# peabody124/PosePipeline

Hardware: AMD Instinct MI355X
Metric: frames/sec (whole node), detect->2D->3D cascade on 1080p; MPJPE vs reference (higher is better)
Workload: dtype f32; eligible float32 convolutions are evaluated as 2-term float16 splits (22 significand bits under per-channel / per-sample power-of-two scales, 3 products per term) on the 16-bit matrix cores with float32 accumulation (float32-accurate at any input magnitude, not bit-identical: tests/test_gpu_spl

## Files before the change

### posepipeline_amd/csrc/api_core.hip

```cpp
#include <dlfcn.h>

#include <algorithm>
#include <memory>

#include "pp_internal.h"
#include "pp_amax.h"

#include <atomic>
extern std::atomic<int> g_decode_generic, g_split_gemm_epi;

static thread_local std::string g_last_error;

void pp_set_error(const char* fmt, ...) {
    char buf[1024];
    va_list ap;
    va_start(ap, fmt);
    vsnprintf(buf, sizeof(buf), fmt, ap);
    va_end(ap);
    g_last_error = buf;
}

namespace {
struct Roctx {
    int (*push)(const char*) = nullptr;
    int (*pop)() = nullptr;
    Roctx() {
        for (const char* lib : {"librocprofiler-sdk-roctx.so", "librocprofiler-sdk-roctx.so.1", "libroctx64.so", "libroctx64.so.4"}) {
            void* h = dlopen(lib, RTLD_LAZY | RTLD_LOCAL);
            if (!h) continue;
            push = reinterpret_cast<int (*)(const char*)>(dlsym(h, "roctxRangePushA"));
            pop = reinterpret_cast<int (*)()>(dlsym(h, "roctxRangePop"));
            if (push && pop) return;
            push = nullptr; pop = nullptr;
        }
    }
};
const Roctx& roctx() {
    static const Roctx r;
    return r;
}
}

void pp_range_push(const char* name) {
    if (roctx().push) (void)roctx().push(name);
}
void pp_range_pop() {
    if (roctx().pop) (void)roctx().pop();
}

int pp_ctx::ensure_scratch(size_t bytes) {
    if (bytes <= scratch_bytes) return PP_OK;
    if (scratch) {
        PP_HIP_CHECK(hipStreamSynchronize(stream));
        PP_HIP_CHECK(hipFree(scratch));
        scratch = nullptr;
        scratch_bytes = 0;
    }
    size_t want = std::max(bytes, size_t(1) << 20);
    PP_HIP_CHECK(hipMalloc(&scratch, want));
    scratch_bytes = want;
    return PP_OK;
}

extern "C" {

int pp_abi_version(void) { return PP_ABI_VERSION; }

int pp_debug_knob(const char* name, int value) {
    PP_REQUIRE(name && value >= -1 && value <= 1, "pp_debug_knob: name and a value in {-1, 0, 1}");
    if (!strcmp(name, "decode_generic")) g_decode_generic.store(value, std::memory_order_relaxed);
    else if (!strcmp(name, "split_gemm_epilogue")) g_split_gemm_epi.store(value, std::memory_order_relaxed);
    else {
        pp_set_error("pp_debug_knob: unknown knob '%s' (decode_generic, split_gemm_epilogue)", name);
        return PP_ERR_ARG;
    }
    return PP_OK;
}

const char* pp_last_error(void) { return g_last_error.c_str(); }

int pp_device_count(void) {
    int n = 0;
    if (hipGetDeviceCount(&n) != hipSuccess) {
        (void)hipGetLastError();
        return 0;
    }
    return n;
}

int pp_ctx_create(int device, pp_ctx** out) {
    PP_REQUIRE(out != nullptr, "pp_ctx_create: out is NULL");
    *out = nullptr;
    int n = 0;
    hipError_t e = hipGetDeviceCount(&n);
    if (e != hipSuccess || n <= 0) {
        (void)hipGetLastError();
        pp_set_error("pp_ctx_create: no HIP device visible (%s) -- this library has no CPU fallback",
                     e == hipSuccess ? "device count 0" : hipGetErrorString(e));
        return PP_ERR_HIP;
    }
    PP_REQUIRE(device >= 0 && device < n, "pp_ctx_create: device %d out of range [0,%d)", device, n);
    PP_HIP_CHECK(hipSetDevice(device));
    std::unique_ptr<pp_ctx> c(new pp_ctx());
    c->device = device;
    PP_HIP_CHECK(hipStreamCreateWithFlags(&c->stream, hipStreamNonBlocking));
    PP_HIP_CHECK(hipEventCreate(&c->ev_start));
    PP_HIP_CHECK(hipEventCreate(&c->ev_stop));
    PP_HIP_CHECK(hipStreamCreateWithFlags(&c->copy_stream, hipStreamNonBlocking));
    PP_HIP_CHECK(hipEventCreateWithFlags(&c->ev_upload, hipEventDisableTiming));
    PP_HIP_CHECK(hipEventCreateWithFlags(&c->ev_consumed, hipEventDisableTiming));
    *out = c.release();
    return PP_OK;
}

void pp_ctx_destroy(pp_ctx* ctx) {
    if (!ctx) return;
    (void)hipSetDevice(ctx->device);
    if (ctx->stream) (void)hipStreamSynchronize(ctx->stream);
    if (ctx->scratch) (void)hipFree(ctx->scratch);
    if (ctx->ev_start) (void)hipEventDestroy(ctx->ev_start);
    if (ctx->ev_stop) (void)hipEventDestroy(ctx->ev_stop);
    if (ctx->copy_stream) {
        (void)hipStreamSynchronize(ctx->copy_stream);
        (void)hipStreamDestroy(ctx->copy_stream);
    }
    if (ctx->ev_upload) (void)hipEventDestroy(ctx->ev_upload);
    if (ctx->ev_consumed) (void)hipEventDestroy(ctx->ev_consumed);
    if (ctx->own_stream && ctx->stream) (void)hipStreamDestroy(ctx->stream);
    delete ctx;
}

int pp_ctx_set_stream(pp_ctx* ctx, void* hip_stream) {
    PP_REQUIRE(ctx, "pp_ctx_set_stream: ctx is NULL");
    PP_HIP_CHECK(hipStreamSynchronize(ctx->stream));
    if (ctx->own_stream && ctx->stream) PP_HIP_CHECK(hipStreamDestroy(ctx->stream));
    ctx->stream = static_cast<hipStream_t>(hip_stream);
    ctx->own_stream = false;
    return PP_OK;
}

int pp_ctx_synchronize(pp_ctx* ctx) {
    PP_REQUIRE(ctx, "pp_ctx_synchronize: ctx is NULL");
    PP_HIP_CHECK(hipStreamSynchronize(ctx->stream));
    return PP_OK;
}

int pp_timer_start(pp_ctx* ctx) {
    PP_REQUIRE(ctx, "pp_timer_start: ctx is NULL");
    PP_HIP_CHECK(hipEventRecord(ctx->ev_start, ctx->stream));
    return PP_OK;
}

int pp_timer_stop(pp_ctx* ctx, float* elapsed_ms) {
    PP_REQUIRE(ctx && elapsed_ms, "pp_timer_stop: NULL argument");
    PP_HIP_CHECK(hipEventRecord(ctx->ev_stop, ctx->stream));
    PP_HIP_CHECK(hipEventSynchronize(ctx->ev_stop));
    PP_HIP_CHECK(hipEventElapsedTime(elapsed_ms, ctx->ev_start, ctx->ev_stop));
    return PP_OK;
}

int pp_malloc(pp_ctx* ctx, size_t bytes, void** dptr) {
    PP_REQUIRE(ctx && dptr, "pp_malloc: NULL argument");
    PP_HIP_CHECK(hipSetDevice(ctx->device));
    PP_HIP_CHECK(hipMalloc(dptr, bytes ? bytes : 1));
    return PP_OK;
}

int pp_free(pp_ctx* ctx, void* dptr) {
    PP_REQUIRE(ctx, "pp_free: ctx is NULL");
    if (!dptr) return PP_OK;
    PP_HIP_CHECK(hipStreamSynchronize(ctx->stream));
    PP_HIP_CHECK(hipFree(dptr));
    return PP_OK;
}

int pp_memcpy_h2d(pp_ctx* ctx, void* dst, const void* src, size_t bytes) {
    PP_REQUIRE(ctx && (bytes == 0 || (dst && src)), "pp_memcpy_h2d: NULL argument");
    PP_HIP_CHECK(hipMemcpyAsync(dst, src, bytes, hipMemcpyHostToDevice, ctx->stream));
    PP_HIP_CHECK(hipStreamSynchronize(ctx->stream));
    return PP_OK;
}

int pp_host_alloc(pp_ctx* ctx, size_t bytes, void** out) {
    PP_REQUIRE(ctx && out, "pp_host_alloc: NULL argument");
    *out = nullptr;
    PP_HIP_CHECK(hipSetDevice(ctx->device));
    PP_HIP_CHECK(hipHostMalloc(out, bytes ? bytes : 1, hipHostMallocDefault));
    return PP_OK;
}

int pp_host_free(pp_ctx* ctx, void* p) {
    PP_REQUIRE(ctx != nullptr, "pp_host_free: ctx is NULL");
    if (p) PP_HIP_CHECK(hipHostFree(p));
    return PP_OK;
}

int pp_upload_begin(pp_ctx* ctx, void* dst, const void* src, size_t bytes) {
    PP_REQUIRE(ctx && (bytes == 0 || (dst && src)), "pp_upload_begin: NULL argument");
    PP_HIP_CHECK(hipStreamWaitEvent(ctx->copy_stream, ctx->ev_consumed, 0));
    PP_HIP_CHECK(hipMemcpyAsync(dst, src, bytes, hipMemcpyHostToDevice, ctx->copy_stream));
    PP_HIP_CHECK(hipEventRecord(ctx->ev_upload, ctx->copy_stream));
    return PP_OK;
}

int pp_upload_begin_nv12(pp_ctx* ctx, void* dst_bgr, void* tmp_nv12, const void* src_host, int frames, int height, int width) {
    PP_REQUIRE(ctx && (frames == 0 || (dst_bgr && tmp_nv12 && src_host)), "pp_upload_begin_nv12: NULL argument");
    PP_REQUIRE(frames >= 0 && height > 0 && width > 0, "pp_upload_begin_nv12: bad shape");
    PP_HIP_CHECK(hipStreamWaitEvent(ctx->copy_stream, ctx->ev_consumed, 0));
    const size_t bytes = (size_t)frames * height * width * 3 / 2;
    if (bytes) PP_HIP_CHECK(hipMemcpyAsync(tmp_nv12, src_host, bytes, hipMemcpyHostToDevice, ctx->copy_stream));
    const int r = pp_launch_nv12_to_bgr((const unsigned char*)tmp_nv12, (unsigned char*)dst_bgr, frames, height, width, ctx->copy_stream);
    if (r != PP_OK) return r;
    PP_HIP_CHECK(hipEventRecord(ctx->ev_upload, ctx->copy_stream));
    return PP_OK;
}

int pp_nv12_to_bgr(pp_ctx* ctx, const uint8_t* nv12, int frames, int height, int width, uint8_t* bgr) {
    PP_REQUIRE(ctx && (frames == 0 || (nv12 && bgr)), "pp_nv12_to_bgr: NULL argument");
    return pp_launch_nv12_to_bgr(nv12, bgr, frames, height, width, ctx->stream);
}

int pp_upload_wait(pp_ctx* ctx, int host_sync) {
    PP_REQUIRE(ctx != nullptr, "pp_upload_wait: ctx is NULL");
    PP_HIP_CHECK(hipStreamWaitEvent(ctx->stream, ctx->ev_upload, 0));
    if (host_sync) PP_HIP_CHECK(hipEventSynchronize(ctx->ev_upload));
    return PP_OK;
}

int pp_upload_release(pp_ctx* ctx) {
    PP_REQUIRE(ctx != nullptr, "pp_upload_release: ctx is NULL");
    PP_HIP_CHECK(hipEventRecord(ctx->ev_consumed, ctx->stream));
    return PP_OK;
}

int pp_memcpy_d2h(pp_ctx* ctx, void* dst, const void* src, size_t bytes) {
    PP_REQUIRE(ctx && (bytes == 0 || (dst && src)), "pp_memcpy_d2h: NULL argument");
    PP_HIP_CHECK(hipMemcpyAsync(dst, src, bytes, hipMemcpyDeviceToHost, ctx->stream));
    PP_HIP_CHECK(hipStreamSynchronize(ctx->stream));
    return PP_OK;
}

int pp_memcpy_d2d(pp_ctx* ctx, void* dst, const void* src, size_t bytes) {
    PP_REQUIRE(ctx && (bytes == 0 || (dst && src)), "pp_memcpy_d2d: NULL argument");
    PP_HIP_CHECK(hipMemcpyAsync(dst, src, bytes, hipMemcpyDeviceToDevice, ctx->stream));
    return PP_OK;
}

}


struct pp_net {
    pp_ctx* ctx = nullptr;
    std::vector<pp_op> ops;
    std::vector<pp_buf> bufs;
    std::vector<size_t> buf_off;
    std::vector<size_t> buf_elems;
    float* weights = nullptr;
    size_t n_weights = 0;
    unsigned char* wsplit = nullptr;
    std::vector<SplitPlan> split_plan;
    int numerics = PP_NET_NUMERICS_EXACT;
    int split_f16 = 0;
    unsigned* amax = nullptr;
    std::vector<int> op_x_slot, op_y_slot, op_post_slot, slot_owner;
    std::vector<int> slot_first, slot_last;
    struct ExtAmax { int buf, slot, first_reader, last_reader; bool provided; };
    std::vector<ExtAmax> ext;
    float* arena = nullptr;
    size_t arena_floats = 0;
    int max_batch = 0;
    hipGraphExec_t graph_exec = nullptr;
    int graph_batch = 0;
    bool use_lanes = true;
    std::vector<hipStream_t> lanes;
    std::vector<int> op_lane;
    std::vector<std::vector<int>> op_waits;
    std::vector<char> op_needs_event;
    std::vector<hipEvent_t> op_done;
    hipEvent_t fork_ev = nullptr;
    std::vector<hipEvent_t> join_ev;
    std::vector<pp_vit_encoder*> vits;
    std::vector<pp_deconv_bf16*> deconvs;

    float* buf_ptr(int b) const { return arena + buf_off[b]; }
    unsigned* amax_slot(int slot) const { return slot >= 0 ? amax + (size_t)slot * max_batch : nullptr; }
};

static ConvArgs net_conv_args(pp_net* net, const pp_op& op, int batch);
static int net_make_lanes(pp_net* net, int n_lanes);

static void net_plan_amax(pp_net* net) {
    const int n = (int)net->ops.size(), nb = (int)net->bufs.size();
    net->op_x_slot.assign(n, -1);
    net->op_y_slot.assign(n, -1);
    net->op_post_slot.assign(n, -1);
    net->slot_owner.clear();
    net->ext.clear();
    if (net->numerics != PP_NET_NUMERICS_SPLIT || !net->split_f16) return;
    auto is_h = [&](int i) { return net->ops[i].type == PP_OP_CONV && net->split_plan[i].kernel != SPLIT_NONE; };
    auto tracks = [&](int i) {
        const pp_op& op = net->ops[i];
        if (op.type == PP_OP_UPSAMPLE_ADD) return true;
        return op.type == PP_OP_CONV && pp_conv_tracks_amax(net_conv_args(net, op, 1), is_h(i));
    };
    {
        std::vector<char> written(nb, 0);
        for (int i = 0; i < n; ++i) {
            const pp_op& op = net->ops[i];
            if (is_h(i) && !written[op.in]) {
                pp_net::ExtAmax* e = nullptr;
                for (auto& x : net->ext)
                    if (x.buf == op.in) e = &x;
                if (!e) {
                    net->ext.push_back({op.in, (int)net->slot_owner.size(), i, i, false});
                    net->slot_owner.push_back(-1);
                    e = &net->ext.back();
                }
                e->last_reader = i;
                net->op_x_slot[i] = e->slot;
            }
            written[op.out] = 1;
        }
    }
    struct Tensor { int slot; std::vector<int> producers; bool wanted; };
    std::vector<Tensor> tensors;
    std::vector<int> cur(nb, -1);
    std::vector<char> read_since(nb, 1);
    std::vector<std::pair<int, int>> readers;
    for (int i = 0; i < n; ++i) {
        const pp_op& op = net->ops[i];
        if (is_h(i) && cur[op.in] >= 0) {
            tensors[cur[op.in]].wanted = true;
            readers.push_back({i, cur[op.in]});
        }
        for (int b : {op.in, op.res1, op.res2, op.in2, op.in3})
            if (b >= 0) read_since[b] = 1;
        if (cur[op.out] < 0 || read_since[op.out]) {
            cur[op.out] = (int)tensors.size();
            tensors.push_back({(int)net->slot_owner.size(), {}, false});
            net->slot_owner.push_back(i);
        }
        tensors[cur[op.out]].producers.push_back(i);
        read_since[op.out] = 0;
    }
    net->slot_first.assign(net->slot_owner.size(), -1);
    net->slot_last.assign(net->slot_owner.size(), -1);
    for (const Tensor& t : tensors) {
        if (!t.wanted) continue;
        net->slot_first[t.slot] = t.producers.front();
        net->slot_last[t.slot] = t.producers.back();
        bool fused = true;
        for (int p : t.producers) fused = fused && tracks(p);
        {
            int covered = 0;
            const int out_b = net->ops[t.producers.front()].out;
            for (int p : t.producers) covered += net->ops[p].type == PP_OP_CONV ? net->ops[p].cout : net->bufs[out_b].c;
            if (covered < net->bufs[out_b].c) fused = false;
        }
        if (fused)
            for (int p : t.producers) net->op_y_slot[p] = t.slot;
        else
            net->op_post_slot[t.producers.back()] = t.slot;
    }
    for (const auto& r : readers) net->op_x_slot[r.first] = tensors[r.second].slot;
}

static int net_reset_amax(pp_net* net, int first, int last, int batch, hipStream_t s) {
    if (!net->amax) return PP_OK;
    int s0 = -1, s1 = -1;
    for (int k = 0; k < (int)net->slot_first.size(); ++k) {
        const int a = net->slot_first[k], b = net->slot_last[k];
        if (a < 0 || b < first || a >= last) continue;
        PP_REQUIRE(a >= first && b < last, "pp_net_run: op range [%d, %d) splits the producers (ops %d .. %d) of a tensor whose per-sample maxima are tracked",
                   first, last, a, b);
    }
    for (int k = 0; k < (int)net->slot_owner.size(); ++k)
        if (net->slot_owner[k] >= first && net->slot_owner[k] < last) {
            if (s0 < 0) s0 = k;
            s1 = k + 1;
        }
    if (s0 >= 0) PP_HIP_CHECK(hipMemsetAsync(net->amax_slot(s0), 0, (size_t)(s1 - s0) * net->max_batch * sizeof(unsigned), s));
    for (auto& e : net->ext) {
        if (e.last_reader < first || e.first_reader >= last) continue;
        if (e.provided) {
            e.provided = false;
            continue;
        }
        PP_HIP_CHECK(hipMemsetAsync(net->amax_slot(e.slot), 0, (size_t)batch * sizeof(unsigned), s));
        int rc = pp_launch_amax(net->buf_ptr(e.buf), batch, net->buf_elems[e.buf], net->amax_slot(e.slot), s);
        if (rc != PP_OK) return rc;
    }
    return PP_OK;
}

static void net_plan_lanes(pp_net* net, int n_lanes) {
    const int n = (int)net->ops.size(), nb = (int)net->bufs.size();
    net->op_lane.assign(n, 0);
    net->op_waits.assign(n, {});
    net->op_needs_event.assign(n, 0);
    std::vector<int> last_writer(nb, -1);
    std::vector<std::vector<int>> readers(nb);
    std::vector<int> lane_tail(n_lanes, -1);
    for (int i = 0; i < n; ++i) {
        const pp_op& op = net->ops[i];
        std::vector<int> deps;
        auto add = [&](int d) {
            if (d >= 0 && std::find(deps.begin(), deps.end(), d) == deps.end()) deps.push_back(d);
        };
        for (int b : {op.in, op.res1, op.res2, op.in2, op.in3})
            if (b >= 0) add(last_writer[b]);
        add(last_writer[op.out]);
        for (int r : readers[op.out]) add(r);
        int lane = -1, best = -1;
        for (int l = 0; l < n_lanes; ++l)
            if (lane_tail[l] >= 0 && lane_tail[l] > best && std::find(deps.begin(), deps.end(), lane_tail[l]) != deps.end()) {
                best = lane_tail[l];
                lane = l;
            }
        if (lane < 0) {
            lane = 0;
            for (int l = 1; l < n_lanes; ++l)
                if (lane_tail[l] < lane_tail[lane]) lane = l;
        }
        net->op_lane[i] = lane;
        for (int d : deps)
            if (net->op_lane[d] != lane) {
                net->op_waits[i].push_back(d);
                net->op_needs_event[d] = 1;
            }
        lane_tail[lane] = i;
        for (int b : {op.in, op.res1, op.res2, op.in2, op.in3})
            if (b >= 0 && b != op.out) readers[b].push_back(i);
        last_writer[op.out] = i;
        readers[op.out].clear();
    }
}

static int net_check_op(const pp_net& net, const pp_op& op, int idx) {
    const int nb = (int)net.bufs.size();
    PP_REQUIRE(op.in >= 0 && op.in < nb && op.out >= 0 && op.out < nb, "op %d: buffer id out of range", idx);
    PP_REQUIRE(op.res1 < nb && op.res2 < nb, "op %d: residual buffer id out of range", idx);
    PP_REQUIRE(op.in2 < nb && op.in3 < nb && (op.type == PP_OP_UPSAMPLE_ADD || (op.in2 < 0 && op.in3 < 0)),
               "op %d: in2 / in3 are inputs of PP_OP_UPSAMPLE_ADD only (-1 elsewhere)", idx);
    const pp_buf& bi = net.bufs[op.in];
    const pp_buf& bo = net.bufs[op.out];
    const int eh = op.pad_end & 1, ew = (op.pad_end >> 1) & 1;
    PP_REQUIRE(op.out_c_off >= 0 && op.in_c_off >= 0 && (op.out_c_off & 3) == 0 && (op.in_c_off & 3) == 0,
               "op %d: channel offsets must be non-negative multiples of 4", idx);
    if (op.type != PP_OP_CONV) {
        for (int b : {op.in, op.out, op.res1, op.res2, op.in2, op.in3})
            PP_REQUIRE(b < 0 || net.bufs[b].pad == 0, "op %d: only convolutions may touch a buffer with a zero halo (buffer %d)", idx, b);
    } else {
        PP_REQUIRE(bo.pad == 0 || (!op.out_nchw && op.out_c_off == 0 && bo.c == op.cout && (op.cout & 3) == 0),
                   "op %d: a halo output buffer must be a plain NHWC tensor of the op's own channels", idx);
    }
    if (op.type == PP_OP_CONV) {
        PP_REQUIRE(bi.c == op.cin && op.in_c_off == 0, "op %d: in buffer has %d channels, op.cin=%d", idx, bi.c, op.cin);
        PP_REQUIRE(op.out_c_off + op.cout <= bo.c && (op.out_c_off == 0 ? true : !op.out_nchw),
                   "op %d: channels [%d, %d) do not fit the out buffer (%d channels)", idx, op.out_c_off,
                   op.out_c_off + op.cout, bo.c);
        PP_REQUIRE(bo.c == op.cout || ((bo.c & 3) == 0 && !op.out_nchw), "op %d: a sliced out buffer needs c %% 4 == 0", idx);
        PP_REQUIRE(op.relu >= PP_RELU_NONE && op.relu <= PP_ACT_SWISH, "op %d: unknown activation %d", idx, op.relu);
        const int ho = pp_conv_out_dim(bi.h + eh, op.kh, op.stride, op.pad_h, op.dil_h) - ((op.pad_end >> 2) & 1);
        const int wo = pp_conv_out_dim(bi.w + ew, op.kw, op.stride, op.pad_w, op.dil_w) - ((op.pad_end >> 3) & 1);
        PP_REQUIRE((ho << op.up_log2) == bo.h && (wo << op.up_log2) == bo.w,
                   "op %d: conv output %dx%d (<<%d) does not match out buffer %dx%d", idx, ho, wo, op.up_log2,
                   bo.h, bo.w);
        const size_t kpad = ((size_t)op.kh * op.kw * op.cin + 31) / 32 * 32;
        const size_t cpad = ((size_t)op.cout + 15) / 16 * 16;
        PP_REQUIRE(op.w_off >= 0 && (size_t)op.w_off + kpad * cpad <= net.n_weights, "op %d: weights out of blob", idx);
        PP_REQUIRE(op.b_off >= 0 && (size_t)op.b_off + cpad <= net.n_weights, "op %d: bias out of blob", idx);
        PP_REQUIRE((op.w_off % 4) == 0 && (op.b_off % 4) == 0, "op %d: blob offsets must be 16-byte aligned", idx);
        if (op.res1 >= 0) PP_REQUIRE(net.bufs[op.res1].c == op.cout, "op %d: res1 channel mismatch", idx);
        if (op.res2 >= 0)
            PP_REQUIRE(net.bufs[op.res2].c == op.cout && net.bufs[op.res2].h == bo.h && net.bufs[op.res2].w == bo.w,
                       "op %d: res2 shape mismatch", idx);
    } else if (op.type == PP_OP_MAXPOOL) {
        PP_REQUIRE(op.cin == op.cout && (op.cin & 3) == 0 && op.in_c_off + op.cin <= bi.c && op.out_c_off + op.cout <= bo.c &&
                       (bi.c & 3) == 0 && (bo.c & 3) == 0,
                   "op %d: maxpool channel slices do not fit", idx);
        PP_REQUIRE(pp_conv_out_dim(bi.h + eh, op.kh, op.stride, op.pad_h, 1) == bo.h &&
                       pp_conv_out_dim(bi.w + ew, op.kw, op.stride, op.pad_w, 1) == bo.w,
                   "op %d: maxpool output dims mismatch", idx);
    } else if (op.type == PP_OP_AVGPOOL) {
        PP_REQUIRE(op.cin == op.cout && (op.cin & 3) == 0 && bi.c == op.cin && bo.c == op.cin && op.in != op.out && op.kh > 0 &&
                       op.kw > 0 && op.stride > 0 && bi.h >= op.kh && bi.w >= op.kw && (bi.h - op.kh) / op.stride + 1 == bo.h &&
                       (bi.w - op.kw) / op.stride + 1 == bo.w,
                   "op %d: avgpool needs in [h][w][c] and out [(h - kh) / s + 1][(w - kw) / s + 1][c], c %% 4 == 0", idx);
    } else if (op.type == PP_OP_COPY) {
        PP_REQUIRE(bi.c == bo.c && bi.h == bo.h && bi.w == bo.w, "op %d: copy shape mismatch", idx);
    } else if (op.type == PP_OP_DEPTH_TO_SPACE) {
        PP_REQUIRE(op.cout > 0 && (op.cout & 3) == 0 && bi.c == 4 * op.cout && bo.c == op.cout && bo.h == 2 * bi.h && bo.w == 2 * bi.w,
                   "op %d: depth_to_space needs in [h][w][4*cout] and out [2h][2w][cout]", idx);
    } else if (op.type == PP_OP_DECONV_BF16) {
        PP_REQUIRE(bi.c == op.cin && bo.c == op.cout && bo.h == 2 * bi.h && bo.w == 2 * bi.w && op.in != op.out,
                   "op %d: deconv_bf16 needs in [h][w][cin] and out [2h][2w][cout]", idx);
        PP_REQUIRE(op.cin % 64 == 0 && (op.cout & 7) == 0, "op %d: deconv_bf16 needs cin %% 64 == 0 and cout %% 8 == 0", idx);
        PP_REQUIRE(op.relu == PP_RELU_NONE || op.relu == PP_RELU_LAST, "op %d: deconv_bf16 supports PP_RELU_NONE / PP_RELU_LAST", idx);
        PP_REQUIRE(op.w_off >= 0 && (op.w_off % 4) == 0 && (size_t)op.w_off + (size_t)16 * op.cout * op.cin <= net.n_weights &&
                       op.b_off >= 0 && (op.b_off % 4) == 0 && (size_t)op.b_off + op.cout <= net.n_weights,
                   "op %d: deconv_bf16 parameters out of blob", idx);
    } else if (op.type == PP_OP_UPSAMPLE_ADD) {
        PP_REQUIRE(op.cin == op.cout && (op.cout & 3) == 0 && bi.c == op.cout && bo.c == op.cout && op.up_log2 >= 0 &&
                       (bi.h << op.up_log2) == bo.h && (bi.w << op.up_log2) == bo.w && op.in != op.out,
                   "op %d: upsample_add needs in [h][w][c] and out [h << up][w << up][c]", idx);
        PP_REQUIRE(op.relu == PP_RELU_NONE || op.relu == PP_RELU_LAST, "op %d: upsample_add supports PP_RELU_NONE / PP_RELU_LAST", idx);
        for (int r : {op.res1, op.res2})
            if (r >= 0)
                PP_REQUIRE(net.bufs[r].c == bo.c && net.bufs[r].h == bo.h && net.bufs[r].w == bo.w, "op %d: residual shape mismatch", idx);
        PP_REQUIRE(op.in3 < 0 || op.in2 >= 0, "op %d: in3 without in2", idx);
        for (int k = 0; k < 2; ++k) {
            const int b = k ? op.in3 : op.in2, u = k ? op.up3_log2 : op.up2_log2;
            if (b >= 0)
                PP_REQUIRE(u >= 0 && u <= 5 && net.bufs[b].c == bo.c && (net.bufs[b].h << u) == bo.h && (net.bufs[b].w << u) == bo.w &&
                               b != op.out, "op %d: in%d must be [h >> up][w >> up][c] of the out buffer", idx, k + 2);
        }
    } else if (op.type == PP_OP_VIT_ENCODER) {
        PP_REQUIRE(op.cin == op.cout && bi.c == op.cin && bo.c == op.cin && bi.h == bo.h && bi.w == bo.w && op.in != op.out,
                   "op %d: vit encoder needs distinct in / out buffers of [h][w][dim]", idx);
        PP_REQUIRE(op.kh > 0 && op.kw > 0 && op.stride > 0, "op %d: vit encoder needs depth (kh), heads (kw), mlp ratio (stride)", idx);
        PP_REQUIRE(op.w_off >= 0 && (op.w_off % 4) == 0 &&
                       (size_t)op.w_off + pp_vit_param_floats(bi.h * bi.w, op.cin, op.kh, op.cin * op.stride) <= net.n_weights,
                   "op %d: vit encoder parameters out of blob", idx);
    } else {
        pp_set_error("op %d: unsupported op type %d", idx, op.type);
        return PP_ERR_UNSUPPORTED;
    }
    return PP_OK;
}

static ConvArgs net_conv_args(pp_net* net, const pp_op& op, int batch) {
    const pp_buf& bi = net->bufs[op.in];
    const pp_buf& bo = net->bufs[op.out];
    ConvArgs a{};
    a.x = net->buf_ptr(op.in);
    a.y = net->buf_ptr(op.out);
    a.w = net->weights + op.w_off;
    a.bias = net->weights + op.b_off;
    a.res1 = op.res1 >= 0 ? net->buf_ptr(op.res1) : nullptr;
    a.res2 = op.res2 >= 0 ? net->buf_ptr(op.res2) : nullptr;
    a.N = batch; a.Hin = bi.h; a.Win = bi.w; a.Cin = op.cin;
    a.Hout = bo.h >> op.up_log2; a.Wout = bo.w >> op.up_log2;
    a.Cout = op.cout; a.CoutPad = (op.cout + 15) / 16 * 16;
    a.KH = op.kh; a.KW = op.kw; a.stride = op.stride; a.pad_h = op.pad_h; a.pad_w = op.pad_w;
    a.dil_h = op.dil_h; a.dil_w = op.dil_w;
    a.K = op.kh * op.kw * op.cin; a.Kpad = (a.K + 31) / 32 * 32;
    a.HWout = a.Hout * a.Wout; a.M = batch * a.HWout;
    a.relu = op.relu; a.up_log2 = op.up_log2; a.out_nchw = op.out_nchw;
    a.res1_shift = op.res1_shift; a.res1_off_w = op.res1_off_w;
    a.res1_H = op.res1 >= 0 ? net->bufs[op.res1].h : 0;
    a.res1_W = op.res1 >= 0 ? net->bufs[op.res1].w : 0;
    a.y_stride = bo.c; a.y_coff = op.out_c_off;
    a.x_pad = bi.pad; a.y_pad = bo.pad;
    a.r1_pad = op.res1 >= 0 ? net->bufs[op.res1].pad : 0;
    a.r2_pad = op.res2 >= 0 ? net->bufs[op.res2].pad : 0;
    const size_t idx = &op - net->ops.data();
    a.wsplit = (net->wsplit && idx < net->split_plan.size() && net->split_plan[idx].off >= 0) ? net->wsplit + net->split_plan[idx].off : nullptr;
    a.numerics = net->numerics;
    a.split_f16 = net->split_f16;
    if (idx < net->op_x_slot.size()) {
        a.x_amax = net->amax_slot(net->op_x_slot[idx]);
        a.y_amax = net->amax_slot(net->op_y_slot[idx]);
    }
    return a;
}

static int net_launch_op_body(pp_net* net, const pp_op& op, int batch, hipStream_t s);

static int net_launch_op(pp_net* net, const pp_op& op, int batch, hipStream_t s) {
    const size_t idx = &op - net->ops.data();
    int rc = net_launch_op_body(net, op, batch, s);
    if (rc == PP_OK && net->amax && net->op_post_slot[idx] >= 0)
        rc = pp_launch_amax(net->buf_ptr(op.out), batch, net->buf_elems[op.out], net->amax_slot(net->op_post_slot[idx]), s);
    return rc;
}

static int net_launch_op_body(pp_net* net, const pp_op& op, int batch, hipStream_t s) {
    const pp_buf& bi = net->bufs[op.in];
    const pp_buf& bo = net->bufs[op.out];
    if (op.type == PP_OP_CONV) {
        const ConvArgs a = net_conv_args(net, op, batch);
        return pp_launch_conv(a, &net->split_plan[&op - net->ops.data()], s);
    } else if (op.type == PP_OP_MAXPOOL) {
        PoolArgs p{};
        p.x = net->buf_ptr(op.in); p.y = net->buf_ptr(op.out);
        p.N = batch; p.Hin = bi.h; p.Win = bi.w; p.C = op.cin; p.Hout = bo.h; p.Wout = bo.w;
        p.x_stride = bi.c; p.x_coff = op.in_c_off; p.y_stride = bo.c; p.y_coff = op.out_c_off;
        p.KH = op.kh; p.KW = op.kw; p.stride = op.stride; p.pad_h = op.pad_h; p.pad_w = op.pad_w;
        return pp_launch_maxpool(p, s);
    } else if (op.type == PP_OP_AVGPOOL) {
        return pp_launch_avgpool(net->buf_ptr(op.in), net->buf_ptr(op.out), batch, bi.h, bi.w, op.cin, op.kh, op.kw, op.stride, s);
    } else if (op.type == PP_OP_COPY) {
        PP_HIP_CHECK(hipMemcpyAsync(net->buf_ptr(op.out), net->buf_ptr(op.in),
                                    (size_t)batch * net->buf_elems[op.in] * sizeof(float),
                                    hipMemcpyDeviceToDevice, s));
        return PP_OK;
    } else if (op.type == PP_OP_DEPTH_TO_SPACE) {
        return pp_launch_depth_to_space(net->buf_ptr(op.in), net->buf_ptr(op.out), batch, bi.h, bi.w, op.cout, s);
    } else if (op.type == PP_OP_DECONV_BF16) {
        return pp_deconv_bf16_run(net->deconvs[&op - net->ops.data()], net->buf_ptr(op.in), net->buf_ptr(op.out), batch,
                                  op.relu == PP_RELU_LAST, s);
    } else if (op.type == PP_OP_UPSAMPLE_ADD) {
        return pp_launch_upsample_add(net->buf_ptr(op.in), op.res1 >= 0 ? net->buf_ptr(op.res1) : nullptr,
                                      op.res2 >= 0 ? net->buf_ptr(op.res2) : nullptr, net->buf_ptr(op.out), batch, bo.h, bo.w,
                                      bo.c, op.up_log2, op.relu == PP_RELU_LAST, s, op.in2 >= 0 ? net->buf_ptr(op.in2) : nullptr,
                                      op.up2_log2, op.in3 >= 0 ? net->buf_ptr(op.in3) : nullptr, op.up3_log2,
                                      net->amax && net->op_y_slot[&op - net->ops.data()] >= 0 ? net->amax_slot(net->op_y_slot[&op - net->ops.data()]) : nullptr);
    } else if (op.type == PP_OP_VIT_ENCODER) {
        pp_vit_encoder* enc = net->vits[&op - net->ops.data()];
        return pp_vit_encoder_run(enc, net->buf_ptr(op.in), net->buf_ptr(op.out), batch, s);
    }
    return PP_ERR_UNSUPPORTED;
}

int pp_net_dims(pp_net* net, int buf, int* h, int* w, int* c) {
    if (!net || buf < 0 || buf >= (int)net->bufs.size()) return PP_ERR_ARG;
    *h = net->bufs[buf].h; *w = net->bufs[buf].w; *c = net->bufs[buf].c;
    return PP_OK;
}
int pp_net_max_batch(pp_net* net) { return net ? net->max_batch : 0; }
pp_ctx* pp_net_ctx(pp_net* net) { return net ? net->ctx : nullptr; }

unsigned* pp_net_input_amax_slot(pp_net* net, int buf) {
    if (!net || !net->amax) return nullptr;
    for (auto& e : net->ext)
        if (e.buf == buf) return net->amax_slot(e.slot);
    return nullptr;
}

extern "C" {

int pp_net_create(pp_ctx* ctx, const pp_op* ops, int n_ops, const pp_buf* bufs, int n_bufs,
                  const float* weights, size_t n_weights, int max_batch, pp_net** out) {
    return pp_net_create_mem(ctx, ops, n_ops, bufs, n_bufs, weights, n_weights, PP_MEM_HOST, max_batch, out);
}

int pp_net_create_mem(pp_ctx* ctx, const pp_op* ops, int n_ops, const pp_buf* bufs, int n_bufs,
                      const float* weights, size_t n_weights, int weights_mem, int max_batch, pp_net** out) {
    return pp_net_create_ex(ctx, ops, n_ops, bufs, n_bufs, weights, n_weights, weights_mem, max_batch, PP_NET_NUMERICS_DEFAULT, out);
}

int pp_net_numerics(pp_net* net) { return net ? net->numerics : PP_ERR_ARG; }
int pp_net_split_kind(pp_net* net) {
    if (!net) return PP_ERR_ARG;
    return net->numerics != PP_NET_NUMERICS_SPLIT ? PP_NET_NUMERICS_EXACT : net->split_f16 ? PP_NET_NUMERICS_SPLIT_F16 : PP_NET_NUMERICS_SPLIT_BF16;
}

int pp_net_create_ex(pp_ctx* ctx, const pp_op* ops, int n_ops, const pp_buf* bufs, int n_bufs,
                     const float* weights, size_t n_weights, int weights_mem, int max_batch, int numerics, pp_net** out) {
    PP_REQUIRE(ctx && ops && bufs && weights && out, "pp_net_create: NULL argument");
    PP_REQUIRE(numerics >= PP_NET_NUMERICS_DEFAULT && numerics <= PP_NET_NUMERICS_SPLIT_F16, "pp_net_create_ex: bad numerics %d", numerics);
    PP_REQUIRE(weights_mem == PP_MEM_HOST || weights_mem == PP_MEM_DEVICE, "pp_net_create: bad weights_mem %d", weights_mem);
    PP_REQUIRE(n_ops > 0 && n_bufs > 0 && max_batch > 0, "pp_net_create: empty program");
    *out = nullptr;
    std::unique_ptr<pp_net> net(new pp_net());
    net->ctx = ctx;
    net->ops.assign(ops, ops + n_ops);
    net->bufs.assign(bufs, bufs + n_bufs);
    net->max_batch = max_batch;
    net->n_weights = n_weights;
    net->numerics = numerics != PP_NET_NUMERICS_DEFAULT ? numerics : (pp_conv_split_enabled() ? PP_NET_NUMERICS_SPLIT : PP_NET_NUMERICS_EXACT);
    if (net->numerics >= PP_NET_NUMERICS_SPLIT) {
        net->split_f16 = net->numerics == PP_NET_NUMERICS_SPLIT ? pp_conv_split_f16_default() : net->numerics == PP_NET_NUMERICS_SPLIT_F16;
        net->numerics = PP_NET_NUMERICS_SPLIT;
    }
    size_t off = 0;
    for (int b = 0; b < n_bufs; ++b) {
        PP_REQUIRE(bufs[b].h > 0 && bufs[b].w > 0 && bufs[b].c > 0 && bufs[b].pad >= 0 && bufs[b].pad <= 8, "buffer %d has an empty dim / bad halo", b);
        const size_t e = (size_t)(bufs[b].h + bufs[b].pad) * (bufs[b].w + bufs[b].pad) * bufs[b].c;
        net->buf_elems.push_back(e);
        net->buf_off.push_back(off);
        off += (e * max_batch + 63) / 64 * 64;
    }
    net->arena_floats = off;
    for (int i = 0; i < n_ops; ++i) {
        int rc = net_check_op(*net, net->ops[i], i);
        if (rc != PP_OK) return rc;
    }
    PP_HIP_CHECK(hipSetDevice(ctx->device));
    PP_HIP_CHECK(hipMalloc((void**)&net->weights, n_weights * sizeof(float)));
    PP_HIP_CHECK(hipMemcpyAsync(net->weights, weights, n_weights * sizeof(float),
                                weights_mem == PP_MEM_HOST ? hipMemcpyHostToDevice : hipMemcpyDeviceToDevice, ctx->stream));
    PP_HIP_CHECK(hipMalloc((void**)&net->arena, net->arena_floats * sizeof(float)));
    PP_HIP_CHECK(hipMemsetAsync(net->arena, 0, net->arena_floats * sizeof(float), ctx->stream));
    net->vits.assign(n_ops, nullptr);
    net->deconvs.assign(n_ops, nullptr);
    for (int i = 0; i < n_ops; ++i) {
        const pp_op& op = net->ops[i];
        if (op.type == PP_OP_DECONV_BF16) {
            const pp_buf& bi = net->bufs[op.in];
            int rc = pp_deconv_bf16_create(net->weights + op.w_off, net->weights + op.b_off, bi.h, bi.w, op.cin, op.cout,
                                           max_batch, ctx->stream, &net->deconvs[i]);
            if (rc != PP_OK) {
                pp_net_destroy(net.release());
                return rc;
            }
        }
        if (op.type != PP_OP_VIT_ENCODER) continue;
        const pp_buf& bi = net->bufs[op.in];
        int rc = pp_vit_encoder_create(net->weights + op.w_off, bi.h * bi.w, op.cin, op.kh, op.kw, op.cin * op.stride,
                                       max_batch, ctx->stream, &net->vits[i]);
        if (rc != PP_OK) {
            pp_net_destroy(net.release());
            return rc;
        }
    }
    net->split_plan.assign(n_ops, SplitPlan());
    if (net->numerics == PP_NET_NUMERICS_SPLIT) {
        size_t bytes = 0;
        for (int i = 0; i < n_ops; ++i) {
            if (net->ops[i].type != PP_OP_CONV) continue;
            SplitPlan p = pp_conv_split_plan(net_conv_args(net.get(), net->ops[i], 1));
            if (p.kernel == SPLIT_NONE) continue;
            p.off = (long long)bytes;
            bytes += (p.bytes + 255) / 256 * 256;
            net->split_plan[i] = p;
        }
        net_plan_amax(net.get());
        if (!net->slot_owner.empty()) {
            const size_t ab = net->slot_owner.size() * (size_t)max_batch * sizeof(unsigned);
            PP_HIP_CHECK(hipMalloc((void**)&net->amax, ab));
            PP_HIP_CHECK(hipMemsetAsync(net->amax, 0, ab, ctx->stream));
        }
        if (bytes) {
            PP_HIP_CHECK(hipMalloc((void**)&net->wsplit, bytes));
            for (int i = 0; i < n_ops; ++i) {
                const SplitPlan& p = net->split_plan[i];
                if (p.kernel == SPLIT_NONE) continue;
                int rc = pp_conv_split_weights(p, net_conv_args(net.get(), net->ops[i], 1), net->wsplit + p.off, ctx->stream);
                if (rc != PP_OK) return rc;
            }
        }
    }
    PP_HIP_CHECK(hipStreamSynchronize(ctx->stream));
    for (int i = 0; i < n_ops; ++i)
        if (net->ops[i].type == PP_OP_CONV) {
            int rc = pp_conv_prepare(net_conv_args(net.get(), net->ops[i], 1));
            if (rc != PP_OK) return rc;
        }
    const char* env_lanes = getenv("POSEPIPE_NET_LANES");
    const int n_lanes = env_lanes ? atoi(env_lanes) : 4;
    int rc_l = net_make_lanes(net.get(), n_lanes);
    if (rc_l != PP_OK) return rc_l;
    *out = net.release();
    return PP_OK;
}

static int net_make_lanes(pp_net* net, int n_lanes) {
    for (auto l : net->lanes) (void)hipStreamDestroy(l);
    net->lanes.clear();
    for (auto e : net->op_done)
        if (e) (void)hipEventDestroy(e);
    net->op_done.clear();
    for (auto e : net->join_ev)
        if (e) (void)hipEventDestroy(e);
    net->join_ev.clear();
    if (net->fork_ev) (void)hipEventDestroy(net->fork_ev);
    net->fork_ev = nullptr;
    const int n_ops = (int)net->ops.size();
    if (n_lanes > 1 && n_ops >= 8) {
        net_plan_lanes(net, n_lanes);
        net->lanes.resize(n_lanes);
        for (auto& l : net->lanes) PP_HIP_CHECK(hipStreamCreateWithFlags(&l, hipStreamNonBlocking));
        net->op_done.assign(n_ops, nullptr);
        for (int i = 0; i < n_ops; ++i)
            if (net->op_needs_event[i]) PP_HIP_CHECK(hipEventCreateWithFlags(&net->op_done[i], hipEventDisableTiming));
        PP_HIP_CHECK(hipEventCreateWithFlags(&net->fork_ev, hipEventDisableTiming));
        net->join_ev.resize(n_lanes);
        for (auto& e : net->join_ev) PP_HIP_CHECK(hipEventCreateWithFlags(&e, hipEventDisableTiming));
    }
    return PP_OK;
}

int pp_net_input_amax(pp_net* net, int buf, void** dptr) {
    PP_REQUIRE(net && dptr && buf >= 0 && buf < (int)net->bufs.size(), "pp_net_input_amax: bad argument");
    *dptr = nullptr;
    for (auto& e : net->ext)
        if (e.buf == buf && net->amax) {
            e.provided = true;
            *dptr = net->amax_slot(e.slot);
        }
    return PP_OK;
}

int pp_net_conv_kinds(pp_net* net, int* kinds) {
    PP_REQUIRE(net && kinds, "pp_net_conv_kinds: NULL argument");
    for (size_t i = 0; i < net->ops.size(); ++i) {
        if (net->ops[i].type != PP_OP_CONV) {
            kinds[i] = 0;
            continue;
        }
        kinds[i] = net->split_plan[i].kernel != SPLIT_NONE ? 2 : 1;
    }
    return PP_OK;
}

void pp_net_destroy(pp_net* net) {
    if (!net) return;
    if (net->ctx && net->ctx->stream) (void)hipStreamSynchronize(net->ctx->stream);
    for (auto l : net->lanes) {
        (void)hipStreamSynchronize(l);
        (void)hipStreamDestroy(l);
    }
    for (auto e : net->op_done)
        if (e) (void)hipEventDestroy(e);
    for (auto e : net->join_ev)
        if (e) (void)hipEventDestroy(e);
    if (net->fork_ev) (void)hipEventDestroy(net->fork_ev);
    if (net->graph_exec) (void)hipGraphExecDestroy(net->graph_exec);
    for (auto* v : net->vits) pp_vit_encoder_destroy(v);
    for (auto* d : net->deconvs) pp_deconv_bf16_destroy(d);
    if (net->weights) (void)hipFree(net->weights);
    if (net->wsplit) (void)hipFree(net->wsplit);
    if (net->amax) (void)hipFree(net->amax);
    if (net->arena) (void)hipFree(net->arena);
    delete net;
}

int pp_net_buffer(pp_net* net, int buf, void** dptr, size_t* bytes_per_sample) {
    PP_REQUIRE(net && buf >= 0 && buf < (int)net->bufs.size(), "pp_net_buffer: bad buffer id");
    PP_REQUIRE(net->bufs[buf].pad == 0, "pp_net_buffer: buffer %d has a zero halo (conv-internal layout); expose dense buffers only", buf);
    if (dptr) *dptr = net->buf_ptr(buf);
    if (bytes_per_sample) *bytes_per_sample = net->buf_elems[buf] * sizeof(float);
    return PP_OK;
}

int pp_net_run(pp_net* net, int batch, int first_op, int last_op) {
    PP_REQUIRE(net, "pp_net_run: net is NULL");
    PP_REQUIRE(batch > 0 && batch <= net->max_batch, "pp_net_run: batch %d not in (0,%d]", batch, net->max_batch);
    if (last_op < 0) last_op = (int)net->ops.size();
    PP_REQUIRE(first_op >= 0 && last_op <= (int)net->ops.size() && first_op <= last_op, "pp_net_run: bad op range");
    if (net->graph_exec && batch == net->graph_batch && first_op == 0 && last_op == (int)net->ops.size()) {
        PP_HIP_CHECK(hipGraphLaunch(net->graph_exec, net->ctx->stream));
        return PP_OK;
    }
    hipStream_t main = net->ctx->stream;
    PpRange range("pp_net_run");
    {
        int rc = net_reset_amax(net, first_op, last_op, batch, main);
        if (rc != PP_OK) return rc;
    }
    if (net->lanes.empty() || !net->use_lanes || last_op - first_op < 8) {
        for (int i = first_op; i < last_op; ++i) {
            int rc = net_launch_op(net, net->ops[i], batch, main);
            if (rc != PP_OK) return rc;
        }
        return PP_OK;
    }
    PP_HIP_CHECK(hipEventRecord(net->fork_ev, main));
    for (hipStream_t l : net->lanes) PP_HIP_CHECK(hipStreamWaitEvent(l, net->fork_ev, 0));
    for (int i = first_op; i < last_op; ++i) {
        hipStream_t s = net->lanes[net->op_lane[i]];
        for (int d : net->op_waits[i])
            if (d >= first_op) PP_HIP_CHECK(hipStreamWaitEvent(s, net->op_done[d], 0));
        int rc = net_launch_op(net, net->ops[i], batch, s);
        if (rc != PP_OK) return rc;
        if (net->op_needs_event[i]) PP_HIP_CHECK(hipEventRecord(net->op_done[i], s));
    }
    for (size_t l = 0; l < net->lanes.size(); ++l) {
        PP_HIP_CHECK(hipEventRecord(net->join_ev[l], net->lanes[l]));
        PP_HIP_CHECK(hipStreamWaitEvent(main, net->join_ev[l], 0));
    }
    return PP_OK;
}

int pp_net_vit_timing(pp_net* net, int enable, float* ms3, int* n_gemm) {
    PP_REQUIRE(net, "pp_net_vit_timing: net is NULL");
    for (auto* v : net->vits) {
        if (!v) continue;
        if (ms3) {
            PP_HIP_CHECK(hipStreamSynchronize(net->ctx->stream));
            int rc = pp_vit_encoder_get_timing(v, ms3, n_gemm);
            if (rc != PP_OK) return rc;
        }
        pp_vit_encoder_set_timing(v, enable);
        return PP_OK;
    }
    pp_set_error("pp_net_vit_timing: the program has no PP_OP_VIT_ENCODER");
    return PP_ERR_STATE;
}

int pp_net_set_lane_count(pp_net* net, int n_lanes) {
    PP_REQUIRE(net && n_lanes >= 1 && n_lanes <= 16, "pp_net_set_lane_count: net is NULL or n_lanes not in [1, 16]");
    PP_HIP_CHECK(hipStreamSynchronize(net->ctx->stream));
    for (auto l : net->lanes) PP_HIP_CHECK(hipStreamSynchronize(l));
    if (net->graph_exec) {
        PP_HIP_CHECK(hipGraphExecDestroy(net->graph_exec));
        net->graph_exec = nullptr;
    }
    return net_make_lanes(net, n_lanes);
}

int pp_net_set_lanes(pp_net* net, int enable) {
    PP_REQUIRE(net, "pp_net_set_lanes: net is NULL");
    PP_HIP_CHECK(hipStreamSynchronize(net->ctx->stream));
    net->use_lanes = enable != 0;
    return PP_OK;
}

int pp_net_capture(pp_net* net, int batch) {
    PP_REQUIRE(net, "pp_net_capture: net is NULL");
    PP_REQUIRE(batch > 0 && batch <= net->max_batch, "pp_net_capture: bad batch");
    if (net->graph_exec) {
        PP_HIP_CHECK(hipGraphExecDestroy(net->graph_exec));
        net->graph_exec = nullptr;
    }
    hipStream_t s = net->ctx->stream;
    PP_HIP_CHECK(hipStreamSynchronize(s));
    hipGraph_t graph = nullptr;
    PP_HIP_CHECK(hipStreamBeginCapture(s, hipStreamCaptureModeThreadLocal));
    int rc = net_reset_amax(net, 0, (int)net->ops.size(), batch, s);
    for (size_t i = 0; i < net->ops.size() && rc == PP_OK; ++i) rc = net_launch_op(net, net->ops[i], batch, s);
    hipError_t e = hipStreamEndCapture(s, &graph);
    if (rc != PP_OK) {
        if (graph) (void)hipGraphDestroy(graph);
        return rc;
    }
    PP_HIP_CHECK(e);
    PP_HIP_CHECK(hipGraphInstantiate(&net->graph_exec, graph, nullptr, nullptr, 0));
    PP_HIP_CHECK(hipGraphDestroy(graph));
    net->graph_batch = batch;
    return PP_OK;
}

int pp_net_forward(pp_net* net, int batch, int in_buf, const float* in, int out_buf, float* out, int mem) {
    PP_REQUIRE(net && in && out, "pp_net_forward: NULL argument");
    PP_REQUIRE(in_buf >= 0 && in_buf < (int)net->bufs.size() && out_buf >= 0 && out_buf < (int)net->bufs.size(),
               "pp_net_forward: bad buffer id");
    PP_REQUIRE(batch > 0 && batch <= net->max_batch, "pp_net_forward: batch %d not in (0,%d]", batch, net->max_batch);
    PP_REQUIRE(net->bufs[in_buf].pad == 0 && net->bufs[out_buf].pad == 0, "pp_net_forward: input / output buffers must be dense (pad 0)");
    hipStream_t s = net->ctx->stream;
    const hipMemcpyKind kin = mem == PP_MEM_HOST ? hipMemcpyHostToDevice : hipMemcpyDeviceToDevice;
    const hipMemcpyKind kout = mem == PP_MEM_HOST ? hipMemcpyDeviceToHost : hipMemcpyDeviceToDevice;
    PP_HIP_CHECK(hipMemcpyAsync(net->buf_ptr(in_buf), in, (size_t)batch * net->buf_elems[in_buf] * sizeof(float), kin, s));
    for (auto& e : net->ext)
        if (e.buf == in_buf) e.provided = false;
    int rc = pp_net_run(net, batch, 0, (int)net->ops.size());
    if (rc != PP_OK) return rc;
    PP_HIP_CHECK(hipMemcpyAsync(out, net->buf_ptr(out_buf), (size_t)batch * net->buf_elems[out_buf] * sizeof(float), kout, s));
    PP_HIP_CHECK(hipStreamSynchronize(s));
    return PP_OK;
}

int pp_net_profile(pp_net* net, int batch, float* ms_per_op) {
    PP_REQUIRE(net, "pp_net_profile: net is NULL");
    PP_REQUIRE(batch > 0 && batch <= net->max_batch, "pp_net_profile: bad batch");
    hipStream_t s = net->ctx->stream;
    const size_t n = net->ops.size();
    std::vector<hipEvent_t> ev(n + 1);
    for (auto& e : ev) PP_HIP_CHECK(hipEventCreate(&e));
    int rc = net_reset_amax(net, 0, (int)n, batch, s);
    PP_HIP_CHECK(hipEventRecord(ev[0], s));
    for (size_t i = 0; i < n && rc == PP_OK; ++i) {
        rc = net_launch_op(net, net->ops[i], batch, s);
        if (rc == PP_OK && hipEventRecord(ev[i + 1], s) != hipSuccess) rc = PP_ERR_HIP;
    }
    if (rc == PP_OK && hipStreamSynchronize(s) != hipSuccess) rc = PP_ERR_HIP;
    if (rc == PP_OK && ms_per_op) {
        for (size_t i = 0; i < n; ++i) {
            float ms = 0.f;
            (void)hipEventElapsedTime(&ms, ev[i], ev[i + 1]);
            ms_per_op[i] = ms;
        }
    }
    for (auto& e : ev) (void)hipEventDestroy(e);
    return rc;
}

int pp_conv2d(pp_ctx* ctx, const pp_op* op, int n, int hin, int win, const float* x, const float* w,
              const float* bias, const float* res1, const float* res2, float* y, int res1_h, int res1_w,
              int mem) {
    PP_REQUIRE(ctx && op && x && w && bias && y, "pp_conv2d: NULL argument");
    PP_REQUIRE(op->type == PP_OP_CONV, "pp_conv2d: op is not a conv");
    PP_REQUIRE(n > 0 && hin > 0 && win > 0, "pp_conv2d: empty input");
    ConvArgs a{};
    a.N = n; a.Hin = hin; a.Win = win; a.Cin = op->cin;
    a.Hout = pp_conv_out_dim(hin + (op->pad_end & 1), op->kh, op->stride, op->pad_h, op->dil_h) - ((op->pad_end >> 2) & 1);
    a.Wout = pp_conv_out_dim(win + ((op->pad_end >> 1) & 1), op->kw, op->stride, op->pad_w, op->dil_w) - ((op->pad_end >> 3) & 1);
    PP_REQUIRE(a.Hout > 0 && a.Wout > 0, "pp_conv2d: empty output");
    a.Cout = op->cout; a.CoutPad = (op->cout + 15) / 16 * 16;
    a.KH = op->kh; a.KW = op->kw; a.stride = op->stride; a.pad_h = op->pad_h; a.pad_w = op->pad_w;
    a.dil_h = op->dil_h; a.dil_w = op->dil_w;
    a.K = op->kh * op->kw * op->cin; a.Kpad = (a.K + 31) / 32 * 32;
    a.HWout = a.Hout * a.Wout; a.M = n * a.HWout;
    a.relu = op->relu; a.up_log2 = op->up_log2; a.out_nchw = op->out_nchw;
    a.res1_shift = op->res1_shift; a.res1_off_w = op->res1_off_w;
    const int Ho2 = a.Hout << op->up_log2, Wo2 = a.Wout << op->up_log2;
    a.res1_H = res1 ? (res1_h > 0 ? res1_h : Ho2) : 0;
    a.res1_W = res1 ? (res1_w > 0 ? res1_w : Wo2) : 0;
    a.y_stride = op->cout; a.y_coff = 0;
    PP_REQUIRE(op->out_c_off == 0 && op->in_c_off == 0, "pp_conv2d: channel slices need a layer program");
    const size_t x_e = (size_t)n * hin * win * op->cin;
    const size_t w_e = (size_t)a.Kpad * a.CoutPad;
    const size_t b_e = a.CoutPad;
    const size_t y_e = (size_t)n * Ho2 * Wo2 * op->cout;
    const size_t r1_e = res1 ? (size_t)n * a.res1_H * a.res1_W * op->cout : 0;
    const size_t r2_e = res2 ? y_e : 0;
    if (mem == PP_MEM_DEVICE) {
        a.x = x; a.w = w; a.bias = bias; a.res1 = res1; a.res2 = res2; a.y = y;
        return pp_launch_conv(a, nullptr, ctx->stream);
    }
    size_t total = 0;
    for (size_t e : {x_e, w_e, b_e, y_e, r1_e, r2_e}) total += ScratchCursor::align(e * sizeof(float));
    int rc = ctx->ensure_scratch(total);
    if (rc != PP_OK) return rc;
    ScratchCursor cur(ctx);
    float* dx = cur.take<float>(x_e);
    float* dw = cur.take<float>(w_e);
    float* db = cur.take<float>(b_e);
    float* dy = cur.take<float>(y_e);
    float* dr1 = cur.take<float>(r1_e);
    float* dr2 = cur.take<float>(r2_e);
    hipStream_t s = ctx->stream;
    PP_HIP_CHECK(hipMemcpyAsync(dx, x, x_e * 4, hipMemcpyHostToDevice, s));
    PP_HIP_CHECK(hipMemcpyAsync(dw, w, w_e * 4, hipMemcpyHostToDevice, s));
    PP_HIP_CHECK(hipMemcpyAsync(db, bias, b_e * 4, hipMemcpyHostToDevice, s));
    if (res1) PP_HIP_CHECK(hipMemcpyAsync(dr1, res1, r1_e * 4, hipMemcpyHostToDevice, s));
    if (res2) PP_HIP_CHECK(hipMemcpyAsync(dr2, res2, r2_e * 4, hipMemcpyHostToDevice, s));
    a.x = dx; a.w = dw; a.bias = db; a.res1 = res1 ? dr1 : nullptr; a.res2 = res2 ? dr2 : nullptr; a.y = dy;
    rc = pp_launch_conv(a, nullptr, s);
    if (rc != PP_OK) return rc;
    PP_HIP_CHECK(hipMemcpyAsync(y, dy, y_e * 4, hipMemcpyDeviceToHost, s));
    PP_HIP_CHECK(hipStreamSynchronize(s));
    return PP_OK;
}

}
```

### posepipeline_amd/csrc/conv_igemm.hip

```cpp
#include <dlfcn.h>

#include <algorithm>
#include <atomic>
#include <cstdlib>
#include <map>
#include <mutex>
#include <vector>

#include "pp_internal.h"
#include "pp_amax.h"

typedef float f32x4 __attribute__((ext_vector_type(4)));

namespace {

constexpr int BK = 32;

__device__ __forceinline__ int swz(int j) {
    return ((j >> 1) & 1) | ((j & 1) << 1) | ((((j >> 1) ^ (j >> 2)) & 1) << 2);
}

__device__ __forceinline__ unsigned udiv(unsigned n, unsigned m, unsigned s1, unsigned s2) {
    const unsigned t = __umulhi(m, n);
    return (t + ((n - t) >> s1)) >> s2;
// ... 82 lines not shown
        const bool kok = k0 + 4 * kq < a.K;
        if constexpr (WALK) {
            int kw1 = kw0 + 1, kh1 = kh0;
            if (kw1 == a.KW) {
                kw1 = 0;
                kh1 = kh0 + 1;
            }
            const unsigned d0 = (unsigned)((kh0 * a.dil_h * a.Win + kw0 * a.dil_w) * a.Cin + c0s) * 4u;
            const unsigned d1 = (unsigned)((kh1 * a.dil_h * a.Win + kw1 * a.dil_w) * a.Cin + c0s - a.Cin) * 4u;
            const unsigned p0 = ((unsigned)(kh0 * a.dil_h) << 16) | (unsigned)(kw0 * a.dil_w);
            const unsigned p1 = ((unsigned)(kh1 * a.dil_h) << 16) | (unsigned)(kw1 * a.dil_w);
            const bool first = 4 * kq < a.Cin - c0s;
            const unsigned dpk = kok ? (first ? p0 : p1) : 0x7fff7fffu;
            const unsigned delta = (first ? d0 : d1) + (unsigned)kq16;
#pragma unroll
            for (int i = 0; i < NQ; ++i) {
                const u16x2 hw = __builtin_bit_cast(u16x2, __builtin_bit_cast(i16x2, phw[i]) + __builtin_bit_cast(i16x2, dpk));
                const bool ok = __builtin_bit_cast(unsigned, __builtin_elementwise_max(hw, __builtin_bit_cast(u16x2, lim))) == lim;
                const unsigned off = ok ? pbase[i] + delta : 0xffffffffu;
                xr[i] = __builtin_bit_cast(float4, __builtin_amdgcn_raw_buffer_load_b128(xrsrc, (int)off, 0, 0));
            }
            c0s += BK;
            if (c0s >= a.Cin) {
                c0s -= a.Cin;
                kh0 = kh1;
                kw0 = kw1;
            }
        } else {
            const unsigned k4 = (unsigned)(k0 + 4 * kq);
            const unsigned tap = udiv(k4, a.div_c_m, a.div_c_s1, a.div_c_s2);
            const int qc = (int)(k4 - tap * (unsigned)a.Cin);
            const int qkh = (int)udiv(tap, a.div_kw_m, a.div_kw_s1, a.div_kw_s2);
            const int qkw = (int)tap - qkh * a.KW;
            const int dh = qkh * a.dil_h, dw = qkw * a.dil_w;
#pragma unroll
            for (int i = 0; i < NQ; ++i) {
                const int hi = (phw[i] >> 16) + dh;
                const int wi = (int)(short)(phw[i] & 0xffff) + dw;
                const bool ok = kok && (unsigned)hi < (unsigned)a.Hin && (unsigned)wi < (unsigned)a.Win;
                const unsigned off = ok ? (pbase[i] + (unsigned)((hi * a.Win + wi) * a.Cin + qc)) * 4u : 0xffffffffu;
                xr[i] = __builtin_bit_cast(float4, __builtin_amdgcn_raw_buffer_load_b128(xrsrc, (int)off, 0, 0));
            }
        }
        const float* wsrc = wblob + (size_t)(k0 / BK) * a.CoutPad * BK;
        wr0 = *reinterpret_cast<const float4*>(wsrc + wofs0);
        if (NW > 1) wr1 = *reinterpret_cast<const float4*>(wsrc + wofs1);
    };

    auto store_chunk = [&]() {
        const int within = kq & 3, hi_slot = kq >> 2;
#pragma unroll
        for (int i = 0; i < NQ; ++i) {
            float* row = Xs + (prow0 + 32 * i) * BK + within;
            row[((0 + hi_slot) ^ wsw) * 4] = xr[i].x;
            row[((2 + hi_slot) ^ wsw) * 4] = xr[i].y;
            row[((4 + hi_slot) ^ wsw) * 4] = xr[i].z;
            row[((6 + hi_slot) ^ wsw) * 4] = xr[i].w;
        }
        *reinterpret_cast<float4*>(Ws + prow0 * BK + ((kq ^ wsw) * 4)) = wr0;
        if (NW > 1) *reinterpret_cast<float4*>(Ws + (prow0 + 32) * BK + ((kq ^ wsw) * 4)) = wr1;
    };

    f32x4 acc[CT][PT];
#pragma unroll
    for (int ct = 0; ct < CT; ++ct)
#pragma unroll
        for (int pt = 0; pt < PT; ++pt) acc[ct][pt] = f32x4{0.f, 0.f, 0.f, 0.f};

    const int lrow = lane >> 4;
    const int lcol = lane & 15;
    const int rsw = swz(lcol);
    const float* wrd = Ws + lcol * BK;
    const float* xrd = Xs + (wave * (16 * PT) + lcol) * BK;

    f32x4 av[CT], bv[PT];
    auto read_operands = [&](int h) {
        const int so = ((2 * lrow + h) ^ rsw) * 4;
#pragma unroll
        for (int ct = 0; ct < CT; ++ct) av[ct] = *reinterpret_cast<const f32x4*>(wrd + ct * 16 * BK + so);
#pragma unroll
        for (int pt = 0; pt < PT; ++pt) bv[pt] = *reinterpret_cast<const f32x4*>(xrd + pt * 16 * BK + so);
    };
    auto mma_steps = [&](int s0, int s1) {
#pragma unroll
        for (int s = s0; s < s1; ++s)
#pragma unroll
            for (int ct = 0; ct < CT; ++ct)
#pragma unroll
                for (int pt = 0; pt < PT; ++pt)
                    acc[ct][pt] = __builtin_amdgcn_mfma_f32_16x16x4f32(av[ct][s], bv[pt][s], acc[ct][pt], 0, 0, 0);
    };

    load_chunk(0);
    int k0 = 0;
    for (; k0 + BK < a.Kpad; k0 += BK) {
        __syncthreads();
        store_chunk();
        __syncthreads();
        read_operands(0);
        __builtin_amdgcn_sched_barrier(0);
        mma_steps(0, 1);
        __builtin_amdgcn_sched_barrier(0);
        load_chunk(k0 + BK);
        __builtin_amdgcn_sched_barrier(0);
        mma_steps(1, 4);
        read_operands(1);
        mma_steps(0, 4);
    }
    __syncthreads();
    store_chunk();
    __syncthreads();
    read_operands(0);
    mma_steps(0, 4);
    if (k0 + 16 < a.K) {
        read_operands(1);
        mma_steps(0, 4);
    }

    const int up = a.up_log2;
    const int f = 1 << up;
    const int Ho2 = a.Hout << up, Wo2 = a.Wout << up;
    const bool vec4 = ((a.Cout & 3) == 0) && !a.out_nchw;
    const bool res1_plain = (a.res1_shift == 0 && a.res1_off_w == 0 && a.res1_H == Ho2 && a.res1_W == Wo2);
    if (up == 0 && vec4 && (!a.res1 || res1_plain) && a.relu <= PP_RELU_FIRST && a.y_stride == a.Cout) {
        constexpr int PB = (CT * PT <= 6) ? PT : 1;
        bool cok[CT];
        int cos[CT];
        float4 b4[CT];
#pragma unroll
        for (int ct = 0; ct < CT; ++ct) {
            const int co = c0 + ct * 16 + 4 * lrow;
            cok[ct] = co < a.Cout;
            cos[ct] = cok[ct] ? co : 0;
            b4[ct] = *reinterpret_cast<const float4*>(a.bias + cos[ct]);
        }
        float ymax[PT];
#pragma unroll
        for (int pt = 0; pt < PT; ++pt) ymax[pt] = 0.f;
#pragma unroll
        for (int p0 = 0; p0 < PT; p0 += PB) {
            bool mok[PB];
            size_t moff[PB];
#pragma unroll
            for (int pb = 0; pb < PB; ++pb) {
                const int m = m0 + wave * (16 * PT) + (p0 + pb) * 16 + lcol;
                mok[pb] = m < a.M;
                moff[pb] = (size_t)(mok[pb] ? m : 0) * (size_t)a.Cout;
            }
            float4 o[CT][PB];
            if (a.res1) {
#pragma unroll
                for (int ct = 0; ct < CT; ++ct)
#pragma unroll
                    for (int pb = 0; pb < PB; ++pb)
                        o[ct][pb] = *reinterpret_cast<const float4*>(a.res1 + moff[pb] + cos[ct]);
            }
#pragma unroll
            for (int ct = 0; ct < CT; ++ct)
#pragma unroll
                for (int pb = 0; pb < PB; ++pb) {
                    const f32x4 c = acc[ct][p0 + pb];
                    float4 v = make_float4(c[0] + b4[ct].x, c[1] + b4[ct].y, c[2] + b4[ct].z, c[3] + b4[ct].w);
                    if (a.relu == PP_RELU_FIRST) { v.x = fmaxf(v.x, 0.f); v.y = fmaxf(v.y, 0.f); v.z = fmaxf(v.z, 0.f); v.w = fmaxf(v.w, 0.f); }
                    if (a.res1) { v.x += o[ct][pb].x; v.y += o[ct][pb].y; v.z += o[ct][pb].z; v.w += o[ct][pb].w; }
                    o[ct][pb] = v;
                }
            if (a.res2) {
                float4 r2[CT][PB];
#pragma unroll
                for (int ct = 0; ct < CT; ++ct)
#pragma unroll
                    for (int pb = 0; pb < PB; ++pb)
                        r2[ct][pb] = *reinterpret_cast<const float4*>(a.res2 + moff[pb] + cos[ct]);
#pragma unroll
                for (int ct = 0; ct < CT; ++ct)
#pragma unroll
                    for (int pb = 0; pb < PB; ++pb) {
                        o[ct][pb].x += r2[ct][pb].x; o[ct][pb].y += r2[ct][pb].y;
                        o[ct][pb].z += r2[ct][pb].z; o[ct][pb].w += r2[ct][pb].w;
                    }
            }
#pragma unroll
            for (int ct = 0; ct < CT; ++ct)
#pragma unroll
                for (int pb = 0; pb < PB; ++pb) {
                    float4 v = o[ct][pb];
                    if (a.relu == PP_RELU_LAST) { v.x = fmaxf(v.x, 0.f); v.y = fmaxf(v.y, 0.f); v.z = fmaxf(v.z, 0.f); v.w = fmaxf(v.w, 0.f); }
                    if (mok[pb] && cok[ct]) {
                        *reinterpret_cast<float4*>(a.y + moff[pb] + cos[ct]) = v;
                        ymax[p0 + pb] = fmaxf(ymax[p0 + pb], pp_abs4max(v));
                    }
                }
        }
        if (a.y_amax) {
            __shared__ float amax_red[16];
            int yimg[PT];
#pragma unroll
            for (int pt = 0; pt < PT; ++pt)
                yimg[pt] = (int)udiv((unsigned)min(m0 + wave * (16 * PT) + pt * 16 + lcol, a.M - 1), a.div_hw_m, a.div_hw_s1, a.div_hw_s2);
            const unsigned wlast = (unsigned)min(m0 + 64 * PT - 1, a.M - 1);
            pp_amax_commit_wg<4, PT>(a.y_amax, yimg, ymax, (int)udiv((unsigned)min(m0, (int)wlast), a.div_hw_m, a.div_hw_s1, a.div_hw_s2),
                                     (int)udiv(wlast, a.div_hw_m, a.div_hw_s1, a.div_hw_s2), amax_red);
        }
        return;
    }
#pragma unroll
    for (int pt = 0; pt < PT; ++pt) {
        const int m = m0 + wave * (16 * PT) + pt * 16 + lcol;
        if (m >= a.M) continue;
        const int n = (int)udiv((unsigned)m, a.div_hw_m, a.div_hw_s1, a.div_hw_s2);
        const int rem = m - n * a.HWout;
        const int ho = (int)udiv((unsigned)rem, a.div_w_m, a.div_w_s1, a.div_w_s2);
        const int wo = rem - ho * a.Wout;
#pragma unroll
        for (int ct = 0; ct < CT; ++ct) {
            const int co = c0 + ct * 16 + 4 * lrow;
            if (co >= a.Cout) continue;
            const float4 b4 = *reinterpret_cast<const float4*>(a.bias + co);
            float v[4] = {acc[ct][pt][0] + b4.x, acc[ct][pt][1] + b4.y, acc[ct][pt][2] + b4.z,
                          acc[ct][pt][3] + b4.w};
            if (a.relu == PP_RELU_FIRST) {
#pragma unroll
                for (int r = 0; r < 4; ++r) v[r] = fmaxf(v[r], 0.f);
            } else if (a.relu >= PP_ACT_LEAKY) {
#pragma unroll
                for (int r = 0; r < 4; ++r) v[r] = activate(v[r], a.relu);
            }
            for (int dy = 0; dy < f; ++dy) {
                for (int dx = 0; dx < f; ++dx) {
                    const int h2 = (ho << up) + dy, w2 = (wo << up) + dx;
                    const size_t opix = ((size_t)n * Ho2 + h2) * Wo2 + w2;
                    float o[4] = {v[0], v[1], v[2], v[3]};
                    if (a.res1) {
                        size_t rpix = opix;
                        if (!res1_plain) {
                            rpix = ((size_t)n * a.res1_H + (h2 >> a.res1_shift)) * a.res1_W +
                                   (w2 >> a.res1_shift) + a.res1_off_w;
                        }
                        const float* rp = a.res1 + rpix * a.Cout + co;
                        if (vec4) {
                            const float4 r4 = *reinterpret_cast<const float4*>(rp);
                            o[0] += r4.x; o[1] += r4.y; o[2] += r4.z; o[3] += r4.w;
                        } else {
#pragma unroll
                            for (int r = 0; r < 4; ++r)
                                if (co + r < a.Cout) o[r] += rp[r];
                        }
                    }
                    if (a.res2) {
                        const float* rp = a.res2 + opix * a.Cout + co;
                        if (vec4) {
                            const float4 r4 = *reinterpret_cast<const float4*>(rp);
                            o[0] += r4.x; o[1] += r4.y; o[2] += r4.z; o[3] += r4.w;
                        } else {
#pragma unroll
                            for (int r = 0; r < 4; ++r)
                                if (co + r < a.Cout) o[r] += rp[r];
                        }
                    }
                    if (a.relu == PP_RELU_LAST) {
#pragma unroll
                        for (int r = 0; r < 4; ++r) o[r] = fmaxf(o[r], 0.f);
                    }
                    if (a.out_nchw) {
                        const size_t plane = (size_t)Ho2 * Wo2;
                        float* yp = a.y + ((size_t)n * a.Cout + co) * plane + (size_t)h2 * Wo2 + w2;
#pragma unroll
                        for (int r = 0; r < 4; ++r)
                            if (co + r < a.Cout) yp[r * plane] = o[r];
                    } else if (vec4) {
                        *reinterpret_cast<float4*>(a.y + opix * a.y_stride + a.y_coff + co) = make_float4(o[0], o[1], o[2], o[3]);
                    } else {
                        float* yp = a.y + opix * a.y_stride + a.y_coff + co;
#pragma unroll
                        for (int r = 0; r < 4; ++r)
                            if (co + r < a.Cout) yp[r] = o[r];
                    }
                }
            }
        }
    }
}

template <int CT, int PT>
int launch_t(const ConvArgs& a, hipStream_t stream) {
    dim3 grid((a.M + 64 * PT - 1) / (64 * PT), (a.CoutPad + 16 * CT - 1) / (16 * CT));
    if (a.Cin >= BK)
        hipLaunchKernelGGL((conv_igemm_kernel<CT, PT, true>), grid, dim3(256), 0, stream, a);
    else
        hipLaunchKernelGGL((conv_igemm_kernel<CT, PT, false>), grid, dim3(256), 0, stream, a);
    hipError_t e = hipGetLastError();
    if (e != hipSuccess) {
        pp_set_error("conv_igemm launch failed: %s", hipGetErrorString(e));
        return PP_ERR_HIP;
    }
    return PP_OK;
}

template <int CT>
int launch_ct(const ConvArgs& a, int pt, hipStream_t stream) {
    return pt >= 2 ? launch_t<CT, 2>(a, stream) : launch_t<CT, 1>(a, stream);
}

__global__ __launch_bounds__(256) void maxpool_kernel(PoolArgs a) {
    const int c4n = a.C >> 2;
    const size_t xs = a.x_stride ? a.x_stride : a.C, ys = a.y_stride ? a.y_stride : a.C;
    const size_t total = (size_t)a.N * a.Hout * a.Wout * c4n;
    for (size_t i = blockIdx.x * (size_t)blockDim.x + threadIdx.x; i < total; i += (size_t)gridDim.x * blockDim.x) {
        const int c4 = i % c4n;
        size_t p = i / c4n;
        const int wo = p % a.Wout;
        p /= a.Wout;
        const int ho = p % a.Hout;
        const int n = p / a.Hout;
        float4 m = make_float4(-INFINITY, -INFINITY, -INFINITY, -INFINITY);
        for (int kh = 0; kh < a.KH; ++kh) {
            const int hi = ho * a.stride - a.pad_h + kh;
            if ((unsigned)hi >= (unsigned)a.Hin) continue;
            for (int kw = 0; kw < a.KW; ++kw) {
                const int wi = wo * a.stride - a.pad_w + kw;
                if ((unsigned)wi >= (unsigned)a.Win) continue;
                const float4 v = *reinterpret_cast<const float4*>(
                    a.x + (((size_t)n * a.Hin + hi) * a.Win + wi) * xs + a.x_coff + 4 * c4);
                m.x = fmaxf(m.x, v.x); m.y = fmaxf(m.y, v.y); m.z = fmaxf(m.z, v.z); m.w = fmaxf(m.w, v.w);
            }
        }
        *reinterpret_cast<float4*>(a.y + (((size_t)n * a.Hout + ho) * a.Wout + wo) * ys + a.y_coff + 4 * c4) = m;
    }
}

int env_int(const char* name, int dflt) {
    const char* v = getenv(name);
    return v ? atoi(v) : dflt;
}

struct TuneKey {
    int cin, cout, kh, kw, stride, dil_h, dil_w;
    bool operator<(const TuneKey& o) const { return memcmp(this, &o, sizeof(TuneKey)) < 0; }
};
struct TuneTable {
    struct Choice { int m, ct, pt, variant; };
    std::map<TuneKey, std::vector<Choice>> best;
    TuneTable() {
        std::string path;
        if (const char* e = getenv("POSEPIPE_CONV_TUNING")) {
            path = e;
        } else {
            Dl_info info;
            if (dladdr((void*)&pp_conv_out_dim, &info) && info.dli_fname) {
                path = info.dli_fname;
                const size_t slash = path.rfind('/');
                path = (slash == std::string::npos ? std::string(".") : path.substr(0, slash)) + "/conv_tuning.txt";
            }
        }
        if (path.empty() || path == "0") return;
        FILE* f = fopen(path.c_str(), "r");
        if (!f) return;
        char line[256];
        while (fgets(line, sizeof(line), f)) {
            TuneKey k;
            memset(&k, 0, sizeof(k));
            Choice c{0, 0, 0, -1};
            if (line[0] == '#' || sscanf(line, "%d %d %d %d %d %d %d %d %d %d %d", &k.cin, &k.cout, &k.kh, &k.kw, &k.stride, &k.dil_h,
                                         &k.dil_w, &c.m, &c.ct, &c.pt, &c.variant) < 10)
                continue;
            if (c.ct >= 1 && c.ct <= 4 && (c.pt == 1 || c.pt == 2) && c.m > 0 && c.variant != 2) best[k].push_back(c);
        }
        fclose(f);
        for (auto& kv : best) std::sort(kv.second.begin(), kv.second.end(), [](const Choice& x, const Choice& y) { return x.m < y.m; });
    }
    const Choice* find(const TuneKey& k, int m) const {
        auto it = best.find(k);
        if (it == best.end()) return nullptr;
        const Choice* pick = nullptr;
        double best_r = 1.5;
        for (const Choice& c : it->second) {
            const double r = c.m > m ? (double)c.m / m : (double)m / c.m;
            if (r <= best_r) {
                best_r = r;
                pick = &c;
            }
        }
        return pick;
    }
};
struct TapKey {
    int dev, cin, kh, kw, dil_h, dil_w, win, k;
    bool operator<(const TapKey& o) const { return memcmp(this, &o, sizeof(TapKey)) < 0; }
};
std::mutex g_tap_mutex;
std::map<TapKey, uint2*> g_tap_tables;

const uint2* tap_table_for(const ConvArgs& a, bool create) {
    TapKey key;
    memset(&key, 0, sizeof(key));
    if (hipGetDevice(&key.dev) != hipSuccess) return nullptr;
    const int pitch = a.Win + a.x_pad;
    key.cin = a.Cin; key.kh = a.KH; key.kw = a.KW; key.dil_h = a.dil_h; key.dil_w = a.dil_w; key.win = pitch; key.k = a.K;
    std::lock_guard<std::mutex> lock(g_tap_mutex);
    auto it = g_tap_tables.find(key);
    if (it != g_tap_tables.end()) return it->second;
    if (!create) return nullptr;
    const int nsteps = (a.K + 15) / 16;
    std::vector<uint2> h((size_t)(nsteps + 1) * 4);
    for (int s = 0; s <= nsteps; ++s)
        for (int q = 0; q < 4; ++q) {
            const int k = 16 * s + 4 * q;
            uint2 e = make_uint2(0x7fff7fffu, 0x80000000u);
            if (k < a.K) {
                const int tap = k / a.Cin, c = k - tap * a.Cin;
                const int kh = tap / a.KW, kw = tap - kh * a.KW;
                e.x = ((unsigned)(kh * a.dil_h) << 16) | (unsigned)(kw * a.dil_w);
                e.y = (unsigned)(((kh * a.dil_h * pitch + kw * a.dil_w) * a.Cin + c) * 4);
            }
            h[(size_t)s * 4 + q] = e;
        }
    uint2* d = nullptr;
    if (hipMalloc((void**)&d, h.size() * sizeof(uint2)) != hipSuccess) return nullptr;
    if (hipMemcpy(d, h.data(), h.size() * sizeof(uint2), hipMemcpyHostToDevice) != hipSuccess) {
        (void)hipFree(d);
        return nullptr;
    }
    g_tap_tables[key] = d;
    return d;
}

int g_force_ct = 0, g_force_pt = 0;
int g_variant = -1;

}

extern "C" int pp_conv_variant(int variant) {
    if (variant < -1 || variant > 4) {
        pp_set_error("pp_conv_variant: -1 (default), 0 (two-barrier kernel), 1 (three-stage pipelined kernel), 3 (pipelined + tap table: "
                     "the bit-exact default) or 4 (bf16-split kernel where eligible)");
        return PP_ERR_ARG;
    }
    g_variant = variant;
    return PP_OK;
}

extern "C" int pp_conv_force(int ct, int pt) {
    if (ct < 0 || ct > 4 || (pt != 0 && pt != 1 && pt != 2)) {
        pp_set_error("pp_conv_force: ct in 0..4, pt in {0, 1, 2} (0 = automatic)");
        return PP_ERR_ARG;
    }
    g_force_ct = ct;
    g_force_pt = pt;
    return PP_OK;
}

int pp_conv_out_dim(int in, int k, int stride, int pad, int dil) {
    return (in + 2 * pad - dil * (k - 1) - 1) / stride + 1;
}

static void magic_u32(unsigned d, unsigned* m, unsigned* s1, unsigned* s2) {
    unsigned l = 0;
    while ((1ull << l) < d) ++l;
    *m = (unsigned)((((1ull << l) - d) << 32) / d + 1);
    *s1 = l < 1 ? l : 1;
    *s2 = l > 0 ? l - 1 : 0;
}

std::atomic<int> g_exact{-1};
bool pp_conv_split_enabled() {
    static const int env_exact = env_int("POSEPIPE_CONV_EXACT", 0);
    static const int env_variant = env_int("POSEPIPE_CONV_VARIANT", -1);
    const int v = g_variant >= 0 ? g_variant : env_variant;
    const int ge = g_exact.load(std::memory_order_relaxed);
    const int exact = ge >= 0 ? ge : env_exact;
    return v == 4 || (v < 0 && !exact);
}

std::atomic<int> g_split_f16{-1};
bool pp_conv_split_f16_default() {
    static const int env_f16 = env_int("POSEPIPE_SPLIT_F16", 1);
    const int g = g_split_f16.load(std::memory_order_relaxed);
    return (g >= 0 ? g : env_f16) != 0;
}

extern "C" int pp_conv_split_kind(int f16) {
    if (f16 < -1 || f16 > 1) {
        pp_set_error("pp_conv_split_kind: 1 (two float16 terms, three products), 0 (three bfloat16 terms, six products) or -1 (POSEPIPE_SPLIT_F16)");
        return PP_ERR_ARG;
    }
    g_split_f16.store(f16, std::memory_order_relaxed);
    return PP_OK;
}

extern "C" int pp_conv_exact(int exact) {
    if (exact < -1 || exact > 1) {
        pp_set_error("pp_conv_exact: 1 (bit-exact fp32 MFMA kernels), 0 (bf16-split kernels where eligible) or -1 (POSEPIPE_CONV_EXACT)");
        return PP_ERR_ARG;
    }
    g_exact.store(exact, std::memory_order_relaxed);
    return PP_OK;
}

bool pp_conv_tracks_amax(const ConvArgs& a, bool split) {
    if (a.HWout < 64) return false;
    if (split) return true;
    const int Ho2 = a.Hout << a.up_log2, Wo2 = a.Wout << a.up_log2;
    const bool res1_plain = a.res1_shift == 0 && a.res1_off_w == 0 && a.res1_H == Ho2 && a.res1_W == Wo2;
    return a.up_log2 == 0 && (a.Cout & 3) == 0 && !a.out_nchw && (!a.res1 || res1_plain) && a.relu <= PP_RELU_FIRST &&
           (a.y_stride == 0 || a.y_stride == a.Cout);
}

int pp_conv_prepare(const ConvArgs& a) {
    if (a.Cin % 4 != 0 || a.K <= 0) return PP_OK;
    return tap_table_for(a, true) ? PP_OK : PP_ERR_HIP;
}

int pp_launch_conv(const ConvArgs& a_in, const SplitPlan* plan, hipStream_t stream) {
    ConvArgs a = a_in;
    a.tap_table = nullptr;
    magic_u32((unsigned)a.HWout, &a.div_hw_m, &a.div_hw_s1, &a.div_hw_s2);
    magic_u32((unsigned)a.Wout, &a.div_w_m, &a.div_w_s1, &a.div_w_s2);
    magic_u32((unsigned)a.Cin, &a.div_c_m, &a.div_c_s1, &a.div_c_s2);
    magic_u32((unsigned)a.KW, &a.div_kw_m, &a.div_kw_s1, &a.div_kw_s2);
    static const int xcd_remap = env_int("POSEPIPE_CONV_XCD", 1);
    a.xcd_remap = xcd_remap;
    if (a.Cin % 4 != 0) {
        pp_set_error("conv: Cin=%d must be a multiple of 4 (pad the input channels)", a.Cin);
        return PP_ERR_ARG;
    }
    if (a.Hin + a.pad_h >= 32768 || a.Win + a.pad_w >= 32768) {
        pp_set_error("conv: spatial dims must be < 32768");
        return PP_ERR_ARG;
    }
    if (a.M <= 0) return PP_OK;
    const size_t img_bytes = (size_t)(a.Hin + a.x_pad) * (a.Win + a.x_pad) * a.Cin * sizeof(float);
    static const size_t max_bytes_env = (size_t)env_int("POSEPIPE_CONV_MAX_MB", 0) << 20;
    const size_t max_bytes = max_bytes_env ? max_bytes_env : 0xfffffff0u;
    if (img_bytes > max_bytes) {
        pp_set_error("conv: one input image of %zu bytes exceeds the 4 GiB buffer range", img_bytes);
        return PP_ERR_ARG;
    }
    if ((size_t)a.N * img_bytes > max_bytes) {
        const int per = (int)(max_bytes / img_bytes);
        const size_t y_img = (size_t)((a.Hout << a.up_log2) + a.y_pad) * ((a.Wout << a.up_log2) + a.y_pad) * (a.y_stride ? a.y_stride : a.Cout);
        const size_t r1_img = (size_t)(a.res1_H + a.r1_pad) * (a.res1_W + a.r1_pad) * a.Cout;
        const size_t r2_img = (size_t)((a.Hout << a.up_log2) + a.r2_pad) * ((a.Wout << a.up_log2) + a.r2_pad) * a.Cout;
        for (int n0 = 0; n0 < a.N; n0 += per) {
            ConvArgs p = a_in;
            p.N = std::min(per, a.N - n0);
            p.M = p.N * a.HWout;
            p.x = a.x + (size_t)n0 * (img_bytes / sizeof(float));
            p.y = a.y + (size_t)n0 * y_img;
            if (a.res1) p.res1 = a.res1 + (size_t)n0 * r1_img;
            if (a.res2) p.res2 = a.res2 + (size_t)n0 * r2_img;
            if (a.x_amax) p.x_amax = a.x_amax + n0;
            if (a.y_amax) p.y_amax = a.y_amax + n0;
            const int rc = pp_launch_conv(p, plan, stream);
            if (rc != PP_OK) return rc;
        }
        return PP_OK;
    }
    a.x_bytes = (unsigned)((size_t)a.N * img_bytes);
    if (a.y_stride == 0) a.y_stride = a.Cout;
    if (plan && plan->kernel != SPLIT_NONE) return pp_launch_conv_split(*plan, a, stream);
    if (!plan && a.numerics == 0 && pp_conv_split_enabled()) {
        a.split_f16 = pp_conv_split_f16_default();
        const SplitPlan p = pp_conv_split_plan(a);
        if (p.kernel != SPLIT_NONE) {
            void* tmp = nullptr;
            const size_t wbytes = (p.bytes + 255) / 256 * 256;
            PP_HIP_CHECK(hipMalloc(&tmp, wbytes + (p.f16 ? (size_t)a.N * sizeof(unsigned) : 0)));
            a.wsplit = tmp;
            int rc = pp_conv_split_weights(p, a, tmp, stream);
            if (rc == PP_OK && p.f16) {
                unsigned* am = reinterpret_cast<unsigned*>(static_cast<unsigned char*>(tmp) + wbytes);
                if (hipMemsetAsync(am, 0, (size_t)a.N * sizeof(unsigned), stream) != hipSuccess) rc = PP_ERR_HIP;
                if (rc == PP_OK) rc = pp_launch_amax(a.x, a.N, img_bytes / sizeof(float), am, stream);
                a.x_amax = am;
            }
            if (rc == PP_OK) rc = pp_launch_conv_split(p, a, stream);
            (void)hipStreamSynchronize(stream);
            (void)hipFree(tmp);
            return rc;
        }
    }
    if (a.y_amax && !pp_conv_tracks_amax(a, false)) {
        pp_set_error("conv: this layer's epilogue does not track the output maximum (ConvArgs::y_amax; see pp_conv_tracks_amax)");
        return PP_ERR_STATE;
    }
    static const int force_ct = env_int("POSEPIPE_CONV_CT", 0), force_pt = env_int("POSEPIPE_CONV_PT", 0),
                     min_blocks = env_int("POSEPIPE_CONV_MIN_BLOCKS", 512);
    const int tiles = a.CoutPad / 16;
    int best_ct = 1, best_waste = 1 << 30;
    for (int ct = 4; ct >= 1; --ct) {
        const int waste = ((tiles + ct - 1) / ct) * ct - tiles;
        if (waste < best_waste) {
            best_waste = waste;
            best_ct = ct;
        }
    }
    static const TuneTable tuning;
    static const int env_variant = env_int("POSEPIPE_CONV_VARIANT", -1);
    int tuned_pt = 0, variant = 0;
    if (!tuning.best.empty()) {
        TuneKey k;
        memset(&k, 0, sizeof(k));
        k.cin = a.Cin; k.cout = a.Cout; k.kh = a.KH; k.kw = a.KW; k.stride = a.stride; k.dil_h = a.dil_h; k.dil_w = a.dil_w;
        if (const TuneTable::Choice* c = tuning.find(k, a.M)) {
            best_ct = c->ct;
            tuned_pt = c->pt;
            if (c->variant >= 0) variant = c->variant;
        }
    }
    if (env_variant >= 0) variant = env_variant;
    if (g_variant >= 0) variant = g_variant;
    if (variant == 4) variant = 0;
    if (force_ct) best_ct = force_ct;
    if (g_force_ct) best_ct = g_force_ct;
    const int cblocks = (tiles + best_ct - 1) / best_ct;
    int pt = 2;
    while (pt > 1 && (long)((a.M + 64 * pt - 1) / (64 * pt)) * cblocks < min_blocks) pt >>= 1;
    if (tuned_pt) pt = tuned_pt;
    if (force_pt) pt = force_pt;
    if (g_force_pt) pt = g_force_pt;
    {
        static const int pt_by_ct[5] = {0, env_int("POSEPIPE_CONV_PT_CT1", 0), env_int("POSEPIPE_CONV_PT_CT2", 0),
                                        env_int("POSEPIPE_CONV_PT_CT3", 0), env_int("POSEPIPE_CONV_PT_CT4", 0)};
        if (pt_by_ct[best_ct] && (long)((a.M + 64 * pt_by_ct[best_ct] - 1) / (64 * pt_by_ct[best_ct])) * cblocks >= min_blocks)
            pt = pt_by_ct[best_ct];
    }
    a.no_bounds = 0;
    const bool halo = (a.x_pad | a.y_pad | a.r1_pad | a.r2_pad) != 0;
    if (halo) variant = 3;
    if (variant == 3) {
        a.no_bounds = a.pad_h <= a.x_pad && a.pad_w <= a.x_pad &&
                      (a.Hout - 1) * a.stride - a.pad_h + (a.KH - 1) * a.dil_h <= a.Hin - 1 + a.x_pad &&
                      (a.Wout - 1) * a.stride - a.pad_w + (a.KW - 1) * a.dil_w <= a.Win - 1 + a.x_pad && a.x_bytes < 0x7fffff00u;
        a.tap_table = tap_table_for(a, true);
        if (!a.tap_table) {
            pp_set_error("conv: could not build the tap table");
            return PP_ERR_HIP;
        }
    }
    if (variant >= 1) return pp_launch_conv_p3(a, best_ct, pt, stream, variant == 2);
    switch (best_ct) {
        case 4: return launch_ct<4>(a, pt, stream);
        case 3: return launch_ct<3>(a, pt, stream);
        case 2: return launch_ct<2>(a, pt, stream);
        default: return launch_ct<1>(a, pt, stream);
    }
}

int pp_launch_maxpool(const PoolArgs& a, hipStream_t stream) {
    if (a.C % 4 != 0) {
        pp_set_error("maxpool: C=%d must be a multiple of 4", a.C);
        return PP_ERR_ARG;
    }
    const size_t total = (size_t)a.N * a.Hout * a.Wout * (a.C / 4);
    if (total == 0) return PP_OK;
    const int blocks = (int)std::min<size_t>((total + 255) / 256, 256 * 8);
    hipLaunchKernelGGL(maxpool_kernel, dim3(blocks), dim3(256), 0, stream, a);
    hipError_t e = hipGetLastError();
    if (e != hipSuccess) {
        pp_set_error("maxpool launch failed: %s", hipGetErrorString(e));
        return PP_ERR_HIP;
    }
    return PP_OK;
}
```

### posepipeline_amd/csrc/conv_split.hip

```cpp
#include <algorithm>
#include <atomic>
#include <map>
#include <mutex>
#include <type_traits>
#include <vector>
#include <cstring>
#include <cstdio>

#include "pp_internal.h"
#include "pp_amax.h"

#ifndef PP_SPLIT_ABLATE
#define PP_SPLIT_ABLATE 0
#endif

typedef __attribute__((ext_vector_type(8))) __bf16 bf16x8;
typedef __attribute__((ext_vector_type(8))) _Float16 f16x8;
typedef __attribute__((ext_vector_type(16))) float f32x16;

std::atomic<int> g_split_gemm_epi{-1};

namespace {


// ... 1424 lines not shown
        __builtin_amdgcn_s_barrier();
    }

    }

    PP_TL_MARK(2);
    PP_TL_MARK(6);
    if (a.epi_lds) {
        unsigned char* stg = smem + wave * (16384 + 2048);
        uint4* tab = reinterpret_cast<uint4*>(stg + 16384);
#pragma unroll
        for (int i = 0; i < 2; ++i) {
            const int p = lane + 64 * i;
            const long long m = m0 + wm * 128 + p;
            uint4 t = make_uint4(0u, 0u, 0u, 0u);
            if (m < a.S) {
                const int img = (int)pp_udiv((unsigned)m, a.dv_per), rem = (int)((unsigned)m - (unsigned)img * (unsigned)(a.H * a.W));
                const int oy = (int)pp_udiv((unsigned)rem, a.dv_row), ox = rem - oy * a.W;
                t.x = (unsigned)(((size_t)img * (a.H + a.y_pad) + oy) * (a.W + a.y_pad) + ox);
                t.y = (unsigned)(((size_t)img * (a.r1_H + a.r1_pad) + (oy >> a.r1_shift)) * (a.r1_W + a.r1_pad) + (ox >> a.r1_shift));
                t.z = (unsigned)(((size_t)img * (a.H + a.r2_pad) + oy) * (a.W + a.r2_pad) + ox);
                t.w = (unsigned)img + 1u;
            }
            tab[p] = t;
        }
        const int rdrow = lane >> 3, rdpos = lane & 7, rdchunk = rdpos ^ rdrow;
        float xinv[H ? 4 : 1];
        if constexpr (H) {
#pragma unroll
            for (int pb = 0; pb < 4; ++pb) xinv[pb] = pp_act_unscale(oam_first);
            if (img_first != img_last) {
#pragma unroll
                for (int pb = 0; pb < 4; ++pb) {
                    const unsigned mp = (unsigned)min(m0 + wm * 128 + pb * 32 + (lane & 31), a.S - 1);
                    xinv[pb] = pp_act_unscale(a.x_amax[pp_udiv(mp, a.dv_per)]);
                }
            }
        }
        float ymax = 0.f, ymax1 = 0.f;
#pragma unroll
        for (int cb = 0; cb < 2; ++cb) {
#pragma unroll
            for (int pb = 0; pb < 4; ++pb)
#pragma unroll
                for (int g = 0; g < 4; ++g) {
                    const int co = (cb0 + cb) * 32 + 8 * g + 4 * (lane >> 5);
                    const float4 b4 = *reinterpret_cast<const float4*>(a.bias + co);
                    const f32x16 cc = acc[cb][pb];
                    float4 v;
                    if constexpr (H) {
                        const float4 sc = *reinterpret_cast<const float4*>(a.wscale + co);
                        const float xi = xinv[pb];
                        v = make_float4(__builtin_fmaf(cc[4 * g + 0], sc.x * xi, b4.x), __builtin_fmaf(cc[4 * g + 1], sc.y * xi, b4.y),
                                        __builtin_fmaf(cc[4 * g + 2], sc.z * xi, b4.z), __builtin_fmaf(cc[4 * g + 3], sc.w * xi, b4.w));
                    } else {
                        v = make_float4(cc[4 * g + 0] + b4.x, cc[4 * g + 1] + b4.y, cc[4 * g + 2] + b4.z, cc[4 * g + 3] + b4.w);
                    }
                    if (a.relu == PP_RELU_FIRST) { v.x = fmaxf(v.x, 0.f); v.y = fmaxf(v.y, 0.f); v.z = fmaxf(v.z, 0.f); v.w = fmaxf(v.w, 0.f); }
                    else if (a.relu >= PP_ACT_LEAKY) { v.x = split_activate(v.x, a.relu); v.y = split_activate(v.y, a.relu); v.z = split_activate(v.z, a.relu); v.w = split_activate(v.w, a.relu); }
                    *reinterpret_cast<float4*>(stg + (pb * 32 + (lane & 31)) * 128 + (((2 * g + (lane >> 5)) ^ (lane & 7)) << 4)) = v;
                }
            const int co = (cb0 + cb) * 32 + rdchunk * 4;
            const unsigned* tabw = reinterpret_cast<const unsigned*>(tab);
#pragma unroll
            for (int h8 = 0; h8 < 2; ++h8) {
            float4 vv[8];
#pragma unroll
            for (int i8 = 0; i8 < 8; ++i8) vv[i8] = *reinterpret_cast<const float4*>(stg + ((h8 * 8 + i8) * 8 + rdrow) * 128 + rdpos * 16);
            if (a.res1) {
                float4 rv[8];
#pragma unroll
                for (int i8 = 0; i8 < 8; ++i8) rv[i8] = *reinterpret_cast<const float4*>(a.res1 + (size_t)tabw[((h8 * 8 + i8) * 8 + rdrow) * 4 + 1] * a.Cout + co);
#pragma unroll
                for (int i8 = 0; i8 < 8; ++i8) { vv[i8].x += rv[i8].x; vv[i8].y += rv[i8].y; vv[i8].z += rv[i8].z; vv[i8].w += rv[i8].w; }
            }
            if (a.res2) {
                float4 rv[8];
#pragma unroll
                for (int i8 = 0; i8 < 8; ++i8) rv[i8] = *reinterpret_cast<const float4*>(a.res2 + (size_t)tabw[((h8 * 8 + i8) * 8 + rdrow) * 4 + 2] * a.Cout + co);
#pragma unroll
                for (int i8 = 0; i8 < 8; ++i8) { vv[i8].x += rv[i8].x; vv[i8].y += rv[i8].y; vv[i8].z += rv[i8].z; vv[i8].w += rv[i8].w; }
            }
#pragma unroll
            for (int i8 = 0; i8 < 8; ++i8) {
                const int it = h8 * 8 + i8;
                float4 v = vv[i8];
                if (a.relu == PP_RELU_LAST) { v.x = fmaxf(v.x, 0.f); v.y = fmaxf(v.y, 0.f); v.z = fmaxf(v.z, 0.f); v.w = fmaxf(v.w, 0.f); }
                const uint2 t = *reinterpret_cast<const uint2*>(tabw + (it * 8 + rdrow) * 4);
                const unsigned tw = tabw[(it * 8 + rdrow) * 4 + 3];
                if (tw) *reinterpret_cast<float4*>(a.y + (size_t)t.x * a.Cout + co) = v;
                if (a.y_amax) {
                    const float m = tw ? pp_abs4max(v) : 0.f;
                    if (img_last - img_first <= 1) {
                        if ((int)tw - 1 == img_first) ymax = fmaxf(ymax, m);
                        else ymax1 = fmaxf(ymax1, m);
                    } else {
                        float m8 = fmaxf(m, __shfl_xor(m, 1));
                        m8 = fmaxf(m8, __shfl_xor(m8, 2));
                        m8 = fmaxf(m8, __shfl_xor(m8, 4));
                        if (rdpos == 0 && m8 > 0.f) atomicMax(a.y_amax + (tw - 1u), __float_as_uint(m8));
                    }
                }
            }
            }
        }
        if (a.y_amax) {
            const unsigned wlast = (unsigned)min(m0 + BM - 1, a.S - 1);
            const int im[2] = {img_first, img_last};
            const float ym[2] = {ymax, ymax1};
            pp_amax_commit_wg<NWAVE, 2>(a.y_amax, im, ym, (int)pp_udiv((unsigned)min(m0, (long long)wlast), a.dv_per), (int)pp_udiv(wlast, a.dv_per),
                                        reinterpret_cast<float*>(smem));
        }
        PP_TL_MARK(3);
#ifdef PP_SPLIT_TIMELINE
        asm volatile("s_waitcnt vmcnt(0)" ::: "memory");
        PP_TL_MARK(7);
#endif
        PP_TL_FLUSH();
        return;
    }

    int rimg[4];
    float rmax[4];
#pragma unroll
    for (int pb = 0; pb < 4; ++pb) {
        const long long mt = m0 + wm * 128 + pb * 32 + (lane & 31);
        const bool pok = mt < a.S;
        const long long m = pok ? mt : a.S - 1;
        const int img = (int)pp_udiv((unsigned)m, a.dv_per), rem = (int)((unsigned)m - (unsigned)img * (unsigned)(a.H * a.W));
        float xi = 1.f, ymax = 0.f;
        if constexpr (H) xi = pp_act_unscale(a.x_amax[img]);
        rimg[pb] = img;
        const int oy = (int)pp_udiv((unsigned)rem, a.dv_row), ox = rem - oy * a.W;
        const size_t ypix = ((size_t)img * (a.H + a.y_pad) + oy) * (a.W + a.y_pad) + ox;
        const size_t r1pix = ((size_t)img * (a.r1_H + a.r1_pad) + (oy >> a.r1_shift)) * (a.r1_W + a.r1_pad) + (ox >> a.r1_shift);
        const size_t r2pix = ((size_t)img * (a.H + a.r2_pad) + oy) * (a.W + a.r2_pad) + ox;
#pragma unroll
        for (int cb = 0; cb < 2; ++cb) {
#pragma unroll
            for (int g = 0; g < 4; ++g) {
                const int co = (cb0 + cb) * 32 + 8 * g + 4 * (lane >> 5);
                if (co >= a.Cout || !pok) continue;
                const float4 b4 = *reinterpret_cast<const float4*>(a.bias + co);
                const f32x16 cc = acc[cb][pb];
                float4 v;
                if constexpr (H) {
                    const float4 sc = *reinterpret_cast<const float4*>(a.wscale + co);
                    v = make_float4(__builtin_fmaf(cc[4 * g + 0], sc.x * xi, b4.x), __builtin_fmaf(cc[4 * g + 1], sc.y * xi, b4.y),
                                    __builtin_fmaf(cc[4 * g + 2], sc.z * xi, b4.z), __builtin_fmaf(cc[4 * g + 3], sc.w * xi, b4.w));
                } else {
                    v = make_float4(cc[4 * g + 0] + b4.x, cc[4 * g + 1] + b4.y, cc[4 * g + 2] + b4.z, cc[4 * g + 3] + b4.w);
                }
                if (a.relu == PP_RELU_FIRST) { v.x = fmaxf(v.x, 0.f); v.y = fmaxf(v.y, 0.f); v.z = fmaxf(v.z, 0.f); v.w = fmaxf(v.w, 0.f); }
                else if (a.relu >= PP_ACT_LEAKY) { v.x = split_activate(v.x, a.relu); v.y = split_activate(v.y, a.relu); v.z = split_activate(v.z, a.relu); v.w = split_activate(v.w, a.relu); }
                if (a.res1) {
                    const float4 r = *reinterpret_cast<const float4*>(a.res1 + r1pix * a.Cout + co);
                    v.x += r.x; v.y += r.y; v.z += r.z; v.w += r.w;
                }
                if (a.res2) {
                    const float4 r = *reinterpret_cast<const float4*>(a.res2 + r2pix * a.Cout + co);
                    v.x += r.x; v.y += r.y; v.z += r.z; v.w += r.w;
                }
                if (a.relu == PP_RELU_LAST) { v.x = fmaxf(v.x, 0.f); v.y = fmaxf(v.y, 0.f); v.z = fmaxf(v.z, 0.f); v.w = fmaxf(v.w, 0.f); }
                *reinterpret_cast<float4*>(a.y + ypix * a.Cout + co) = v;
                ymax = fmaxf(ymax, pp_abs4max(v));
            }
        }
        rmax[pb] = ymax;
    }
    if (a.y_amax) {
        const unsigned wlast = (unsigned)min(m0 + BM - 1, a.S - 1);
        pp_amax_commit_wg<NWAVE, 4>(a.y_amax, rimg, rmax, (int)pp_udiv((unsigned)min(m0, (long long)wlast), a.dv_per), (int)pp_udiv(wlast, a.dv_per),
                                    reinterpret_cast<float*>(smem));
    }
}

template <bool H>
__global__ __launch_bounds__(256) void split_weights_kernel(const float* w, uint4* out, int Cin, int taps, int CoutPad, int ncb,
                                                            size_t total, const float* cmax) {
    const size_t i = blockIdx.x * (size_t)256 + threadIdx.x;
    if (i >= total) return;
    const int lane = (int)(i & 63);
    size_t r = i >> 6;
    const int cb = (int)(r % ncb);
    r /= ncb;
    const int t = (int)(r % taps);
    const int c = (int)(r / taps);
    const int cout = cb * 32 + (lane & 31);
    unsigned short h[3][8];
#pragma unroll
    for (int j = 0; j < 8; ++j) {
        const int cin = c * 16 + (lane >> 5) * 8 + j;
        const int k = t * Cin + cin;
        float v = 0.f;
        if (cout < CoutPad) v = w[((size_t)(k >> 5) * CoutPad + cout) * 32 + 8 * (k & 3) + ((k & 31) >> 2)];
        if constexpr (H) {
            split_weight_h(v, channel_scale(cmax[cout]), h[0][j], h[1][j], h[2][j]);
            continue;
        }
        const __bf16 q0 = (__bf16)v;
        const float r1 = v - (float)q0;
        const __bf16 q1 = (__bf16)r1;
        const float r2 = r1 - (float)q1;
        const __bf16 q2 = (__bf16)r2;
        h[0][j] = __builtin_bit_cast(unsigned short, q0);
        h[1][j] = __builtin_bit_cast(unsigned short, q1);
        h[2][j] = __builtin_bit_cast(unsigned short, q2);
    }
    constexpr int WPL = H ? 2 : 3;
    const size_t frag = (i >> 6) * WPL;
#pragma unroll
    for (int pl = 0; pl < WPL; ++pl) {
        uint4 o;
        o.x = h[pl][0] | ((unsigned)h[pl][1] << 16);
        o.y = h[pl][2] | ((unsigned)h[pl][3] << 16);
        o.z = h[pl][4] | ((unsigned)h[pl][5] << 16);
        o.w = h[pl][6] | ((unsigned)h[pl][7] << 16);
        out[(frag + pl) * 64 + lane] = o;
    }
}

void make_magic(unsigned d, unsigned (&dv)[2]) {
    if (d <= 1) { dv[0] = 0; dv[1] = 32; return; }
    unsigned k = 0;
    while ((1ull << k) < d) ++k;
    dv[0] = (unsigned)((((1ull << k) - d) << 32) / d + 1);
    dv[1] = k - 1;
}

int env_int(const char* name, int dflt) {
    const char* v = getenv(name);
    return v ? atoi(v) : dflt;
}

TileGeom pick_tile(int H, int W, int max_np, int pxb) {
    static const int force = env_int("POSEPIPE_SPLIT_TILE", -1);
    TileGeom best{};
    best.eff = -1.0;
    const int cand[4][2] = {{0, 0}, {0, 1}, {1, 0}, {2, 0}};
    const int nblk = 4 * pxb;
    for (int i = 0; i < 4; ++i) {
        if (force >= 0 && i != force) continue;
        TileGeom g{};
        g.bw_log2 = cand[i][0];
        g.gx_log2 = cand[i][1];
        const int BW = 32 >> g.bw_log2, BH = 1 << g.bw_log2, GX = 1 << g.gx_log2, GY = nblk / GX;
        g.TW = GX * BW;
        g.TH = GY * BH;
        g.PWp = g.TW + 2;
        if (g.bw_log2 == 2)
            while (g.PWp % 8 != 4) ++g.PWp;
        g.NP = (g.TH + 2) * g.PWp;
        g.NPp = g.NP;
        while (g.NPp % 8 != 4) ++g.NPp;
        g.tiles_x = (W + g.TW - 1) / g.TW;
        g.tiles_y = (H + g.TH - 1) / g.TH;
        if (g.NP > max_np) continue;
        g.eff = (double)H * W / ((double)g.tiles_x * g.tiles_y * 128.0 * pxb) - 1e-4 * g.NP / 256.0;
        if (g.eff > best.eff) best = g;
    }
    return best;
}

TileGeom pick_tile_s2(int H, int W, int max_np) {
    static const int force = env_int("POSEPIPE_SPLIT_TILE_S2", -1);
    TileGeom best{};
    best.eff = -1.0;
    const int cand[4][2] = {{0, 0}, {1, 0}, {2, 0}, {1, 1}};
    for (int i = 0; i < 4; ++i) {
        if (force >= 0 && i != force) continue;
        TileGeom g{};
        g.bw_log2 = cand[i][0];
        g.gx_log2 = cand[i][1];
        const int BW = 32 >> g.bw_log2, BH = 1 << g.bw_log2, GX = 1 << g.gx_log2, GY = 4 / GX;
        g.TW = GX * BW;
        g.TH = GY * BH;
        g.PWp = g.TW + 1;
        if (g.bw_log2 == 2)
            while (g.PWp % 8 != 4) ++g.PWp;
        g.NP = 4 * (g.TH + 1) * g.PWp;
        g.NPp = g.NP;
        while (g.NPp % 8 != 4) ++g.NPp;
        g.tiles_x = (W + g.TW - 1) / g.TW;
        g.tiles_y = (H + g.TH - 1) / g.TH;
        if (g.NP > max_np) continue;
        g.eff = (double)H * W / ((double)g.tiles_x * g.tiles_y * 128.0) - 0.05 * g.NP / 612.0;
        if (g.eff > best.eff) best = g;
    }
    return best;
}

struct StemArgs {
    const float* x;
    const uint4* w;
    const float* wscale;
    const float* bias;
    float* y;
    const unsigned* x_amax;
    unsigned* y_amax;
    int N, Hin, Win, xp_h, xp_w, Hout, Wout, y_pad, relu;
    int tiles_x, tiles_y, ntiles;
    unsigned dv_tx[2], dv_ty[2];
    unsigned x_bytes;
};
constexpr int STEM_TH = 16, STEM_TW = 32, STEM_PH = 2 * STEM_TH + 5, STEM_PW = 72, STEM_STEPS = 14;
constexpr int STEM_PLANE = STEM_PH * STEM_PW * 8, STEM_BUF = 2 * STEM_PLANE, STEM_WBYTES = STEM_STEPS * 2 * 2 * 1024;
constexpr int STEM_SLOTS = (STEM_PH * STEM_PW + 511) / 512;
constexpr int STEM_LDS = STEM_WBYTES + 2 * STEM_BUF + 256;

__global__ __launch_bounds__(512, 1) void conv_split_stem7_kernel(StemArgs a) {
    extern __shared__ __attribute__((aligned(16))) unsigned char smem[];
    unsigned char* const wl = smem;
    unsigned char* const pbase = smem + STEM_WBYTES;
    float* const red = reinterpret_cast<float*>(smem + STEM_WBYTES + 2 * STEM_BUF);
    const int tid = threadIdx.x, lane = tid & 63, wave = tid >> 6;
    const int px = lane & 31, hk = lane >> 5;

    for (int i = tid; i < STEM_WBYTES / 16; i += 512) reinterpret_cast<uint4*>(wl)[i] = a.w[i];

    const __amdgpu_buffer_rsrc_t xrsrc = __builtin_amdgcn_make_buffer_rsrc((void*)a.x, 0, (int)a.x_bytes, 0x00020000);
    float4 xr[STEM_SLOTS];
    int tn = 0, ty0 = 0, tx0 = 0;
    auto locate = [&](int t, int& n, int& y0, int& x0) {
        const unsigned q = pp_udiv((unsigned)t, a.dv_tx);
        x0 = (int)((unsigned)t - q * (unsigned)a.tiles_x) * STEM_TW;
        n = (int)pp_udiv(q, a.dv_ty);
        y0 = (int)(q - (unsigned)n * (unsigned)a.tiles_y) * STEM_TH;
    };
    auto load_patch = [&](int t) {
        locate(t, tn, ty0, tx0);
#pragma unroll
        for (int j = 0; j < STEM_SLOTS; ++j) {
            const int p = tid + 512 * j;
            const int pr = p / STEM_PW, pc = p - pr * STEM_PW;
            const int iy = 2 * ty0 - 3 + pr, ix = 2 * tx0 - 3 + pc;
            const bool ok = p < STEM_PH * STEM_PW && (unsigned)iy < (unsigned)a.Hin && (unsigned)ix < (unsigned)a.Win;
            const unsigned off = ok ? (unsigned)((tn * a.xp_h + iy) * a.xp_w + ix) * 16u : 0xffffffffu;
            xr[j] = __builtin_bit_cast(float4, __builtin_amdgcn_raw_buffer_load_b128(xrsrc, (int)off, 0, 0));
        }
    };
    auto store_patch = [&](int buf, float sx) {
#pragma unroll
        for (int j = 0; j < STEM_SLOTS; ++j) {
            const int p = tid + 512 * j;
            uint2 p0, p1;
            split4h(xr[j], sx, p0, p1);
            if (p >= STEM_PH * STEM_PW) continue;
            unsigned char* d = pbase + buf * STEM_BUF + p * 8;
            *reinterpret_cast<uint2*>(d) = p0;
            *reinterpret_cast<uint2*>(d + STEM_PLANE) = p1;
        }
    };

    const int xofs = ((4 * wave) * STEM_PW + 2 * px + 2 * hk) * 8;
    const unsigned char* const wlane = wl + lane * 16;
    const int rdrow = lane >> 3, rdc = lane & 7;
    float bias_l[2][4], wsc_l[2][4];
#pragma unroll
    for (int cb = 0; cb < 2; ++cb) {
        const float4 b = *reinterpret_cast<const float4*>(a.bias + cb * 32 + 4 * rdc);
        const float4 c = *reinterpret_cast<const float4*>(a.wscale + cb * 32 + 4 * rdc);
        bias_l[cb][0] = b.x; bias_l[cb][1] = b.y; bias_l[cb][2] = b.z; bias_l[cb][3] = b.w;
        wsc_l[cb][0] = c.x; wsc_l[cb][1] = c.y; wsc_l[cb][2] = c.z; wsc_l[cb][3] = c.w;
    }

    int t = blockIdx.x;
    if (t >= a.ntiles) return;
    load_patch(t);
    {
        const float sx = pp_act_scale(a.x_amax[tn]);
        store_patch(0, sx);
    }
    __syncthreads();
    int it = 0;
    for (; t < a.ntiles; t += gridDim.x, ++it) {
        const int buf = it & 1;
        int n, y0, x0;
        locate(t, n, y0, x0);
        const unsigned am = a.x_amax[n];
        const int tnext = t + (int)gridDim.x;
        const bool more = tnext < a.ntiles;
        unsigned am_next = 0;
        if (more) {
            load_patch(tnext);
            am_next = a.x_amax[tn];
        }
        f32x16 acc[2][2];
#pragma unroll
        for (int cb = 0; cb < 2; ++cb)
#pragma unroll
            for (int pb = 0; pb < 2; ++pb)
#pragma unroll
                for (int i = 0; i < 16; ++i) acc[cb][pb][i] = 0.f;
        const unsigned char* const pl = pbase + buf * STEM_BUF + xofs;
        uint4 wf[2][2][2], xf[2][2][2];
        auto load_frags = [&](int s, int set) {
#pragma unroll
            for (int cb = 0; cb < 2; ++cb)
#pragma unroll
                for (int pn = 0; pn < 2; ++pn) wf[set][cb][pn] = *reinterpret_cast<const uint4*>(wlane + ((s * 2 + cb) * 2 + pn) * 1024);
#pragma unroll
            for (int pb = 0; pb < 2; ++pb)
#pragma unroll
                for (int pn = 0; pn < 2; ++pn)
                    xf[set][pb][pn] = *reinterpret_cast<const uint4*>(pl + pn * STEM_PLANE + ((2 * pb + (s >> 1)) * STEM_PW + (s & 1) * 4) * 8);
        };
        load_frags(0, 0);
#pragma unroll
        for (int s = 0; s < STEM_STEPS; ++s) {
            if (s == STEM_STEPS / 2 && more) store_patch(buf ^ 1, pp_act_scale(am_next));
            if (s + 1 < STEM_STEPS) load_frags(s + 1, (s + 1) & 1);
            __builtin_amdgcn_sched_barrier(0);
            constexpr int WI[3] = {1, 0, 0}, XI[3] = {0, 1, 0};
#pragma unroll
            for (int p = 0; p < 3; ++p)
#pragma unroll
                for (int pb = 0; pb < 2; ++pb)
#pragma unroll
                    for (int cb = 0; cb < 2; ++cb)
                        acc[cb][pb] = __builtin_amdgcn_mfma_f32_32x32x16_f16(__builtin_bit_cast(f16x8, wf[s & 1][cb][WI[p]]),
                                                                             __builtin_bit_cast(f16x8, xf[s & 1][pb][XI[p]]), acc[cb][pb], 0, 0, 0);
            __builtin_amdgcn_sched_barrier(0);
        }
        __syncthreads();

        const float xinv = pp_act_unscale(am);
        unsigned char* const stg = pbase + buf * STEM_BUF + wave * 4096;
        float ymax = 0.f;
#pragma unroll
        for (int pb = 0; pb < 2; ++pb) {
            const int oy = y0 + 2 * wave + pb;
#pragma unroll
            for (int cb = 0; cb < 2; ++cb) {
#pragma unroll
                for (int g = 0; g < 4; ++g) {
                    const float4 v = make_float4(acc[cb][pb][4 * g], acc[cb][pb][4 * g + 1], acc[cb][pb][4 * g + 2], acc[cb][pb][4 * g + 3]);
                    *reinterpret_cast<float4*>(stg + px * 128 + (((2 * g + hk) ^ (px & 7)) << 4)) = v;
                }
                asm volatile("s_waitcnt lgkmcnt(0)" ::: "memory");
#pragma unroll
                for (int r4 = 0; r4 < 4; ++r4) {
                    const int r = r4 * 8 + rdrow, ox = x0 + r;
                    const float4 c = *reinterpret_cast<const float4*>(stg + r * 128 + ((rdc ^ (r & 7)) << 4));
                    float4 v = make_float4(__builtin_fmaf(c.x, wsc_l[cb][0] * xinv, bias_l[cb][0]), __builtin_fmaf(c.y, wsc_l[cb][1] * xinv, bias_l[cb][1]),
                                           __builtin_fmaf(c.z, wsc_l[cb][2] * xinv, bias_l[cb][2]), __builtin_fmaf(c.w, wsc_l[cb][3] * xinv, bias_l[cb][3]));
                    if (a.relu != PP_RELU_NONE) { v.x = fmaxf(v.x, 0.f); v.y = fmaxf(v.y, 0.f); v.z = fmaxf(v.z, 0.f); v.w = fmaxf(v.w, 0.f); }
                    if (oy < a.Hout && ox < a.Wout) {
                        *reinterpret_cast<float4*>(a.y + (((size_t)n * (a.Hout + a.y_pad) + oy) * (a.Wout + a.y_pad) + ox) * 64 + cb * 32 + 4 * rdc) = v;
                        ymax = fmaxf(ymax, pp_abs4max(v));
                    }
                }
                asm volatile("s_waitcnt lgkmcnt(0)" ::: "memory");
            }
        }
        if (a.y_amax) {
            const int img[1] = {n};
            const float m[1] = {ymax};
            pp_amax_commit_wg<8, 1>(a.y_amax, img, m, n, n, red);
        }
        __syncthreads();
    }
}

__global__ __launch_bounds__(256) void split_weights_stem7_kernel(const float* w, uint4* out, int CoutPad, const float* cmax) {
    const int i = blockIdx.x * 256 + threadIdx.x;
    if (i >= STEM_STEPS * 2 * 64) return;
    const int lane = i & 63, cb = (i >> 6) & 1, s = i >> 7;
    const int cout = cb * 32 + (lane & 31);
    unsigned short h[2][8];
#pragma unroll
    for (int j = 0; j < 8; ++j) {
        const int dy = s >> 1, dx = 4 * (s & 1) + 2 * (lane >> 5) + (j >> 2), c = j & 3;
        float v = 0.f;
        if (dx < 7) {
            const int k = (dy * 7 + dx) * 4 + c;
            v = w[((size_t)(k >> 5) * CoutPad + cout) * 32 + 8 * (k & 3) + ((k & 31) >> 2)];
        }
        unsigned short q2;
        split_weight_h(v, channel_scale(cmax[cout]), h[0][j], h[1][j], q2);
    }
#pragma unroll
    for (int pn = 0; pn < 2; ++pn) {
        uint4 o;
        o.x = h[pn][0] | ((unsigned)h[pn][1] << 16);
        o.y = h[pn][2] | ((unsigned)h[pn][3] << 16);
        o.z = h[pn][4] | ((unsigned)h[pn][5] << 16);
        o.w = h[pn][6] | ((unsigned)h[pn][7] << 16);
        out[(size_t)(((s * 2 + cb) * 2 + pn) * 64 + lane)] = o;
    }
}

}


static TileGeom tap_tiling(const ConvArgs& a, int nw, int stream_env) {
    const int max_np = nw == 8 ? 768 : 512, xp_h = a.Hin + a.x_pad, xp_w = a.Win + a.x_pad;
    TileGeom g = pick_tile(a.Hout, a.Wout, max_np, nw / 2);
    g.mode = MODE_TILE;
    const int snp = 64 * nw + 2 + 2 * xp_w;
    const double stream_eff = (double)a.Hout * a.Wout / ((double)xp_h * xp_w);
    bool use_stream = a.x_pad >= 1 && snp <= max_np && (g.eff < 0 || stream_eff > g.eff + 0.02);
    if (stream_env == 0 && g.eff >= 0) use_stream = false;
    if (stream_env == 1 && a.x_pad >= 1 && snp <= max_np) use_stream = true;
    if (use_stream) {
        g.mode = MODE_STREAM;
        g.PWp = xp_w;
        g.NP = g.NPp = snp;
        while (g.NPp % 8 != 4) ++g.NPp;
    }
    return g;
}

SplitPlan pp_conv_split_plan(const ConvArgs& a) {
    static const int stem7_on = env_int("POSEPIPE_SPLIT_STEM7", 1);
    static const int s2_on = env_int("POSEPIPE_SPLIT_S2", 1), s2p_on = env_int("POSEPIPE_SPLIT_S2P", 1);
    static const int gemm8_on = env_int("POSEPIPE_SPLIT_GEMM8", 1), gemm4_min_c = env_int("POSEPIPE_SPLIT_GEMM4_MIN_C", 64);
    static const int gemm_min_cin = env_int("POSEPIPE_SPLIT_GEMM_MIN_CIN", 1024);
    static const int c48_on = env_int("POSEPIPE_SPLIT_C48", 1), c48_mult = env_int("POSEPIPE_SPLIT_C48_MULT", 0);
    static const int stream_env = env_int("POSEPIPE_SPLIT_STREAM", -1);
    const char* s2_env = getenv("POSEPIPE_SPLIT_S2_MIN_CIN");
    SplitPlan p;
    p.f16 = a.split_f16 != 0;
    const size_t wpl = p.f16 ? 2 : 3;
    p.ncb = (a.Cout + 31) / 32;
    p.nout = p.ncb * 32;
    if (stem7_on && p.f16 && a.KH == 7 && a.KW == 7 && a.stride == 2 && a.pad_h == 3 && a.pad_w == 3 && a.dil_h == 1 && a.dil_w == 1 &&
        a.Cin == 4 && a.Cout == 64 && a.CoutPad >= 64 && a.up_log2 == 0 && !a.out_nchw && !a.res1 && !a.res2 &&
        (a.relu == PP_RELU_NONE || a.relu == PP_RELU_FIRST || a.relu == PP_RELU_LAST) && (a.y_stride == 0 || a.y_stride == a.Cout) &&
        a.y_coff == 0 && a.Hout == (a.Hin - 1) / 2 + 1 && a.Wout == (a.Win - 1) / 2 + 1) {
        p.kernel = SPLIT_STEM7;
        p.cin = a.Cin;
        p.frag_bytes = STEM_WBYTES;
        p.bytes = p.frag_bytes + (size_t)2 * p.nout * sizeof(float);
        return p;
    }
    const bool k3 = a.KH == 3 && a.KW == 3 && a.stride == 1 && a.pad_h == 1 && a.pad_w == 1 && a.dil_h == 1 && a.dil_w == 1 &&
                    a.Hout == a.Hin && a.Wout == a.Win;
    const bool k1 = a.KH == 1 && a.KW == 1 && a.pad_h == 0 && a.pad_w == 0;
    const bool full = a.KH == a.Hin && a.KW == a.Win && a.pad_h == 0 && a.pad_w == 0 && a.dil_h == 1 && a.dil_w == 1 &&
                      a.x_pad == 0 && a.Hout == 1 && a.Wout == 1 && !k1;
    const bool s2_pick = s2_env ? a.Cin >= atoi(s2_env) : p.f16 ? (a.Cin >= 96 || (a.Cin >= 48 && p.ncb >= 6)) : (a.Cin >= 128 && (p.ncb & 1) == 0);
    const bool s2_shape = a.KH == 3 && a.KW == 3 && a.stride == 2 && a.pad_h == 1 && a.pad_w == 1 && a.dil_h == 1 && a.dil_w == 1 && !full;
    const bool s2p_map = a.Hout * a.Wout >= 1500 || (a.Hout * a.Wout >= 400 && a.Cout >= 96);
    const bool s2p = s2p_on && p.f16 && s2_shape && s2p_map;
    const bool k3s2 = s2_on && s2_shape && (s2_pick || s2p);
    if (!(k3 || k1 || full || k3s2)) return p;
    p.taps = (k3 || k3s2) ? 9 : 1;
    p.cin = full ? a.K : a.Cin;
    const bool product = gemm8_on && p.taps == 1 && p.cin >= gemm4_min_c && a.Cout % 128 == 0;
    const bool one_column = p.f16 && p.cin >= 256 && a.Cout > 32 && a.Cout <= 64 && a.HWout >= 4096;
    if (p.taps == 1 && p.cin < gemm_min_cin && !one_column && !product) return p;
    const bool res1_plain = !a.res1 || (a.res1_off_w == 0 && a.res1_shift >= 0 && a.res1_shift <= 4 &&
                                        ((a.Hout - 1) >> a.res1_shift) < a.res1_H && ((a.Wout - 1) >> a.res1_shift) < a.res1_W &&
                                        (a.res1_shift > 0 || (a.res1_H == a.Hout && a.res1_W == a.Wout)));
    if (!(p.cin % 16 == 0 && a.Cout % 4 == 0 && a.up_log2 == 0 && !a.out_nchw && res1_plain && a.relu <= PP_ACT_SWISH &&
          (a.y_stride == 0 || a.y_stride == a.Cout) && a.y_coff == 0))
        return p;
    const bool c48 = c48_on && k3 && ((a.Cout > 32 && a.Cout <= 48) || (c48_mult == 1 && a.Cout % 48 == 0) || (c48_mult == 2 && a.Cout == 192));
    size_t steps = (size_t)(p.cin / 16) * p.taps;
    if (product) {
        p.kernel = SPLIT_PRODUCT;
    } else if (!k3 && !s2p) {
        p.kernel = p.taps > 1 ? SPLIT_TAP_GATHER : SPLIT_ONE_TAP;
        p.tile[0].mode = MODE_GEMM;
        p.tile[0].NP = 256;
        p.tile[0].NPp = 260;
    } else if (s2p) {
        p.kernel = SPLIT_S2P;
        p.tile[0] = pick_tile_s2(a.Hout, a.Wout, 13 * 64);
        p.tile[0].mode = MODE_TILE;
    } else if (c48) {
        p.kernel = SPLIT_C48;
        p.ncb = (a.Cout + 47) / 48 * 3;
        p.nout = p.ncb * 16;
        steps = (size_t)(p.cin / 16) * 5;
        p.tile[0] = tap_tiling(a, 4, stream_env);
    } else {
        p.kernel = SPLIT_TAP3;
        p.tile[0] = tap_tiling(a, 4, stream_env);
        p.tile[1] = tap_tiling(a, 8, stream_env);
    }
    p.frag_bytes = (steps + 1) * p.ncb * wpl * 64 * sizeof(uint4);
    p.bytes = p.frag_bytes + (p.f16 ? (size_t)2 * p.nout * sizeof(float) : 0);
    return p;
}

int pp_conv_split_weights(const SplitPlan& p, const ConvArgs& a, void* out, hipStream_t stream) {
    float* cmax = nullptr;
    if (p.f16) {
        float* inv_scale = reinterpret_cast<float*>(static_cast<unsigned char*>(out) + p.frag_bytes);
        cmax = inv_scale + p.nout;
        hipLaunchKernelGGL(weight_channel_max_kernel, dim3((unsigned)p.nout), dim3(64), 0, stream, a.w, a.Kpad / 32, a.CoutPad, p.nout, cmax, inv_scale);
    }
    const char* what = "split_weights";
    if (p.kernel == SPLIT_STEM7) {
        what = "split_weights_stem7";
        hipLaunchKernelGGL(split_weights_stem7_kernel, dim3((STEM_STEPS * 2 * 64 + 255) / 256), dim3(256), 0, stream, a.w, (uint4*)out, a.CoutPad, cmax);
    } else if (p.kernel == SPLIT_C48) {
        what = "split_weights48";
        const size_t total = (size_t)(p.cin / 16) * 5 * p.ncb * 64;
        const dim3 grid((unsigned)((total + 255) / 256));
        if (p.f16) hipLaunchKernelGGL(split_weights48_kernel<true>, grid, dim3(256), 0, stream, a.w, (uint4*)out, p.cin, a.CoutPad, p.ncb, total, cmax);
        else hipLaunchKernelGGL(split_weights48_kernel<false>, grid, dim3(256), 0, stream, a.w, (uint4*)out, p.cin, a.CoutPad, p.ncb, total, cmax);
    } else {
        const size_t total = (size_t)(p.cin / 16) * p.taps * p.ncb * 64;
        const dim3 grid((unsigned)((total + 255) / 256));
        if (p.f16) hipLaunchKernelGGL(split_weights_kernel<true>, grid, dim3(256), 0, stream, a.w, (uint4*)out, p.cin, p.taps, a.CoutPad, p.ncb, total, cmax);
        else hipLaunchKernelGGL(split_weights_kernel<false>, grid, dim3(256), 0, stream, a.w, (uint4*)out, p.cin, p.taps, a.CoutPad, p.ncb, total, cmax);
    }
    hipError_t e = hipGetLastError();
    if (e != hipSuccess) {
        pp_set_error("%s launch failed: %s", what, hipGetErrorString(e));
        return PP_ERR_HIP;
    }
    return PP_OK;
}

__global__ __launch_bounds__(256) void amax_kernel(const float4* x, size_t quads, unsigned per, unsigned* amax) {
    const unsigned n = blockIdx.x / per, part = blockIdx.x - n * per;
    const float4* xs = x + (size_t)n * quads;
    float m = 0.f;
    for (size_t i = (size_t)part * 256 + threadIdx.x; i < quads; i += (size_t)per * 256) m = fmaxf(m, pp_abs4max(xs[i]));
    __shared__ float red[16];
    const int im[1] = {(int)n};
    const float mm[1] = {m};
    pp_amax_commit_wg<4, 1>(amax, im, mm, (int)n, (int)n, red);
}

int pp_launch_amax(const float* x, int n, size_t elems, unsigned* amax, hipStream_t stream) {
    if (n <= 0 || elems == 0) return PP_OK;
    if (elems % 4 != 0) {
        pp_set_error("amax: %zu floats per sample (a multiple of 4 is required)", elems);
        return PP_ERR_ARG;
    }
    const size_t quads = elems / 4;
    const unsigned per = (unsigned)std::min<size_t>(std::max<size_t>((quads + 1023) / 1024, 1), std::max<size_t>(2048 / (size_t)n, 1));
    hipLaunchKernelGGL(amax_kernel, dim3(per * (unsigned)n), dim3(256), 0, stream, (const float4*)x, quads, per, amax);
    hipError_t e = hipGetLastError();
    if (e != hipSuccess) {
        pp_set_error("amax launch failed: %s", hipGetErrorString(e));
        return PP_ERR_HIP;
    }
    return PP_OK;
}

#ifdef PP_SPLIT_TIMELINE
static unsigned long long* tl_buf = nullptr;
static const size_t TL_MAX_WG = 1 << 19;
static unsigned long long* tl_begin(const ConvArgs& a, hipStream_t stream) {
    static const char* path = getenv("POSEPIPE_SPLIT_TIMELINE");
    static const int only_cin = env_int("POSEPIPE_SPLIT_TIMELINE_CIN", 0);
    static const int max_launches = env_int("POSEPIPE_SPLIT_TIMELINE_MAX", 300);
    static int recorded = 0;
    if (!path || (only_cin && a.Cin != only_cin) || recorded >= max_launches) return nullptr;
    ++recorded;
    if (!tl_buf && hipMalloc(&tl_buf, TL_MAX_WG * 128) != hipSuccess) return nullptr;
    (void)hipMemsetAsync(tl_buf, 0, TL_MAX_WG * 128, stream);
    return tl_buf;
}
static void tl_end(const ConvArgs& a, const SplitArgs& s, const char* kernel, unsigned nwg, hipStream_t stream) {
    if (!s.dbg) return;
    (void)hipStreamSynchronize(stream);
    nwg = std::min<unsigned>(nwg, TL_MAX_WG);
    std::vector<unsigned long long> h((size_t)nwg * 16);
    (void)hipMemcpy(h.data(), tl_buf, h.size() * 8, hipMemcpyDeviceToHost);
    static int launch = 0;
    FILE* f = fopen(getenv("POSEPIPE_SPLIT_TIMELINE"), "ab");
    if (!f) return;
    long long hdr[16] = {0x54494d454c494e45ll, launch++, (long long)nwg, a.N, a.Hout, a.Wout, a.Cin, a.Cout, s.mode, s.nchunks, s.gx, s.gy,
                         a.res1 != nullptr, a.res2 != nullptr, 0, 0};
    memcpy(&hdr[14], kernel, std::min<size_t>(strlen(kernel), 15));
    fwrite(hdr, 8, 16, f);
    fwrite(h.data(), 8, h.size(), f);
    fclose(f);
}
#define PP_TL_BEGIN() s.dbg = tl_begin(a, stream)
#define PP_TL_END(name, nwg) tl_end(a, s, name, nwg, stream)
#else
#define PP_TL_BEGIN()
#define PP_TL_END(name, nwg)
#endif

static void fill_divisors(SplitArgs& s) {
    const bool stream_mode = s.mode == MODE_STREAM;
    make_magic(stream_mode ? (unsigned)(s.xp_h * s.PWp) : (unsigned)(s.H * s.W), s.dv_per);
    make_magic(stream_mode ? (unsigned)s.PWp : (unsigned)s.W, s.dv_row);
    make_magic((unsigned)std::max(s.tiles_x, 1), s.dv_tx);
    make_magic((unsigned)std::max(s.tiles_y, 1), s.dv_ty);
    make_magic((unsigned)std::max(s.PWp, 1), s.dv_pw);
    make_magic((unsigned)std::max(s.gy, 1), s.dv_ncol);
    make_magic((unsigned)std::max(s.gx >> 3, 1), s.dv_run0);
    make_magic((unsigned)((s.gx >> 3) + 1), s.dv_run1);
    make_magic((unsigned)std::max(s.ktaps, 1), s.dv_ktaps);
    make_magic((unsigned)std::max(s.KW, 1), s.dv_kw);
}

template <auto K, int MAX_LDS, class Args>
static void launch_split(dim3 grid, unsigned threads, size_t lds, hipStream_t stream, const Args& s) {
    static PpPerDeviceOnce once;
    once.run([] { (void)hipFuncSetAttribute((const void*)K, hipFuncAttributeMaxDynamicSharedMemorySize, MAX_LDS); });
    hipLaunchKernelGGL(K, grid, dim3(threads), lds, stream, s);
}

template <int NS, int... MORE, class F>
static void with_nslot(int nslot, F&& f) {
    if constexpr (sizeof...(MORE) == 0) f(std::integral_constant<int, NS>());
    else if (nslot <= NS) f(std::integral_constant<int, NS>());
    else with_nslot<MORE...>(nslot, f);
}

template <int T, int NW, bool R4, int NS>
static void launch_tap(int cob, bool f16, dim3 grid, size_t lds, hipStream_t stream, const SplitArgs& s) {
    constexpr int L = (NW == 8 ? 160 : 100) * 1024;
    if constexpr (R4) {
        if (cob == 3) return launch_split<conv_split_kernel<9, NS, 3, 2, 4, true, true>, L>(grid, 256, lds, stream, s);
        if (cob == 4) return launch_split<conv_split_kernel<9, NS, 4, 2, 4, true, true>, L>(grid, 256, lds, stream, s);
    }
    if (f16 && cob == 2) launch_split<conv_split_kernel<T, NS, 2, 2, NW, R4, true>, L>(grid, 64 * NW, lds, stream, s);
    else if (f16) launch_split<conv_split_kernel<T, NS, 1, 2, NW, R4, true>, L>(grid, 64 * NW, lds, stream, s);
    else if (cob == 2) launch_split<conv_split_kernel<T, NS, 2, 2, NW, R4, false>, L>(grid, 64 * NW, lds, stream, s);
    else launch_split<conv_split_kernel<T, NS, 1, 2, NW, R4, false>, L>(grid, 64 * NW, lds, stream, s);
}

static unsigned apply_tiling(SplitArgs& s, const TileGeom& g, const ConvArgs& a, int nw) {
    s.mode = g.mode;
    s.NP = g.NP;
    s.NPp = g.NPp;
    if (g.mode == MODE_GEMM) {
        s.S = (long long)a.M;
        return (unsigned)((a.M + 255) / 256);
    }
    s.PWp = g.PWp;
    if (g.mode == MODE_STREAM) {
        s.S = (long long)a.N * s.xp_h * s.xp_w;
        return (unsigned)((s.S + 64 * nw - 1) / (64 * nw));
    }
    s.tiles_x = g.tiles_x; s.tiles_y = g.tiles_y; s.TH = g.TH; s.TW = g.TW; s.bw_log2 = g.bw_log2; s.gx_log2 = g.gx_log2;
    return (unsigned)(g.tiles_x * g.tiles_y * a.N);
}

static int launch_stem7(const ConvArgs& a, hipStream_t stream) {
    if (!a.x_amax) {
        pp_set_error("conv_split: the fp16 form needs the per-sample maximum of its input (ConvArgs::x_amax)");
        return PP_ERR_STATE;
    }
    StemArgs s{};
    s.x = a.x; s.w = (const uint4*)a.wsplit; s.bias = a.bias; s.y = a.y;
    s.wscale = reinterpret_cast<const float*>(static_cast<const unsigned char*>(a.wsplit) + STEM_WBYTES);
    s.x_amax = a.x_amax; s.y_amax = a.y_amax;
    s.N = a.N; s.Hin = a.Hin; s.Win = a.Win; s.xp_h = a.Hin + a.x_pad; s.xp_w = a.Win + a.x_pad;
    s.Hout = a.Hout; s.Wout = a.Wout; s.y_pad = a.y_pad; s.relu = a.relu;
    s.tiles_x = (a.Wout + STEM_TW - 1) / STEM_TW;
    s.tiles_y = (a.Hout + STEM_TH - 1) / STEM_TH;
    s.ntiles = a.N * s.tiles_x * s.tiles_y;
    s.x_bytes = a.x_bytes;
    make_magic((unsigned)s.tiles_x, s.dv_tx);
    make_magic((unsigned)s.tiles_y, s.dv_ty);
    static const int ncu = [] {
        int dev = 0, n = 256;
        if (hipGetDevice(&dev) == hipSuccess) (void)hipDeviceGetAttribute(&n, hipDeviceAttributeMultiprocessorCount, dev);
        return n > 0 ? n : 256;
    }();
    launch_split<conv_split_stem7_kernel, STEM_LDS>(dim3((unsigned)std::min(s.ntiles, ncu)), 512, STEM_LDS, stream, s);
    hipError_t e = hipGetLastError();
    if (e != hipSuccess) {
        pp_set_error("conv_split_stem7 launch failed: %s", hipGetErrorString(e));
        return PP_ERR_HIP;
    }
    return PP_OK;
}

int pp_launch_conv_split(const SplitPlan& p, const ConvArgs& a, hipStream_t stream) {
    if (a.wsplit && p.kernel == SPLIT_STEM7) return launch_stem7(a, stream);
    if (!a.wsplit || p.kernel == SPLIT_NONE) {
        pp_set_error("conv_split: layer not eligible");
        return PP_ERR_ARG;
    }
    static const int colmaj_mb = env_int("POSEPIPE_SPLIT_COLMAJOR_MB", 256), gemm_remap = env_int("POSEPIPE_SPLIT_GEMM_REMAP", 1);
    static const int epi_env = env_int("POSEPIPE_SPLIT_GEMM_EPI", 1);
    static const int cob2_env = env_int("POSEPIPE_SPLIT_S2_COB", 0), cob_env = env_int("POSEPIPE_SPLIT_COB", 0);
    static const int nw8_f16 = env_int("POSEPIPE_SPLIT_NW8_F16", 0);
    static const int nw8_min_blocks = env_int("POSEPIPE_SPLIT_NW8_MIN_BLOCKS", 512), nw8_min_chunks = env_int("POSEPIPE_SPLIT_NW8_MIN_CHUNKS", 16);
    static const int ring4_env = env_int("POSEPIPE_SPLIT_RING4", 1), ring48_env = env_int("POSEPIPE_SPLIT_RING48", 1);
    const bool full = p.cin != a.Cin;
    SplitArgs s{};
    s.x = a.x; s.w = (const uint4*)a.wsplit; s.bias = a.bias; s.res1 = a.res1; s.res2 = a.res2; s.y = a.y;
    s.N = a.N; s.H = a.Hout; s.W = a.Wout; s.Cin = p.cin; s.Cout = a.Cout;
    s.ncb = p.ncb;
    s.xp_h = full ? 1 : a.Hin + a.x_pad;
    s.xp_w = full ? 1 : a.Win + a.x_pad;
    s.stride = a.stride;
    s.y_pad = a.y_pad; s.r1_pad = a.r1_pad; s.r2_pad = a.r2_pad; s.relu = a.relu;
    s.r1_shift = a.res1 ? a.res1_shift : 0;
    s.r1_H = a.res1 ? a.res1_H : a.Hout;
    s.r1_W = a.res1 ? a.res1_W : a.Wout;
    s.nchunks = p.cin / 16;
    s.ktaps = 1; s.KW = a.KW; s.pad = a.pad_h; s.Hin = a.Hin; s.Win = a.Win;
    if (p.kernel == SPLIT_TAP_GATHER) {
        s.ktaps = p.taps;
        s.nchunks = (p.cin / 16) * p.taps;
    }
    s.x_bytes = a.x_bytes;
    s.xcd_remap = a.xcd_remap;
    const bool f16 = p.f16 != 0;
    const int xp = f16 ? 2 : 3;
    const int wpl = f16 ? 2 : 3;
    s.wscale = f16 ? reinterpret_cast<const float*>(static_cast<const unsigned char*>(a.wsplit) + p.frag_bytes) : nullptr;
    s.x_amax = a.x_amax;
    s.y_amax = a.y_amax;
    if (f16 && !a.x_amax) {
        pp_set_error("conv_split: the fp16 form needs the per-sample maximum of its input (ConvArgs::x_amax)");
        return PP_ERR_STATE;
    }
    PP_TL_BEGIN();
    s.col_major = (size_t)a.x_bytes <= (size_t)colmaj_mb << 20;
    const char* tag;
    dim3 grid;
    if (p.kernel == SPLIT_PRODUCT) {
        s.mode = MODE_GEMM;
        s.S = (long long)a.M;
        s.col_major = 0;
        const int BM = 256, BN = 128;
        grid = dim3((unsigned)((a.M + BM - 1) / BM), (unsigned)(a.Cout / BN));
        s.gx = (int)grid.x; s.gy = (int)grid.y;
        s.xcd_remap = gemm_remap && s.gy > 1;
        if (s.xcd_remap) grid = dim3((unsigned)((s.gx + 7) / 8 * 8 * s.gy), 1);
        const int epi_knob = g_split_gemm_epi.load(std::memory_order_relaxed);
        s.epi_lds = epi_knob >= 0 ? epi_knob : epi_env;
        const int nwave = 4;
        fill_divisors(s);
        const size_t lds_loop = f16 ? (size_t)3 * BM * 64 + (size_t)3 * BN * 2 * wpl * 16 : (size_t)2 * (xp * 2 * (BM + 4) * 16 + BN * 2 * wpl * 16);
        const size_t lds = std::max<size_t>(lds_loop, s.epi_lds ? (size_t)nwave * (16384 + 2048) : 0);
        if (f16) launch_split<conv_split_gemm_kernel<2, 2, true>, 80 * 1024>(grid, 256, lds, stream, s);
        else launch_split<conv_split_gemm_kernel<2, 2, false>, 80 * 1024>(grid, 256, lds, stream, s);
        tag = "g256x128";
    } else if (p.kernel == SPLIT_S2P) {
        if (p.tile[0].eff < 0) {
            pp_set_error("conv_split: no strided-patch tile for a %dx%d map", a.Hout, a.Wout);
            return PP_ERR_STATE;
        }
        const unsigned gx = apply_tiling(s, p.tile[0], a, 4);
        s.SP = (s.TH + 1) * s.PWp;
        int cob = 1;
        for (int c : {4, 3, 2})
            if (s.ncb % c == 0 && (size_t)2 * 2 * s.NPp * 16 + (size_t)4 * c * 2 * 1024 <= 80 * 1024 && (cob2_env == 0 || cob2_env == c)) {
                cob = c;
                break;
            }
        grid = dim3(gx, (unsigned)(s.ncb / cob));
        s.gx = (int)grid.x; s.gy = (int)grid.y;
        if (s.xcd_remap) grid = dim3((unsigned)((s.gx + 7) / 8 * 8 * s.gy), 1);
        fill_divisors(s);
        make_magic((unsigned)s.SP, s.dv_row);
        const size_t lds = (size_t)2 * 2 * s.NPp * 16 + (size_t)4 * cob * 2 * 1024;
        with_nslot<10, 11, 13>((s.NP + 63) / 64, [&](auto ns) {
            constexpr int NS = decltype(ns)::value, L = 100 * 1024;
            if (cob == 4) launch_split<conv_split_kernel<9, NS, 4, 1, 4, true, true, true>, L>(grid, 256, lds, stream, s);
            else if (cob == 3) launch_split<conv_split_kernel<9, NS, 3, 1, 4, true, true, true>, L>(grid, 256, lds, stream, s);
            else if (cob == 2) launch_split<conv_split_kernel<9, NS, 2, 1, 4, true, true, true>, L>(grid, 256, lds, stream, s);
            else launch_split<conv_split_kernel<9, NS, 1, 1, 4, true, true, true>, L>(grid, 256, lds, stream, s);
        });
        tag = "s2p";
    } else if (p.kernel == SPLIT_C48) {
        const unsigned gx = apply_tiling(s, p.tile[0], a, 4);
        s.gx = (int)gx;
        s.gy = s.ncb / 3;
        grid = s.xcd_remap ? dim3((unsigned)((s.gx + 7) / 8 * 8 * s.gy), 1) : dim3(gx, (unsigned)s.gy);
        fill_divisors(s);
        const size_t patch48 = (size_t)2 * xp * 2 * s.NPp * 16;
        const bool ring48 = f16 && ring48_env && patch48 + (size_t)4 * 3 * wpl * 1024 <= 80 * 1024;
        const size_t lds = patch48 + (ring48 ? (size_t)4 * 3 * wpl * 1024 : 0);
        with_nslot<5, 6, 7, 8>((s.NP + 63) / 64, [&](auto ns) {
            constexpr int NS = decltype(ns)::value, L = 100 * 1024;
            if (ring48) launch_split<conv_split48_kernel<NS, true, true>, L>(grid, 256, lds, stream, s);
            else if (f16) launch_split<conv_split48_kernel<NS, true, false>, L>(grid, 256, lds, stream, s);
            else launch_split<conv_split48_kernel<NS, false, false>, L>(grid, 256, lds, stream, s);
        });
        tag = "c48";
    } else {
        const bool tap3 = p.kernel == SPLIT_TAP3;
        int cob = (s.ncb & 1) ? 1 : 2;
        if (tap3 && f16 && s.ncb % 3 == 0 && (cob_env == 0 || cob_env == 3)) cob = 3;
        else if (tap3 && f16 && s.ncb % 4 == 0 && (cob_env == 0 || cob_env == 4)) cob = 4;
        int nw = tap3 && (!f16 || nw8_f16) ? 8 : 4;
        unsigned gx = apply_tiling(s, p.tile[nw == 8], a, nw);
        if (nw == 8 && !((long)gx * (s.ncb / cob) >= nw8_min_blocks && s.nchunks >= nw8_min_chunks)) {
            nw = 4;
            gx = apply_tiling(s, p.tile[0], a, nw);
        }
        const int nslot = (s.NP + 16 * nw - 1) / (16 * nw);
        const auto ring_fits = [&](int c) {
            return ring4_env && nw == 4 && s.mode != MODE_GEMM && (size_t)xp * 2 * s.NPp * 16 + (size_t)4 * c * wpl * 1024 <= 80 * 1024;
        };
        if (cob >= 3 && !(ring_fits(cob) && (cob_env >= 3 || (long)gx * (s.ncb / cob) >= 400))) cob = (s.ncb & 1) ? 1 : 2;
        const bool ring = ring_fits(cob);
        grid = dim3(gx, (unsigned)(s.ncb / cob));
        s.gx = (int)grid.x; s.gy = (int)grid.y;
        if (s.xcd_remap) grid = dim3((unsigned)((s.gx + 7) / 8 * 8 * s.gy), 1);
        const size_t lds = (size_t)(ring ? 1 : 2) * xp * 2 * s.NPp * 16 + ((nw == 8 || ring) ? (size_t)4 * cob * wpl * 1024 : 0);
        fill_divisors(s);
        if (s.mode == MODE_GEMM) launch_tap<1, 4, false, 4>(cob, f16, grid, lds, stream, s);
        else if (nw == 8) with_nslot<5, 6>(nslot, [&](auto ns) { launch_tap<9, 8, false, decltype(ns)::value>(cob, f16, grid, lds, stream, s); });
        else if (ring) with_nslot<5, 6, 7, 8>(nslot, [&](auto ns) { launch_tap<9, 4, true, decltype(ns)::value>(cob, f16, grid, lds, stream, s); });
        else with_nslot<5, 6, 7, 8>(nslot, [&](auto ns) { launch_tap<9, 4, false, decltype(ns)::value>(cob, f16, grid, lds, stream, s); });
        tag = s.mode == MODE_GEMM ? "gemm4" : nw == 8 ? "nw8" : ring ? "ring4" : "nw4";
    }
    PP_TL_END(tag, grid.x * grid.y);
    hipError_t e = hipGetLastError();
    if (e != hipSuccess) {
        pp_set_error("conv_split (%s) launch failed: %s", tag, hipGetErrorString(e));
        return PP_ERR_HIP;
    }
    return PP_OK;
}
```

### posepipeline_amd/csrc/crop_affine.hip

```cpp
#include <cmath>

#include "pp_internal.h"

namespace {

__device__ __forceinline__ int sat_round_i32(double v) {
    double r = rint(v);
    if (r > 2147483647.0) return 2147483647;
    if (r < -2147483648.0) return (int)0x80000000;
    return (int)r;
}

__device__ __forceinline__ int sat_short(int v) { return v < -32768 ? -32768 : (v > 32767 ? 32767 : v); }

__global__ __launch_bounds__(256) void crop_affine_kernel(const uint8_t* __restrict__ frames, int H, int W,
                                                          const PersonXform* __restrict__ xf, int n_person,
                                                          int out_w, int out_h, const float* __restrict__ lut,
                                                          int cm0, int cm1, int cm2, int flip,
                                                          float* __restrict__ out, uint8_t* __restrict__ crop_u8) {
    __shared__ float s_lut[3 * 256];
    for (int i = threadIdx.x; i < 768; i += blockDim.x) s_lut[i] = lut[i];
    __syncthreads();
    const int person = blockIdx.y;
    const PersonXform t = xf[person];
    const int npix = out_w * out_h;
    const size_t sample = (size_t)npix * 4;
    float* o0 = out + (size_t)person * sample;
    float* o1 = out + (size_t)(n_person + person) * sample;
    const uint8_t* img = frames + (size_t)t.frame * H * W * 3;
    for (int p = blockIdx.x * blockDim.x + threadIdx.x; p < npix; p += gridDim.x * blockDim.x) {
        const int y = p / out_w;
        const int x = p - y * out_w;
        float4 v = make_float4(0.f, 0.f, 0.f, 0.f);
        uint8_t c3[3] = {0, 0, 0};
        if (t.valid) {
            const int adelta = sat_round_i32(__dmul_rn(__dmul_rn(t.a00, (double)x), 1024.0));
            const int bdelta = sat_round_i32(__dmul_rn(__dmul_rn(t.a10, (double)x), 1024.0));
            const int X0 = sat_round_i32(__dmul_rn(__dadd_rn(__dmul_rn(t.a01, (double)y), t.b0), 1024.0)) + 16;
            const int Y0 = sat_round_i32(__dmul_rn(__dadd_rn(__dmul_rn(t.a11, (double)y), t.b1), 1024.0)) + 16;
            const int X = (X0 + adelta) >> 5;
            const int Y = (Y0 + bdelta) >> 5;
            const int sx = sat_short(X >> 5), sy = sat_short(Y >> 5);
            const int fx = X & 31, fy = Y & 31;
            const int w00 = (32 - fx) * (32 - fy), w01 = fx * (32 - fy), w10 = (32 - fx) * fy, w11 = fx * fy;
            const bool x0in = (unsigned)sx < (unsigned)W, x1in = (unsigned)(sx + 1) < (unsigned)W;
            const bool y0in = (unsigned)sy < (unsigned)H, y1in = (unsigned)(sy + 1) < (unsigned)H;
            const uint8_t* r0 = img + ((size_t)sy * W + sx) * 3;
            const uint8_t* r1 = r0 + (size_t)W * 3;
#pragma unroll
            for (int c = 0; c < 3; ++c) {
                const int p00 = (y0in && x0in) ? r0[c] : 0;
                const int p01 = (y0in && x1in) ? r0[3 + c] : 0;
                const int p10 = (y1in && x0in) ? r1[c] : 0;
                const int p11 = (y1in && x1in) ? r1[3 + c] : 0;
                c3[c] = (uint8_t)(((p00 * w00 + p01 * w01 + p10 * w10 + p11 * w11) * 32 + 16384) >> 15);
            }
            v.x = s_lut[0 * 256 + c3[cm0]];
            v.y = s_lut[1 * 256 + c3[cm1]];
            v.z = s_lut[2 * 256 + c3[cm2]];
        }
        *reinterpret_cast<float4*>(o0 + (size_t)p * 4) = v;
        if (flip) *reinterpret_cast<float4*>(o1 + ((size_t)y * out_w + (out_w - 1 - x)) * 4) = v;
        if (crop_u8) {
            uint8_t* cp = crop_u8 + ((size_t)person * npix + p) * 3;
            cp[0] = c3[0]; cp[1] = c3[1]; cp[2] = c3[2];
        }
    }
}

__global__ __launch_bounds__(256) void flip_w_kernel(const float4* __restrict__ src, float4* __restrict__ dst,
                                                     size_t rows, int w) {
    const size_t total = rows * w;
    for (size_t i = blockIdx.x * (size_t)blockDim.x + threadIdx.x; i < total; i += (size_t)gridDim.x * blockDim.x) {
        const size_t r = i / w;
        const int x = (int)(i - r * w);
        dst[r * w + (w - 1 - x)] = src[i];
    }
}

bool solve6(double A[6][6], double b[6], double x[6]) {
    const int n = 6;
    for (int i = 0; i < n; ++i) {
        int k = i;
        for (int j = i + 1; j < n; ++j)
            if (std::fabs(A[j][i]) > std::fabs(A[k][i])) k = j;
        if (std::fabs(A[k][i]) < 2.220446049250313e-16 * 100) return false;
        if (k != i) {
            for (int j = i; j < n; ++j) std::swap(A[i][j], A[k][j]);
            std::swap(b[i], b[k]);
        }
        const double d = -1.0 / A[i][i];
        for (int j = i + 1; j < n; ++j) {
            const double alpha = A[j][i] * d;
            for (int c = i + 1; c < n; ++c) A[j][c] += alpha * A[i][c];
            b[j] += alpha * b[i];
        }
    }
    for (int i = n - 1; i >= 0; --i) {
        double s = b[i];
        for (int c = i + 1; c < n; ++c) s -= A[i][c] * x[c];
        x[i] = s / A[i][i];
    }
    return true;
}

}

bool pp_person_transform(const double* bb, int out_w, int out_h, float cs[4], PersonXform* t, int udp) {
    t->valid = 0;
    cs[0] = cs[1] = cs[2] = cs[3] = 0.f;
    if (std::isnan(bb[0]) || std::isnan(bb[1]) || std::isnan(bb[2]) || std::isnan(bb[3])) return false;
    double x = bb[0], y = bb[1], w = bb[2], h = bb[3];
    const double aspect = (double)out_w / (double)out_h;
    const float cx = (float)(x + w * 0.5), cy = (float)(y + h * 0.5);
    if (w > aspect * h) h = w * 1.0 / aspect;
    else if (w < aspect * h) w = h * aspect;
    float sx = (float)(w / 200.0), sy = (float)(h / 200.0);
    sx = sx * 1.25f;
    sy = sy * 1.25f;
    cs[0] = cx; cs[1] = cy; cs[2] = sx; cs[3] = sy;
    double M[6];
    if (udp) {
        const float in_x = cx * 2.0f, in_y = cy * 2.0f, tg_x = sx * 200.0f, tg_y = sy * 200.0f;
        const double scale_x = ((double)out_w - 1.0) / (double)tg_x, scale_y = ((double)out_h - 1.0) / (double)tg_y;
        M[0] = (double)(float)(1.0 * scale_x);
        M[1] = (double)(float)(-0.0 * scale_x);
        M[2] = (double)(float)(scale_x * (-0.5 * (double)in_x * 1.0 + 0.5 * (double)in_y * 0.0 + 0.5 * (double)tg_x));
        M[3] = (double)(float)(0.0 * scale_y);
        M[4] = (double)(float)(1.0 * scale_y);
        M[5] = (double)(float)(scale_y * (-0.5 * (double)in_x * 0.0 - 0.5 * (double)in_y * 1.0 + 0.5 * (double)tg_y));
        if (!(std::isfinite(M[0]) && std::isfinite(M[4]) && std::isfinite(M[2]) && std::isfinite(M[5])))
            for (double& m : M) m = 0.0;
    } else {
    const float src_w = sx * 200.0f;
    const float s0x = cx, s0y = cy;
    const float s1x = (float)((double)cx + 0.0);
    const float s1y = (float)((double)cy + (double)src_w * -0.5);
    const float d0 = s0x - s1x, d1 = s0y - s1y;
    const float s2x = s1x + (-d1), s2y = s1y + d0;
    const float dst_w = (float)out_w, dst_h = (float)out_h;
    const float t0x = (float)(dst_w * 0.5), t0y = (float)(dst_h * 0.5);
    const float t1x = t0x, t1y = (float)((double)t0y + (double)dst_w * -0.5);
    const float e0 = t0x - t1x, e1 = t0y - t1y;
    const float t2x = t1x + (-e1), t2y = t1y + e0;
    const float sp[3][2] = {{s0x, s0y}, {s1x, s1y}, {s2x, s2y}};
    const float dp[3][2] = {{t0x, t0y}, {t1x, t1y}, {t2x, t2y}};
    double A[6][6] = {}, b[6];
    for (int i = 0; i < 3; ++i) {
        A[2 * i][0] = sp[i][0]; A[2 * i][1] = sp[i][1]; A[2 * i][2] = 1.0;
        A[2 * i + 1][3] = sp[i][0]; A[2 * i + 1][4] = sp[i][1]; A[2 * i + 1][5] = 1.0;
        b[2 * i] = dp[i][0]; b[2 * i + 1] = dp[i][1];
    }
    if (!solve6(A, b, M)) {
        for (double& m : M) m = 0.0;
    }
    }
    double D = M[0] * M[4] - M[1] * M[3];
    D = D != 0 ? 1.0 / D : 0;
    const double A11 = M[4] * D, A22 = M[0] * D;
    M[0] = A11; M[1] *= -D; M[3] *= -D; M[4] = A22;
    const double b1 = -M[0] * M[2] - M[1] * M[5];
    const double b2 = -M[3] * M[2] - M[4] * M[5];
    t->a00 = M[0]; t->a01 = M[1]; t->b0 = b1;
    t->a10 = M[3]; t->a11 = M[4]; t->b1 = b2;
    t->valid = 1;
    return true;
}

int pp_enqueue_crop(hipStream_t s, const uint8_t* frames, int h, int w, const PersonXform* xf, int n_person,
                    int out_w, int out_h, const float* lut, const int32_t chan_map[3], int flip, float* out,
                    uint8_t* crop_u8) {
    if (n_person <= 0) return PP_OK;
    const int npix = out_w * out_h;
    dim3 grid(std::min((npix + 255) / 256, 64), n_person);
    hipLaunchKernelGGL(crop_affine_kernel, grid, dim3(256), 0, s, frames, h, w, xf, n_person, out_w, out_h, lut,
                       chan_map[0], chan_map[1], chan_map[2], flip, out, crop_u8);
    PP_HIP_CHECK(hipGetLastError());
    return PP_OK;
}

int pp_enqueue_flip_w(hipStream_t s, const float* src, float* dst, int n, int h, int w) {
    const size_t rows = (size_t)n * h;
    if (rows == 0) return PP_OK;
    const int blocks = (int)std::min<size_t>((rows * w + 255) / 256, 2048);
    hipLaunchKernelGGL(flip_w_kernel, dim3(blocks), dim3(256), 0, s, reinterpret_cast<const float4*>(src),
                       reinterpret_cast<float4*>(dst), rows, w);
    PP_HIP_CHECK(hipGetLastError());
    return PP_OK;
}

extern "C" int pp_crop_affine_normalize(pp_ctx* ctx, const uint8_t* frames, int n_frames, int h, int w,
                                        const int32_t* frame_idx, const double* bbox_tlwh, int n_person,
                                        int out_w, int out_h, const float* lut, const int32_t* chan_map,
                                        int flip, float* out, float* center_scale, uint8_t* crop_u8,
                                        int32_t* valid, int mem) {
    PP_REQUIRE(ctx && frames && frame_idx && bbox_tlwh && lut && chan_map && out, "pp_crop_affine_normalize: NULL argument");
    PP_REQUIRE(n_frames > 0 && h > 0 && w > 0 && out_w > 0 && out_h > 0, "pp_crop_affine_normalize: empty dims");
    if (n_person <= 0) return PP_OK;
    for (int c = 0; c < 3; ++c) PP_REQUIRE(chan_map[c] >= 0 && chan_map[c] < 3, "chan_map[%d] out of range", c);
    std::vector<PersonXform> xf(n_person);
    const int udp = (flip >> 1) & 1;
    flip &= 1;
    for (int i = 0; i < n_person; ++i) {
        PP_REQUIRE(frame_idx[i] >= 0 && frame_idx[i] < n_frames, "frame_idx[%d]=%d out of range", i, frame_idx[i]);
        float cs[4];
        pp_person_transform(bbox_tlwh + 4 * i, out_w, out_h, cs, &xf[i], udp);
        xf[i].frame = frame_idx[i];
        if (center_scale) memcpy(center_scale + 4 * i, cs, sizeof(cs));
        if (valid) valid[i] = xf[i].valid;
    }
    const size_t frames_b = (size_t)n_frames * h * w * 3;
    const size_t n_out = (size_t)n_person * (flip ? 2 : 1);
    const size_t out_e = n_out * out_w * out_h * 4;
    const size_t crop_b = crop_u8 ? (size_t)n_person * out_w * out_h * 3 : 0;
    size_t need = ScratchCursor::align(n_person * sizeof(PersonXform)) + ScratchCursor::align(768 * sizeof(float));
    if (mem == PP_MEM_HOST) need += ScratchCursor::align(frames_b) + ScratchCursor::align(out_e * 4) + ScratchCursor::align(crop_b);
    int rc = ctx->ensure_scratch(need);
    if (rc != PP_OK) return rc;
    ScratchCursor cur(ctx);
    hipStream_t s = ctx->stream;
    PersonXform* dxf = cur.take<PersonXform>(n_person);
    float* dlut = cur.take<float>(768);
    PP_HIP_CHECK(hipMemcpyAsync(dxf, xf.data(), n_person * sizeof(PersonXform), hipMemcpyHostToDevice, s));
    PP_HIP_CHECK(hipMemcpyAsync(dlut, lut, 768 * sizeof(float), hipMemcpyHostToDevice, s));
    const uint8_t* dframes = frames;
    float* dout = out;
    uint8_t* dcrop = crop_u8;
    if (mem == PP_MEM_HOST) {
        uint8_t* df = cur.take<uint8_t>(frames_b);
        PP_HIP_CHECK(hipMemcpyAsync(df, frames, frames_b, hipMemcpyHostToDevice, s));
        dframes = df;
        dout = cur.take<float>(out_e);
        if (crop_u8) dcrop = cur.take<uint8_t>(crop_b);
    }
    rc = pp_enqueue_crop(s, dframes, h, w, dxf, n_person, out_w, out_h, dlut, chan_map, flip, dout, dcrop);
    if (rc != PP_OK) return rc;
    if (mem == PP_MEM_HOST) {
        PP_HIP_CHECK(hipMemcpyAsync(out, dout, out_e * 4, hipMemcpyDeviceToHost, s));
        if (crop_u8) PP_HIP_CHECK(hipMemcpyAsync(crop_u8, dcrop, crop_b, hipMemcpyDeviceToHost, s));
    }
    PP_HIP_CHECK(hipStreamSynchronize(s));
    return PP_OK;
}
```

### posepipeline_amd/csrc/pp_internal.h

```cpp
#pragma once
#include <hip/hip_runtime.h>
#include <cstdarg>
#include <cstdio>
#include <cstring>
#include <string>
#include <vector>
#include <mutex>

#include "posepipe_hip.h"

void pp_set_error(const char* fmt, ...);

#define PP_HIP_CHECK(expr)                                                              \
    do {                                                                                \
        hipError_t _e = (expr);                                                         \
        if (_e != hipSuccess) {                                                         \
            pp_set_error("%s failed: %s (%s:%d)", #expr, hipGetErrorString(_e), __FILE__, \
                         __LINE__);                                                     \
            return PP_ERR_HIP;                                                          \
        }                                                                               \
    } while (0)

#define PP_REQUIRE(cond, ...)            \
    do {                                 \
        if (!(cond)) {                   \
            pp_set_error(__VA_ARGS__);   \
            return PP_ERR_ARG;           \
        }                                \
    } while (0)

struct PpPerDeviceOnce {
    std::mutex m;
    unsigned long long done = 0;
    template <class F> void run(F&& f) {
        int dev = 0;
        (void)hipGetDevice(&dev);
        std::lock_guard<std::mutex> g(m);
        if ((done >> (dev & 63)) & 1ull) return;
        f();
        done |= 1ull << (dev & 63);
    }
};

struct pp_ctx {
    int device = 0;
    hipStream_t stream = nullptr;
    bool own_stream = true;
    hipEvent_t ev_start = nullptr, ev_stop = nullptr;
    hipStream_t copy_stream = nullptr;
    hipEvent_t ev_upload = nullptr;
    hipEvent_t ev_consumed = nullptr;
    void* scratch = nullptr;
    size_t scratch_bytes = 0;
    int ensure_scratch(size_t bytes);
};

struct ScratchCursor {
    pp_ctx* ctx;
    size_t off = 0;
    explicit ScratchCursor(pp_ctx* c) : ctx(c) {}
    static size_t align(size_t b) { return (b + 255) & ~size_t(255); }
    template <class T>
    T* take(size_t count) {
        T* p = reinterpret_cast<T*>(static_cast<char*>(ctx->scratch) + off);
        off += align(count * sizeof(T));
        return p;
    }
};

void pp_range_push(const char* name);
void pp_range_pop();
struct PpRange {
    explicit PpRange(const char* name) { pp_range_push(name); }
    ~PpRange() { pp_range_pop(); }
    PpRange(const PpRange&) = delete;
    PpRange& operator=(const PpRange&) = delete;
};
struct PpStages {
    bool open = false;
    void next(const char* name) {
        if (open) pp_range_pop();
        open = name != nullptr;
        if (open) pp_range_push(name);
    }
    ~PpStages() { next(nullptr); }
};

struct ConvArgs {
    const float* x;
    const float* w;
    const float* bias;
    const float* res1;
    const float* res2;
    float* y;
    int N, Hin, Win, Cin, Hout, Wout, Cout, CoutPad;
    int KH, KW, stride, pad_h, pad_w, dil_h, dil_w;
    int K, Kpad, M, HWout;
    unsigned div_hw_m, div_hw_s1, div_hw_s2, div_w_m, div_w_s1, div_w_s2;
    unsigned div_c_m, div_c_s1, div_c_s2, div_kw_m, div_kw_s1, div_kw_s2;
    int xcd_remap;
    unsigned x_bytes;
    int relu, up_log2, out_nchw;
    int res1_shift, res1_off_w, res1_H, res1_W;
    int y_stride, y_coff;
    const uint2* tap_table;
    int x_pad, y_pad, r1_pad, r2_pad;
    int no_bounds;
    const void* wsplit;
    int numerics;
    int split_f16;
    const unsigned* x_amax;
    unsigned* y_amax;
};
struct TileGeom {
    int TH, TW, bw_log2, gx_log2, PWp, NP, NPp, tiles_x, tiles_y;
    double eff;
    int mode;
};
enum SplitKernel {
    SPLIT_NONE = 0,
    SPLIT_STEM7,
    SPLIT_PRODUCT,
    SPLIT_C48,
    SPLIT_TAP3,
    SPLIT_S2P,
    SPLIT_ONE_TAP,
    SPLIT_TAP_GATHER,
};
struct SplitPlan {
    int kernel = SPLIT_NONE;
    int f16 = 0;
    int taps = 1, cin = 0;
    int ncb = 0;
    int nout = 0;
    size_t frag_bytes = 0;
    size_t bytes = 0;
    TileGeom tile[2] = {};
    long long off = -1;
};
SplitPlan pp_conv_split_plan(const ConvArgs& a);
int pp_conv_split_weights(const SplitPlan& p, const ConvArgs& a, void* out, hipStream_t stream);
int pp_launch_conv_split(const SplitPlan& p, const ConvArgs& a, hipStream_t stream);
bool pp_conv_tracks_amax(const ConvArgs& a, bool split);
bool pp_conv_split_enabled();
bool pp_conv_split_f16_default();
int pp_conv_prepare(const ConvArgs& a);
int pp_conv_out_dim(int in, int k, int stride, int pad, int dil);
int pp_launch_conv(const ConvArgs& a, const SplitPlan* plan, hipStream_t stream);
int pp_launch_conv_p3(const ConvArgs& a, int ct, int pt, hipStream_t stream, bool fake_addresses = false);

struct PoolArgs {
    const float* x;
    float* y;
    int N, Hin, Win, C, Hout, Wout, KH, KW, stride, pad_h, pad_w;
    int x_stride, x_coff, y_stride, y_coff;
};
int pp_launch_maxpool(const PoolArgs& a, hipStream_t stream);
int pp_launch_avgpool(const float* x, float* y, int n, int hin, int win, int c, int kh, int kw, int stride, hipStream_t stream);

struct GemmArgs {
    const void* A;
    const void* B;
    const float* bias;
    const float* res;
    void* C;
    int M, N, K;
    int act;
    int out_bf16;
    int res_mod;
    int group_m;
    int qkv_tokens, qkv_hd;
};
int pp_launch_gemm_bf16(const GemmArgs& a, hipStream_t stream);
int pp_gemm_bf16_prepare();
struct pp_deconv_bf16;
int pp_deconv_bf16_create(const float* weights, const float* bias, int h, int w, int cin, int cout, int max_batch,
                          hipStream_t stream, pp_deconv_bf16** out);
void pp_deconv_bf16_destroy(pp_deconv_bf16* d);
int pp_deconv_bf16_run(pp_deconv_bf16* d, const float* x, float* out, int batch, int relu, hipStream_t stream);
int pp_launch_f32_to_bf16(const float* x, void* y, size_t n, hipStream_t stream);
int pp_launch_nv12_to_bgr(const unsigned char* nv12, unsigned char* bgr, int frames, int h, int w, hipStream_t stream);
int pp_launch_layernorm(const float* x, const float* pos, int pos_mod, float* x_out, const float* gamma,
                        const float* beta, int rows, int dim, float eps, void* y, int out_bf16, hipStream_t stream);
int pp_launch_attention(const void* qkv, int batch, int tokens, int heads, int head_dim, void* out, hipStream_t stream,
                        int head_major = 0);
int pp_launch_depth_to_space(const float* x, float* y, int n, int h, int w, int c, hipStream_t stream);
int pp_launch_upsample_add(const float* t, const float* res1, const float* res2, float* y, int n, int H, int W, int c,
                           int up_log2, int relu, hipStream_t stream, const float* t2 = nullptr, int up2 = 0,
                           const float* t3 = nullptr, int up3 = 0, unsigned* y_amax = nullptr);
struct pp_vit_encoder;
size_t pp_vit_param_floats(int tokens, int dim, int depth, int hidden);
int pp_vit_encoder_create(const float* params, int tokens, int dim, int depth, int heads, int hidden, int max_batch,
                          hipStream_t stream, pp_vit_encoder** out);
void pp_vit_encoder_destroy(pp_vit_encoder* e);
int pp_vit_encoder_run(pp_vit_encoder* e, const float* in, float* out, int batch, hipStream_t stream);
void pp_vit_encoder_set_timing(pp_vit_encoder* e, int enable);
int pp_vit_encoder_get_timing(pp_vit_encoder* e, float ms3[3], int* n_gemm);

struct PersonXform {
    double a00, a01, b0, a10, a11, b1;
    int frame;
    int valid;
};
bool pp_person_transform(const double* bbox_tlwh, int out_w, int out_h, float center_scale[4], PersonXform* t, int udp = 0);
int pp_enqueue_crop(hipStream_t s, const uint8_t* frames, int h, int w, const PersonXform* xf, int n_person,
                    int out_w, int out_h, const float* lut, const int32_t chan_map[3], int flip, float* out,
                    uint8_t* crop_u8);
int pp_enqueue_flip_w(hipStream_t s, const float* src, float* dst, int n, int h, int w);

struct DecodeParams {
    int n, k, h, w;
    int shift_heatmap, post, blur_kernel;
};
int pp_enqueue_decode(hipStream_t s, const DecodeParams& p, const float* hm, const float* hm_flip,
                      const int32_t* flip_perm, const float* center_scale, float* kpts, float* merged);
```

### posepipeline_amd/csrc/topdown.hip

```cpp
#include <memory>

#include "pp_internal.h"

struct pp_topdown {
    pp_ctx* ctx = nullptr;
    pp_net* net = nullptr;
    int in_buf = 0, out_buf = 0;
    int in_h = 0, in_w = 0, hm_h = 0, hm_w = 0, k = 0;
    int flip = 0, shift_heatmap = 0, post = 0, blur_kernel = 0;
    int32_t chan_map[3] = {0, 1, 2};
    int max_person = 0;
    float* d_lut = nullptr;
    int32_t* d_perm = nullptr;
    PersonXform* d_xf = nullptr;
    float* d_cs = nullptr;
    float* d_kpts = nullptr;
    uint8_t* d_frames = nullptr;
    size_t d_frames_bytes = 0;
    PersonXform* h_xf = nullptr;
    float* h_cs = nullptr;
    hipEvent_t ev[4] = {nullptr, nullptr, nullptr, nullptr};
};

int pp_net_dims(pp_net* net, int buf, int* h, int* w, int* c);
int pp_net_max_batch(pp_net* net);
pp_ctx* pp_net_ctx(pp_net* net);

extern "C" void pp_topdown_destroy(pp_topdown* t);

extern "C" {

int pp_topdown_create(pp_net* net, int in_buf, int out_buf, int num_joints, const int32_t* flip_perm,
                      int shift_heatmap, int post, int blur_kernel, const float* lut, const int32_t* chan_map,
                      pp_topdown** out) {
    PP_REQUIRE(net && lut && chan_map && out, "pp_topdown_create: NULL argument");
    *out = nullptr;
    std::unique_ptr<pp_topdown, void (*)(pp_topdown*)> t(new pp_topdown(), pp_topdown_destroy);
    t->net = net;
    t->ctx = pp_net_ctx(net);
    int c = 0, oc = 0;
    PP_REQUIRE(pp_net_dims(net, in_buf, &t->in_h, &t->in_w, &c) == PP_OK && c == 4,
               "pp_topdown_create: input buffer must be NHWC with 4 channels");
    PP_REQUIRE(pp_net_dims(net, out_buf, &t->hm_h, &t->hm_w, &oc) == PP_OK && oc == num_joints,
               "pp_topdown_create: output buffer has %d channels, expected %d", oc, num_joints);
    t->in_buf = in_buf; t->out_buf = out_buf; t->k = num_joints;
    t->flip = flip_perm != nullptr; t->shift_heatmap = shift_heatmap; t->post = post; t->blur_kernel = blur_kernel;
    for (int i = 0; i < 3; ++i) {
        PP_REQUIRE(chan_map[i] >= 0 && chan_map[i] < 3, "chan_map[%d] out of range", i);
        t->chan_map[i] = chan_map[i];
    }
    t->max_person = pp_net_max_batch(net) / (t->flip ? 2 : 1);
    PP_REQUIRE(t->max_person > 0, "pp_topdown_create: net max_batch too small");
    hipStream_t s = t->ctx->stream;
    PP_HIP_CHECK(hipSetDevice(t->ctx->device));
    PP_HIP_CHECK(hipMalloc((void**)&t->d_lut, 768 * sizeof(float)));
    PP_HIP_CHECK(hipMemcpyAsync(t->d_lut, lut, 768 * sizeof(float), hipMemcpyHostToDevice, s));
    if (flip_perm) {
        for (int i = 0; i < num_joints; ++i)
            PP_REQUIRE(flip_perm[i] >= 0 && flip_perm[i] < num_joints, "flip_perm[%d] out of range", i);
        PP_HIP_CHECK(hipMalloc((void**)&t->d_perm, num_joints * sizeof(int32_t)));
        PP_HIP_CHECK(hipMemcpyAsync(t->d_perm, flip_perm, num_joints * sizeof(int32_t), hipMemcpyHostToDevice, s));
    }
    PP_HIP_CHECK(hipMalloc((void**)&t->d_xf, t->max_person * sizeof(PersonXform)));
    PP_HIP_CHECK(hipMalloc((void**)&t->d_cs, t->max_person * 4 * sizeof(float)));
    PP_HIP_CHECK(hipMalloc((void**)&t->d_kpts, (size_t)t->max_person * num_joints * 3 * sizeof(float)));
    PP_HIP_CHECK(hipHostMalloc((void**)&t->h_xf, t->max_person * sizeof(PersonXform), hipHostMallocDefault));
    PP_HIP_CHECK(hipHostMalloc((void**)&t->h_cs, t->max_person * 4 * sizeof(float), hipHostMallocDefault));
    for (auto& e : t->ev) PP_HIP_CHECK(hipEventCreate(&e));
    PP_HIP_CHECK(hipStreamSynchronize(s));
    *out = t.release();
    return PP_OK;
}

void pp_topdown_destroy(pp_topdown* t) {
    if (!t) return;
    if (t->ctx && t->ctx->stream) (void)hipStreamSynchronize(t->ctx->stream);
    if (t->d_lut) (void)hipFree(t->d_lut);
    if (t->d_perm) (void)hipFree(t->d_perm);
    if (t->d_xf) (void)hipFree(t->d_xf);
    if (t->d_cs) (void)hipFree(t->d_cs);
    if (t->d_kpts) (void)hipFree(t->d_kpts);
    if (t->d_frames) (void)hipFree(t->d_frames);
    if (t->h_xf) (void)hipHostFree(t->h_xf);
    if (t->h_cs) (void)hipHostFree(t->h_cs);
    for (auto& e : t->ev)
        if (e) (void)hipEventDestroy(e);
    delete t;
}

static int topdown_tail(pp_topdown* t, int n_person, float* kpts, int kpts_mem, bool check_valid) {
    hipStream_t s = t->ctx->stream;
    const int batch = n_person * (t->flip ? 2 : 1);
    PP_HIP_CHECK(hipEventRecord(t->ev[1], s));
    PpStages stage;
    stage.next("topdown.backbone_program");
    int rc = pp_net_run(t->net, batch, 0, -1);
    if (rc != PP_OK) return rc;
    PP_HIP_CHECK(hipEventRecord(t->ev[2], s));
    stage.next("topdown.flip_merge_decode");
    void* hm_ptr = nullptr;
    size_t hm_bytes = 0;
    rc = pp_net_buffer(t->net, t->out_buf, &hm_ptr, &hm_bytes);
    if (rc != PP_OK) return rc;
    const float* hm = static_cast<const float*>(hm_ptr);
    const float* hm_flip = t->flip ? hm + (size_t)n_person * (hm_bytes / sizeof(float)) : nullptr;
    const DecodeParams dp{n_person, t->k, t->hm_h, t->hm_w, t->shift_heatmap, t->post, t->blur_kernel};
    float* dk = kpts_mem == PP_MEM_DEVICE ? kpts : t->d_kpts;
    rc = pp_enqueue_decode(s, dp, hm, hm_flip, t->d_perm, t->d_cs, dk, nullptr);
    if (rc != PP_OK) return rc;
    PP_HIP_CHECK(hipEventRecord(t->ev[3], s));
    if (check_valid) {
        const size_t row = (size_t)t->k * 3;
        for (int i = 0; i < n_person; ++i)
            if (!t->h_xf[i].valid) PP_HIP_CHECK(hipMemsetAsync(dk + (size_t)i * row, 0, row * sizeof(float), s));
    }
    if (kpts_mem == PP_MEM_HOST) {
        PP_HIP_CHECK(hipMemcpyAsync(kpts, dk, (size_t)n_person * t->k * 3 * sizeof(float), hipMemcpyDeviceToHost, s));
    }
    PP_HIP_CHECK(hipStreamSynchronize(s));
    return PP_OK;
}

int pp_topdown_run(pp_topdown* t, const uint8_t* frames, int n_frames, int h, int w, int frames_mem,
                   const int32_t* frame_idx, const double* bbox_tlwh, int n_person, float* kpts, int kpts_mem,
                   int32_t* valid) {
    PP_REQUIRE(t && frames && frame_idx && bbox_tlwh && kpts, "pp_topdown_run: NULL argument");
    PP_REQUIRE(n_person >= 0 && n_person <= t->max_person, "pp_topdown_run: n_person %d exceeds capacity %d", n_person,
               t->max_person);
    if (n_person == 0) return PP_OK;
    hipStream_t s = t->ctx->stream;
    for (int i = 0; i < n_person; ++i) {
        PP_REQUIRE(frame_idx[i] >= 0 && frame_idx[i] < n_frames, "frame_idx[%d]=%d out of range", i, frame_idx[i]);
        pp_person_transform(bbox_tlwh + 4 * i, t->in_w, t->in_h, t->h_cs + 4 * i, &t->h_xf[i], t->post == 2);
        t->h_xf[i].frame = frame_idx[i];
        if (valid) valid[i] = t->h_xf[i].valid;
    }
    PP_HIP_CHECK(hipEventRecord(t->ev[0], s));
    PP_HIP_CHECK(hipMemcpyAsync(t->d_xf, t->h_xf, n_person * sizeof(PersonXform), hipMemcpyHostToDevice, s));
    PP_HIP_CHECK(hipMemcpyAsync(t->d_cs, t->h_cs, n_person * 4 * sizeof(float), hipMemcpyHostToDevice, s));
    const uint8_t* dframes = frames;
    if (frames_mem == PP_MEM_HOST) {
        const size_t bytes = (size_t)n_frames * h * w * 3;
        if (bytes > t->d_frames_bytes) {
            if (t->d_frames) PP_HIP_CHECK(hipFree(t->d_frames));
            t->d_frames = nullptr;
            PP_HIP_CHECK(hipMalloc((void**)&t->d_frames, bytes));
            t->d_frames_bytes = bytes;
        }
        PP_HIP_CHECK(hipMemcpyAsync(t->d_frames, frames, bytes, hipMemcpyHostToDevice, s));
        dframes = t->d_frames;
    }
    void* in_ptr = nullptr;
    int rc = pp_net_buffer(t->net, t->in_buf, &in_ptr, nullptr);
    if (rc != PP_OK) return rc;
    rc = pp_enqueue_crop(s, dframes, h, w, t->d_xf, n_person, t->in_w, t->in_h, t->d_lut, t->chan_map, t->flip,
                         static_cast<float*>(in_ptr), nullptr);
    if (rc != PP_OK) return rc;
    return topdown_tail(t, n_person, kpts, kpts_mem, true);
}

int pp_topdown_run_precropped(pp_topdown* t, const float* x_nhwc4, int x_mem, const float* center_scale,
                              int n_person, float* kpts, int kpts_mem) {
    PP_REQUIRE(t && x_nhwc4 && center_scale && kpts, "pp_topdown_run_precropped: NULL argument");
    PP_REQUIRE(n_person >= 0 && n_person <= t->max_person, "pp_topdown_run_precropped: n_person %d exceeds capacity %d",
               n_person, t->max_person);
    if (n_person == 0) return PP_OK;
    hipStream_t s = t->ctx->stream;
    void* in_ptr = nullptr;
    size_t in_bytes = 0;
    int rc = pp_net_buffer(t->net, t->in_buf, &in_ptr, &in_bytes);
    if (rc != PP_OK) return rc;
    float* din = static_cast<float*>(in_ptr);
    PP_HIP_CHECK(hipEventRecord(t->ev[0], s));
    if (x_nhwc4 != din) {
        PP_HIP_CHECK(hipMemcpyAsync(din, x_nhwc4, (size_t)n_person * in_bytes,
                                    x_mem == PP_MEM_HOST ? hipMemcpyHostToDevice : hipMemcpyDeviceToDevice, s));
    }
    memcpy(t->h_cs, center_scale, (size_t)n_person * 4 * sizeof(float));
    PP_HIP_CHECK(hipMemcpyAsync(t->d_cs, t->h_cs, n_person * 4 * sizeof(float), hipMemcpyHostToDevice, s));
    if (t->flip) {
        rc = pp_enqueue_flip_w(s, din, din + (size_t)n_person * (in_bytes / sizeof(float)), n_person, t->in_h, t->in_w);
        if (rc != PP_OK) return rc;
    }
    return topdown_tail(t, n_person, kpts, kpts_mem, false);
}

int pp_topdown_timing(pp_topdown* t, float* ms3) {
    PP_REQUIRE(t && ms3, "pp_topdown_timing: NULL argument");
    for (int i = 0; i < 3; ++i) PP_HIP_CHECK(hipEventElapsedTime(&ms3[i], t->ev[i], t->ev[i + 1]));
    return PP_OK;
}

}
```

Before: 614.1.

## Fuse stem conv with following max-pool and compute amax in crop and pool kernels

Adds a pooled epilogue to the split stem7 conv kernel so the 3x3/s2 max-pool runs inside the conv launch, skipping the write and re-read of the full-resolution stem map. Max-pool and crop kernels now also compute per-sample absolute maxima, so separate amax passes over their outputs are not needed. The maxpool grid is reworked into contiguous chunks to support this. This adds tile halo overlap, more LDS, new planning and invalidation logic, and new ways for graph capture or op-range runs to misbehave.

```diff
diff --git a/posepipeline_amd/csrc/api_core.hip b/posepipeline_amd/csrc/api_core.hip
--- a/posepipeline_amd/csrc/api_core.hip
+++ b/posepipeline_amd/csrc/api_core.hip
@@ -279,6 +279,8 @@
     std::vector<hipEvent_t> op_done;
     hipEvent_t fork_ev = nullptr;
     std::vector<hipEvent_t> join_ev;
+    std::vector<int> fuse_pool, fused_into;
+    std::vector<char> stem_stale;
     std::vector<pp_vit_encoder*> vits;
     std::vector<pp_deconv_bf16*> deconvs;
 
@@ -301,6 +303,7 @@
     auto tracks = [&](int i) {
         const pp_op& op = net->ops[i];
         if (op.type == PP_OP_UPSAMPLE_ADD) return true;
+        if (op.type == PP_OP_MAXPOOL) return net->bufs[op.out].h * net->bufs[op.out].w >= 64;
         return op.type == PP_OP_CONV && pp_conv_tracks_amax(net_conv_args(net, op, 1), is_h(i));
     };
     {
@@ -354,7 +357,8 @@
         {
             int covered = 0;
             const int out_b = net->ops[t.producers.front()].out;
-            for (int p : t.producers) covered += net->ops[p].type == PP_OP_CONV ? net->ops[p].cout : net->bufs[out_b].c;
+            for (int p : t.producers)
+                covered += net->ops[p].type == PP_OP_CONV || net->ops[p].type == PP_OP_MAXPOOL ? net->ops[p].cout : net->bufs[out_b].c;
             if (covered < net->bufs[out_b].c) fused = false;
         }
         if (fused)
@@ -363,6 +367,41 @@
             net->op_post_slot[t.producers.back()] = t.slot;
     }
     for (const auto& r : readers) net->op_x_slot[r.first] = tensors[r.second].slot;
+}
+
+static void net_plan_fuse(pp_net* net) {
+    const int n = (int)net->ops.size();
+    net->fuse_pool.assign(n, -1);
+    net->fused_into.assign(n, -1);
+    net->stem_stale.assign(n, 0);
+    const char* env = getenv("POSEPIPE_FUSE_STEM_POOL");
+    if ((env && atoi(env) == 0) || net->numerics != PP_NET_NUMERICS_SPLIT || !net->split_f16) return;
+    for (int i = 0; i < n; ++i) {
+        const pp_op& c = net->ops[i];
+        if (c.type != PP_OP_CONV || net->split_plan[i].kernel != SPLIT_STEM7) continue;
+        int reader = -1, readers = 0;
+        for (int j = i + 1; j < n; ++j) {
+            const pp_op& o = net->ops[j];
+            for (int b : {o.in, o.res1, o.res2, o.in2, o.in3})
+                if (b == c.out) { reader = j; ++readers; }
+            if (o.out == c.out) break;
+        }
+        if (readers != 1) continue;
+        const pp_op& o = net->ops[reader];
+        const pp_buf& bo = net->bufs[o.out];
+        if (o.type != PP_OP_MAXPOOL || o.in != c.out || o.out == c.out || o.kh != 3 || o.kw != 3 || o.stride != 2 || o.pad_h != 1 || o.pad_w != 1 ||
+            o.pad_end != 0 || o.in_c_off != 0 || o.cin != 64 || net->bufs[c.out].c != 64 || o.out_c_off + 64 > bo.c)
+            continue;
+        if (const int ps = net->op_post_slot[reader]; ps >= 0 && (net->slot_first[ps] != reader || o.out_c_off != 0 || bo.c != 64)) continue;
+        bool between = false;
+        for (int j = i + 1; j < reader; ++j) {
+            const pp_op& m = net->ops[j];
+            for (int b : {m.in, m.out, m.res1, m.res2, m.in2, m.in3}) between = between || b == o.out;
+        }
+        if (between) continue;
+        net->fuse_pool[i] = reader;
+        net->fused_into[reader] = i;
+    }
 }
 
 static int net_reset_amax(pp_net* net, int first, int last, int batch, hipStream_t s) {
@@ -567,8 +606,28 @@
 
 static int net_launch_op_body(pp_net* net, const pp_op& op, int batch, hipStream_t s);
 
-static int net_launch_op(pp_net* net, const pp_op& op, int batch, hipStream_t s) {
+static int net_launch_stem_pool(pp_net* net, int conv, int pool, int batch, hipStream_t s) {
+    const pp_op& po = net->ops[pool];
+    const pp_buf& bo = net->bufs[po.out];
+    ConvArgs a = net_conv_args(net, net->ops[conv], batch);
+    a.y = net->buf_ptr(po.out);
+    a.y_pad = bo.pad; a.y_stride = bo.c; a.y_coff = po.out_c_off;
+    a.pool_h = bo.h; a.pool_w = bo.w;
+    a.y_amax = net->amax_slot(net->op_y_slot[pool] >= 0 ? net->op_y_slot[pool] : net->op_post_slot[pool]);
+    return pp_launch_conv(a, &net->split_plan[conv], s);
+}
+
+static int net_launch_op(pp_net* net, const pp_op& op, int batch, hipStream_t s, int first, int last) {
     const size_t idx = &op - net->ops.data();
+    if (const int pool = net->fuse_pool[idx]; pool >= 0) {
+        net->stem_stale[pool] = pool < last;
+        if (pool < last) return net_launch_stem_pool(net, (int)idx, pool, batch, s);
+    }
+    if (const int conv = net->fused_into[idx]; conv >= 0) {
+        if (conv >= first) return PP_OK;
+        PP_REQUIRE(!net->stem_stale[idx], "pp_net_run: op range [%d, %d) starts between the stem (op %d) and its max-pool (op %d), which last ran as one "
+                   "launch: the pool's input was not written; run both ops, or the stem on its own first", first, last, conv, (int)idx);
+    }
     int rc = net_launch_op_body(net, op, batch, s);
     if (rc == PP_OK && net->amax && net->op_post_slot[idx] >= 0)
         rc = pp_launch_amax(net->buf_ptr(op.out), batch, net->buf_elems[op.out], net->amax_slot(net->op_post_slot[idx]), s);
@@ -587,6 +646,7 @@
         p.N = batch; p.Hin = bi.h; p.Win = bi.w; p.C = op.cin; p.Hout = bo.h; p.Wout = bo.w;
         p.x_stride = bi.c; p.x_coff = op.in_c_off; p.y_stride = bo.c; p.y_coff = op.out_c_off;
         p.KH = op.kh; p.KW = op.kw; p.stride = op.stride; p.pad_h = op.pad_h; p.pad_w = op.pad_w;
+        p.y_amax = net->amax ? net->amax_slot(net->op_y_slot[&op - net->ops.data()]) : nullptr;
         return pp_launch_maxpool(p, s);
     } else if (op.type == PP_OP_AVGPOOL) {
         return pp_launch_avgpool(net->buf_ptr(op.in), net->buf_ptr(op.out), batch, bi.h, bi.w, op.cin, op.kh, op.kw, op.stride, s);
@@ -706,6 +766,9 @@
         }
     }
     net->split_plan.assign(n_ops, SplitPlan());
+    net->fuse_pool.assign(n_ops, -1);
+    net->fused_into.assign(n_ops, -1);
+    net->stem_stale.assign(n_ops, 0);
     if (net->numerics == PP_NET_NUMERICS_SPLIT) {
         size_t bytes = 0;
         for (int i = 0; i < n_ops; ++i) {
@@ -717,6 +780,7 @@
             net->split_plan[i] = p;
         }
         net_plan_amax(net.get());
+        net_plan_fuse(net.get());
         if (!net->slot_owner.empty()) {
             const size_t ab = net->slot_owner.size() * (size_t)max_batch * sizeof(unsigned);
             PP_HIP_CHECK(hipMalloc((void**)&net->amax, ab));
@@ -820,6 +884,16 @@
 int pp_net_buffer(pp_net* net, int buf, void** dptr, size_t* bytes_per_sample) {
     PP_REQUIRE(net && buf >= 0 && buf < (int)net->bufs.size(), "pp_net_buffer: bad buffer id");
     PP_REQUIRE(net->bufs[buf].pad == 0, "pp_net_buffer: buffer %d has a zero halo (conv-internal layout); expose dense buffers only", buf);
+    for (size_t i = 0; i < net->ops.size(); ++i)
+        if (net->fuse_pool[i] >= 0 && net->ops[i].out == buf) {
+            PP_HIP_CHECK(hipStreamSynchronize(net->ctx->stream));
+            if (net->graph_exec) {
+                PP_HIP_CHECK(hipGraphExecDestroy(net->graph_exec));
+                net->graph_exec = nullptr;
+            }
+            net->fused_into[net->fuse_pool[i]] = -1;
+            net->fuse_pool[i] = -1;
+        }
     if (dptr) *dptr = net->buf_ptr(buf);
     if (bytes_per_sample) *bytes_per_sample = net->buf_elems[buf] * sizeof(float);
     return PP_OK;
@@ -842,7 +916,7 @@
     }
     if (net->lanes.empty() || !net->use_lanes || last_op - first_op < 8) {
         for (int i = first_op; i < last_op; ++i) {
-            int rc = net_launch_op(net, net->ops[i], batch, main);
+            int rc = net_launch_op(net, net->ops[i], batch, main, first_op, last_op);
             if (rc != PP_OK) return rc;
         }
         return PP_OK;
@@ -853,7 +927,7 @@
         hipStream_t s = net->lanes[net->op_lane[i]];
         for (int d : net->op_waits[i])
             if (d >= first_op) PP_HIP_CHECK(hipStreamWaitEvent(s, net->op_done[d], 0));
-        int rc = net_launch_op(net, net->ops[i], batch, s);
+        int rc = net_launch_op(net, net->ops[i], batch, s, first_op, last_op);
         if (rc != PP_OK) return rc;
         if (net->op_needs_event[i]) PP_HIP_CHECK(hipEventRecord(net->op_done[i], s));
     }
@@ -910,7 +984,7 @@
     hipGraph_t graph = nullptr;
     PP_HIP_CHECK(hipStreamBeginCapture(s, hipStreamCaptureModeThreadLocal));
     int rc = net_reset_amax(net, 0, (int)net->ops.size(), batch, s);
-    for (size_t i = 0; i < net->ops.size() && rc == PP_OK; ++i) rc = net_launch_op(net, net->ops[i], batch, s);
+    for (size_t i = 0; i < net->ops.size() && rc == PP_OK; ++i) rc = net_launch_op(net, net->ops[i], batch, s, 0, (int)net->ops.size());
     hipError_t e = hipStreamEndCapture(s, &graph);
     if (rc != PP_OK) {
         if (graph) (void)hipGraphDestroy(graph);
@@ -952,7 +1026,7 @@
     int rc = net_reset_amax(net, 0, (int)n, batch, s);
     PP_HIP_CHECK(hipEventRecord(ev[0], s));
     for (size_t i = 0; i < n && rc == PP_OK; ++i) {
-        rc = net_launch_op(net, net->ops[i], batch, s);
+        rc = net_launch_op(net, net->ops[i], batch, s, 0, (int)n);
         if (rc == PP_OK && hipEventRecord(ev[i + 1], s) != hipSuccess) rc = PP_ERR_HIP;
     }
     if (rc == PP_OK && hipStreamSynchronize(s) != hipSuccess) rc = PP_ERR_HIP;
diff --git a/posepipeline_amd/csrc/conv_igemm.hip b/posepipeline_amd/csrc/conv_igemm.hip
--- a/posepipeline_amd/csrc/conv_igemm.hip
+++ b/posepipeline_amd/csrc/conv_igemm.hip
@@ -408,11 +408,14 @@
     return pt >= 2 ? launch_t<CT, 2>(a, stream) : launch_t<CT, 1>(a, stream);
 }
 
-__global__ __launch_bounds__(256) void maxpool_kernel(PoolArgs a) {
+__global__ __launch_bounds__(256) void maxpool_kernel(PoolArgs a, size_t total, size_t chunk) {
     const int c4n = a.C >> 2;
     const size_t xs = a.x_stride ? a.x_stride : a.C, ys = a.y_stride ? a.y_stride : a.C;
-    const size_t total = (size_t)a.N * a.Hout * a.Wout * c4n;
-    for (size_t i = blockIdx.x * (size_t)blockDim.x + threadIdx.x; i < total; i += (size_t)gridDim.x * blockDim.x) {
+    const size_t per = (size_t)a.Hout * a.Wout * c4n;
+    const size_t b0 = blockIdx.x * chunk, b1 = b0 + chunk < total ? b0 + chunk : total;
+    const int img_first = (int)(b0 / per);
+    float ym[2] = {0.f, 0.f};
+    for (size_t i = b0 + threadIdx.x; i < b1; i += 256) {
         const int c4 = i % c4n;
         size_t p = i / c4n;
         const int wo = p % a.Wout;
@@ -432,6 +435,19 @@
             }
         }
         *reinterpret_cast<float4*>(a.y + (((size_t)n * a.Hout + ho) * a.Wout + wo) * ys + a.y_coff + 4 * c4) = m;
+        if (a.y_amax) {
+            const float am = pp_abs4max(m);
+            const int d = n - img_first;
+            if (d == 0) ym[0] = fmaxf(ym[0], am);
+            else if (d == 1) ym[1] = fmaxf(ym[1], am);
+            else if (am > 0.f) atomicMax(a.y_amax + n, __float_as_uint(am));
+        }
+    }
+    if (a.y_amax) {
+        __shared__ float red[16];
+        const int img_last = (int)((b1 - 1) / per);
+        const int im[2] = {img_first, img_first + 1};
+        pp_amax_commit_wg<4, 2>(a.y_amax, im, ym, img_first, img_last > img_first ? img_first + 1 : img_first, red);
     }
 }
 
@@ -644,7 +660,8 @@
     }
     if ((size_t)a.N * img_bytes > max_bytes) {
         const int per = (int)(max_bytes / img_bytes);
-        const size_t y_img = (size_t)((a.Hout << a.up_log2) + a.y_pad) * ((a.Wout << a.up_log2) + a.y_pad) * (a.y_stride ? a.y_stride : a.Cout);
+        const size_t y_img = (size_t)((a.pool_h > 0 ? a.pool_h : a.Hout << a.up_log2) + a.y_pad) * ((a.pool_h > 0 ? a.pool_w : a.Wout << a.up_log2) + a.y_pad) *
+                             (a.y_stride ? a.y_stride : a.Cout);
         const size_t r1_img = (size_t)(a.res1_H + a.r1_pad) * (a.res1_W + a.r1_pad) * a.Cout;
         const size_t r2_img = (size_t)((a.Hout << a.up_log2) + a.r2_pad) * ((a.Wout << a.up_log2) + a.r2_pad) * a.Cout;
         for (int n0 = 0; n0 < a.N; n0 += per) {
@@ -664,6 +681,10 @@
     }
     a.x_bytes = (unsigned)((size_t)a.N * img_bytes);
     if (a.y_stride == 0) a.y_stride = a.Cout;
+    if (a.pool_h > 0 && !(plan && plan->kernel == SPLIT_STEM7)) {
+        pp_set_error("conv: a pooled epilogue (ConvArgs::pool_h) exists on the split stem kernel only");
+        return PP_ERR_ARG;
+    }
     if (plan && plan->kernel != SPLIT_NONE) return pp_launch_conv_split(*plan, a, stream);
     if (!plan && a.numerics == 0 && pp_conv_split_enabled()) {
         a.split_f16 = pp_conv_split_f16_default();
@@ -760,8 +781,8 @@
     }
     const size_t total = (size_t)a.N * a.Hout * a.Wout * (a.C / 4);
     if (total == 0) return PP_OK;
-    const int blocks = (int)std::min<size_t>((total + 255) / 256, 256 * 8);
-    hipLaunchKernelGGL(maxpool_kernel, dim3(blocks), dim3(256), 0, stream, a);
+    const size_t chunk = ((total + 256 * 8 - 1) / (256 * 8) + 255) / 256 * 256;
+    hipLaunchKernelGGL(maxpool_kernel, dim3((unsigned)((total + chunk - 1) / chunk)), dim3(256), 0, stream, a, total, chunk);
     hipError_t e = hipGetLastError();
     if (e != hipSuccess) {
         pp_set_error("maxpool launch failed: %s", hipGetErrorString(e));
diff --git a/posepipeline_amd/csrc/conv_split.hip b/posepipeline_amd/csrc/conv_split.hip
--- a/posepipeline_amd/csrc/conv_split.hip
+++ b/posepipeline_amd/csrc/conv_split.hip
@@ -1750,12 +1750,24 @@
     int tiles_x, tiles_y, ntiles;
     unsigned dv_tx[2], dv_ty[2];
     unsigned x_bytes;
+    int Hp, Wp, y_stride, y_coff;
 };
 constexpr int STEM_TH = 16, STEM_TW = 32, STEM_PH = 2 * STEM_TH + 5, STEM_PW = 72, STEM_STEPS = 14;
 constexpr int STEM_PLANE = STEM_PH * STEM_PW * 8, STEM_BUF = 2 * STEM_PLANE, STEM_WBYTES = STEM_STEPS * 2 * 2 * 1024;
 constexpr int STEM_SLOTS = (STEM_PH * STEM_PW + 511) / 512;
 constexpr int STEM_LDS = STEM_WBYTES + 2 * STEM_BUF + 256;
-
+constexpr int STEM_PTH = 7, STEM_PTW = 15;
+constexpr int STEM_LDS_POOL = STEM_LDS + 8 * 2048;
+static_assert(STEM_LDS_POOL <= 160 * 1024, "stem kernel: LDS");
+
+__device__ __forceinline__ float4 pp_max4(const float4 a, const float4 b) {
+    return make_float4(fmaxf(a.x, b.x), fmaxf(a.y, b.y), fmaxf(a.z, b.z), fmaxf(a.w, b.w));
+}
+__device__ __forceinline__ float4 pp_shfl_down4(const float4 v, int d) {
+    return make_float4(__shfl_down(v.x, d), __shfl_down(v.y, d), __shfl_down(v.z, d), __shfl_down(v.w, d));
+}
+
+template <bool POOL>
 __global__ __launch_bounds__(512, 1) void conv_split_stem7_kernel(StemArgs a) {
     extern __shared__ __attribute__((aligned(16))) unsigned char smem[];
     unsigned char* const wl = smem;
@@ -1771,9 +1783,9 @@
     int tn = 0, ty0 = 0, tx0 = 0;
     auto locate = [&](int t, int& n, int& y0, int& x0) {
         const unsigned q = pp_udiv((unsigned)t, a.dv_tx);
-        x0 = (int)((unsigned)t - q * (unsigned)a.tiles_x) * STEM_TW;
+        x0 = (int)((unsigned)t - q * (unsigned)a.tiles_x) * (POOL ? 2 * STEM_PTW : STEM_TW) - (POOL ? 1 : 0);
         n = (int)pp_udiv(q, a.dv_ty);
-        y0 = (int)(q - (unsigned)n * (unsigned)a.tiles_y) * STEM_TH;
+        y0 = (int)(q - (unsigned)n * (unsigned)a.tiles_y) * (POOL ? 2 * STEM_PTH : STEM_TH) - (POOL ? 1 : 0);
     };
     auto load_patch = [&](int t) {
         locate(t, tn, ty0, tx0);
@@ -1875,30 +1887,83 @@
         const float xinv = pp_act_unscale(am);
         unsigned char* const stg = pbase + buf * STEM_BUF + wave * 4096;
         float ymax = 0.f;
-#pragma unroll
-        for (int pb = 0; pb < 2; ++pb) {
-            const int oy = y0 + 2 * wave + pb;
+        if constexpr (POOL) {
+            const float4 ninf = make_float4(-INFINITY, -INFINITY, -INFINITY, -INFINITY);
+            unsigned char* const xch[2] = {smem + STEM_LDS + wave * 2048, stg};
+            const int hofs = (2 * rdrow * 8 + rdc) * 16;
+            float4 hm[2][2];
 #pragma unroll
             for (int cb = 0; cb < 2; ++cb) {
-#pragma unroll
-                for (int g = 0; g < 4; ++g) {
-                    const float4 v = make_float4(acc[cb][pb][4 * g], acc[cb][pb][4 * g + 1], acc[cb][pb][4 * g + 2], acc[cb][pb][4 * g + 3]);
-                    *reinterpret_cast<float4*>(stg + px * 128 + (((2 * g + hk) ^ (px & 7)) << 4)) = v;
+                float4 v[2][4];
+#pragma unroll
+                for (int pb = 0; pb < 2; ++pb) {
+                    const int oy = y0 + 2 * wave + pb;
+#pragma unroll
+                    for (int g = 0; g < 4; ++g) {
+                        const float4 c = make_float4(acc[cb][pb][4 * g], acc[cb][pb][4 * g + 1], acc[cb][pb][4 * g + 2], acc[cb][pb][4 * g + 3]);
+                        *reinterpret_cast<float4*>(stg + px * 128 + (((2 * g + hk) ^ (px & 7)) << 4)) = c;
+                    }
+                    asm volatile("s_waitcnt lgkmcnt(0)" ::: "memory");
+#pragma unroll
+                    for (int r4 = 0; r4 < 4; ++r4) {
+                        const int r = rdrow * 4 + r4, ox = x0 + r;
+                        const float4 c = *reinterpret_cast<const float4*>(stg + r * 128 + ((rdc ^ (r & 7)) << 4));
+                        float4 w = make_float4(__builtin_fmaf(c.x, wsc_l[cb][0] * xinv, bias_l[cb][0]), __builtin_fmaf(c.y, wsc_l[cb][1] * xinv, bias_l[cb][1]),
+                                               __builtin_fmaf(c.z, wsc_l[cb][2] * xinv, bias_l[cb][2]), __builtin_fmaf(c.w, wsc_l[cb][3] * xinv, bias_l[cb][3]));
+                        if (a.relu != PP_RELU_NONE) { w.x = fmaxf(w.x, 0.f); w.y = fmaxf(w.y, 0.f); w.z = fmaxf(w.z, 0.f); w.w = fmaxf(w.w, 0.f); }
+                        v[pb][r4] = ((unsigned)oy < (unsigned)a.Hout && (unsigned)ox < (unsigned)a.Wout) ? w : ninf;
+                    }
+                    asm volatile("s_waitcnt lgkmcnt(0)" ::: "memory");
                 }
-                asm volatile("s_waitcnt lgkmcnt(0)" ::: "memory");
-#pragma unroll
-                for (int r4 = 0; r4 < 4; ++r4) {
-                    const int r = r4 * 8 + rdrow, ox = x0 + r;
-                    const float4 c = *reinterpret_cast<const float4*>(stg + r * 128 + ((rdc ^ (r & 7)) << 4));
-                    float4 v = make_float4(__builtin_fmaf(c.x, wsc_l[cb][0] * xinv, bias_l[cb][0]), __builtin_fmaf(c.y, wsc_l[cb][1] * xinv, bias_l[cb][1]),
-                                           __builtin_fmaf(c.z, wsc_l[cb][2] * xinv, bias_l[cb][2]), __builtin_fmaf(c.w, wsc_l[cb][3] * xinv, bias_l[cb][3]));
-                    if (a.relu != PP_RELU_NONE) { v.x = fmaxf(v.x, 0.f); v.y = fmaxf(v.y, 0.f); v.z = fmaxf(v.z, 0.f); v.w = fmaxf(v.w, 0.f); }
-                    if (oy < a.Hout && ox < a.Wout) {
-                        *reinterpret_cast<float4*>(a.y + (((size_t)n * (a.Hout + a.y_pad) + oy) * (a.Wout + a.y_pad) + ox) * 64 + cb * 32 + 4 * rdc) = v;
-                        ymax = fmaxf(ymax, pp_abs4max(v));
+                float4 m[4];
+#pragma unroll
+                for (int r4 = 0; r4 < 4; ++r4) m[r4] = pp_max4(v[0][r4], v[1][r4]);
+                const float4 mn = pp_shfl_down4(m[0], 8), vn = pp_shfl_down4(v[0][0], 8);
+                hm[cb][0] = pp_max4(pp_max4(m[0], m[1]), m[2]);
+                hm[cb][1] = pp_max4(pp_max4(m[2], m[3]), mn);
+                *reinterpret_cast<float4*>(xch[cb] + hofs) = pp_max4(pp_max4(v[0][0], v[0][1]), v[0][2]);
+                *reinterpret_cast<float4*>(xch[cb] + hofs + 128) = pp_max4(pp_max4(v[0][2], v[0][3]), vn);
+            }
+            __syncthreads();
+            const int py = ((y0 + 1) >> 1) + wave, qx = ((x0 + 1) >> 1) + 2 * rdrow;
+            if (wave < STEM_PTH && py < a.Hp) {
+#pragma unroll
+                for (int cb = 0; cb < 2; ++cb)
+#pragma unroll
+                    for (int i = 0; i < 2; ++i) {
+                        const float4 o = pp_max4(hm[cb][i], *reinterpret_cast<const float4*>(xch[cb] + 2048 * (cb == 0) + 4096 * (cb == 1) + hofs + 128 * i));
+                        if (2 * rdrow + i < STEM_PTW && qx + i < a.Wp) {
+                            *reinterpret_cast<float4*>(a.y + (((size_t)n * (a.Hp + a.y_pad) + py) * (a.Wp + a.y_pad) + qx + i) * a.y_stride + a.y_coff + cb * 32 + 4 * rdc) = o;
+                            ymax = fmaxf(ymax, pp_abs4max(o));
+                        }
                     }
+            }
+        } else {
+    #pragma unroll
+            for (int pb = 0; pb < 2; ++pb) {
+                const int oy = y0 + 2 * wave + pb;
+    #pragma unroll
+                for (int cb = 0; cb < 2; ++cb) {
+    #pragma unroll
+                    for (int g = 0; g < 4; ++g) {
+                        const float4 v = make_float4(acc[cb][pb][4 * g], acc[cb][pb][4 * g + 1], acc[cb][pb][4 * g + 2], acc[cb][pb][4 * g + 3]);
+                        *reinterpret_cast<float4*>(stg + px * 128 + (((2 * g + hk) ^ (px & 7)) << 4)) = v;
+                    }
+                    asm volatile("s_waitcnt lgkmcnt(0)" ::: "memory");
+    #pragma unroll
+                    for (int r4 = 0; r4 < 4; ++r4) {
+                        const int r = r4 * 8 + rdrow, ox = x0 + r;
+                        const float4 c = *reinterpret_cast<const float4*>(stg + r * 128 + ((rdc ^ (r & 7)) << 4));
+                        float4 v = make_float4(__builtin_fmaf(c.x, wsc_l[cb][0] * xinv, bias_l[cb][0]), __builtin_fmaf(c.y, wsc_l[cb][1] * xinv, bias_l[cb][1]),
+                                               __builtin_fmaf(c.z, wsc_l[cb][2] * xinv, bias_l[cb][2]), __builtin_fmaf(c.w, wsc_l[cb][3] * xinv, bias_l[cb][3]));
+                        if (a.relu != PP_RELU_NONE) { v.x = fmaxf(v.x, 0.f); v.y = fmaxf(v.y, 0.f); v.z = fmaxf(v.z, 0.f); v.w = fmaxf(v.w, 0.f); }
+                        if (oy < a.Hout && ox < a.Wout) {
+                            *reinterpret_cast<float4*>(a.y + (((size_t)n * (a.Hout + a.y_pad) + oy) * (a.Wout + a.y_pad) + ox) * 64 + cb * 32 + 4 * rdc) = v;
+                            ymax = fmaxf(ymax, pp_abs4max(v));
+                        }
+                    }
+                    asm volatile("s_waitcnt lgkmcnt(0)" ::: "memory");
                 }
-                asm volatile("s_waitcnt lgkmcnt(0)" ::: "memory");
             }
         }
         if (a.y_amax) {
@@ -2198,8 +2263,15 @@
     s.x_amax = a.x_amax; s.y_amax = a.y_amax;
     s.N = a.N; s.Hin = a.Hin; s.Win = a.Win; s.xp_h = a.Hin + a.x_pad; s.xp_w = a.Win + a.x_pad;
     s.Hout = a.Hout; s.Wout = a.Wout; s.y_pad = a.y_pad; s.relu = a.relu;
-    s.tiles_x = (a.Wout + STEM_TW - 1) / STEM_TW;
-    s.tiles_y = (a.Hout + STEM_TH - 1) / STEM_TH;
+    const bool pool = a.pool_h > 0;
+    if (pool && (a.pool_h != (a.Hout - 1) / 2 + 1 || a.pool_w != (a.Wout - 1) / 2 + 1 || (a.y_coff & 3) || (a.y_stride & 3) || a.y_coff + 64 > a.y_stride)) {
+        pp_set_error("conv_split_stem7: pooled output %dx%d (channels %d .. of %d) does not fit the %dx%d stem map", a.pool_h, a.pool_w, a.y_coff,
+                     a.y_stride, a.Hout, a.Wout);
+        return PP_ERR_ARG;
+    }
+    s.Hp = a.pool_h; s.Wp = a.pool_w; s.y_stride = a.y_stride; s.y_coff = a.y_coff;
+    s.tiles_x = pool ? (a.pool_w + STEM_PTW - 1) / STEM_PTW : (a.Wout + STEM_TW - 1) / STEM_TW;
+    s.tiles_y = pool ? (a.pool_h + STEM_PTH - 1) / STEM_PTH : (a.Hout + STEM_TH - 1) / STEM_TH;
     s.ntiles = a.N * s.tiles_x * s.tiles_y;
     s.x_bytes = a.x_bytes;
     make_magic((unsigned)s.tiles_x, s.dv_tx);
@@ -2209,7 +2281,8 @@
         if (hipGetDevice(&dev) == hipSuccess) (void)hipDeviceGetAttribute(&n, hipDeviceAttributeMultiprocessorCount, dev);
         return n > 0 ? n : 256;
     }();
-    launch_split<conv_split_stem7_kernel, STEM_LDS>(dim3((unsigned)std::min(s.ntiles, ncu)), 512, STEM_LDS, stream, s);
+    if (pool) launch_split<conv_split_stem7_kernel<true>, STEM_LDS_POOL>(dim3((unsigned)std::min(s.ntiles, ncu)), 512, STEM_LDS_POOL, stream, s);
+    else launch_split<conv_split_stem7_kernel<false>, STEM_LDS>(dim3((unsigned)std::min(s.ntiles, ncu)), 512, STEM_LDS, stream, s);
     hipError_t e = hipGetLastError();
     if (e != hipSuccess) {
         pp_set_error("conv_split_stem7 launch failed: %s", hipGetErrorString(e));
diff --git a/posepipeline_amd/csrc/crop_affine.hip b/posepipeline_amd/csrc/crop_affine.hip
--- a/posepipeline_amd/csrc/crop_affine.hip
+++ b/posepipeline_amd/csrc/crop_affine.hip
@@ -1,6 +1,7 @@
 #include <cmath>
 
 #include "pp_internal.h"
+#include "pp_amax.h"
 
 namespace {
 
@@ -17,7 +18,8 @@
                                                           const PersonXform* __restrict__ xf, int n_person,
                                                           int out_w, int out_h, const float* __restrict__ lut,
                                                           int cm0, int cm1, int cm2, int flip,
-                                                          float* __restrict__ out, uint8_t* __restrict__ crop_u8) {
+                                                          float* __restrict__ out, uint8_t* __restrict__ crop_u8,
+                                                          unsigned* __restrict__ amax) {
     __shared__ float s_lut[3 * 256];
     for (int i = threadIdx.x; i < 768; i += blockDim.x) s_lut[i] = lut[i];
     __syncthreads();
@@ -28,6 +30,7 @@
     float* o0 = out + (size_t)person * sample;
     float* o1 = out + (size_t)(n_person + person) * sample;
     const uint8_t* img = frames + (size_t)t.frame * H * W * 3;
+    float vmax = 0.f;
     for (int p = blockIdx.x * blockDim.x + threadIdx.x; p < npix; p += gridDim.x * blockDim.x) {
         const int y = p / out_w;
         const int x = p - y * out_w;
@@ -60,11 +63,20 @@
             v.z = s_lut[2 * 256 + c3[cm2]];
         }
         *reinterpret_cast<float4*>(o0 + (size_t)p * 4) = v;
+        vmax = fmaxf(vmax, pp_abs4max(v));
         if (flip) *reinterpret_cast<float4*>(o1 + ((size_t)y * out_w + (out_w - 1 - x)) * 4) = v;
         if (crop_u8) {
             uint8_t* cp = crop_u8 + ((size_t)person * npix + p) * 3;
             cp[0] = c3[0]; cp[1] = c3[1]; cp[2] = c3[2];
         }
+    }
+    if (amax) {
+        __shared__ float red[16];
+        const int im[1] = {person};
+        const float mm[1] = {vmax};
+        pp_amax_commit_wg<4, 1>(amax, im, mm, person, person, red);
+        const int imf[1] = {n_person + person};
+        if (flip) pp_amax_commit_wg<4, 1>(amax, imf, mm, imf[0], imf[0], red);
     }
 }
 
@@ -169,12 +181,12 @@
 
 int pp_enqueue_crop(hipStream_t s, const uint8_t* frames, int h, int w, const PersonXform* xf, int n_person,
                     int out_w, int out_h, const float* lut, const int32_t chan_map[3], int flip, float* out,
-                    uint8_t* crop_u8) {
+                    uint8_t* crop_u8, unsigned* amax) {
     if (n_person <= 0) return PP_OK;
     const int npix = out_w * out_h;
     dim3 grid(std::min((npix + 255) / 256, 64), n_person);
     hipLaunchKernelGGL(crop_affine_kernel, grid, dim3(256), 0, s, frames, h, w, xf, n_person, out_w, out_h, lut,
-                       chan_map[0], chan_map[1], chan_map[2], flip, out, crop_u8);
+                       chan_map[0], chan_map[1], chan_map[2], flip, out, crop_u8, amax);
     PP_HIP_CHECK(hipGetLastError());
     return PP_OK;
 }
diff --git a/posepipeline_amd/csrc/pp_internal.h b/posepipeline_amd/csrc/pp_internal.h
--- a/posepipeline_amd/csrc/pp_internal.h
+++ b/posepipeline_amd/csrc/pp_internal.h
@@ -111,6 +111,7 @@
     int split_f16;
     const unsigned* x_amax;
     unsigned* y_amax;
+    int pool_h, pool_w;
 };
 struct TileGeom {
     int TH, TW, bw_log2, gx_log2, PWp, NP, NPp, tiles_x, tiles_y;
@@ -154,6 +155,7 @@
     float* y;
     int N, Hin, Win, C, Hout, Wout, KH, KW, stride, pad_h, pad_w;
     int x_stride, x_coff, y_stride, y_coff;
+    unsigned* y_amax;
 };
 int pp_launch_maxpool(const PoolArgs& a, hipStream_t stream);
 int pp_launch_avgpool(const float* x, float* y, int n, int hin, int win, int c, int kh, int kw, int stride, hipStream_t stream);
@@ -205,7 +207,7 @@
 bool pp_person_transform(const double* bbox_tlwh, int out_w, int out_h, float center_scale[4], PersonXform* t, int udp = 0);
 int pp_enqueue_crop(hipStream_t s, const uint8_t* frames, int h, int w, const PersonXform* xf, int n_person,
                     int out_w, int out_h, const float* lut, const int32_t chan_map[3], int flip, float* out,
-                    uint8_t* crop_u8);
+                    uint8_t* crop_u8, unsigned* amax = nullptr);
 int pp_enqueue_flip_w(hipStream_t s, const float* src, float* dst, int n, int h, int w);
 
 struct DecodeParams {
diff --git a/posepipeline_amd/csrc/topdown.hip b/posepipeline_amd/csrc/topdown.hip
--- a/posepipeline_amd/csrc/topdown.hip
+++ b/posepipeline_amd/csrc/topdown.hip
@@ -1,6 +1,8 @@
+#include <cstdlib>
 #include <memory>
 
 #include "pp_internal.h"
+#include "pp_amax.h"
 
 struct pp_topdown {
     pp_ctx* ctx = nullptr;
@@ -10,6 +12,7 @@
     int flip = 0, shift_heatmap = 0, post = 0, blur_kernel = 0;
     int32_t chan_map[3] = {0, 1, 2};
     int max_person = 0;
+    unsigned* in_amax = nullptr;
     float* d_lut = nullptr;
     int32_t* d_perm = nullptr;
     PersonXform* d_xf = nullptr;
@@ -51,6 +54,10 @@
     }
     t->max_person = pp_net_max_batch(net) / (t->flip ? 2 : 1);
     PP_REQUIRE(t->max_person > 0, "pp_topdown_create: net max_batch too small");
+    {
+        const char* env = getenv("POSEPIPE_CROP_AMAX");
+        if (!env || atoi(env) != 0) t->in_amax = pp_net_input_amax_slot(net, in_buf);
+    }
     hipStream_t s = t->ctx->stream;
     PP_HIP_CHECK(hipSetDevice(t->ctx->device));
     PP_HIP_CHECK(hipMalloc((void**)&t->d_lut, 768 * sizeof(float)));
@@ -153,9 +160,16 @@
     void* in_ptr = nullptr;
     int rc = pp_net_buffer(t->net, t->in_buf, &in_ptr, nullptr);
     if (rc != PP_OK) return rc;
+    const int batch = n_person * (t->flip ? 2 : 1);
+    if (t->in_amax) PP_HIP_CHECK(hipMemsetAsync(t->in_amax, 0, (size_t)batch * sizeof(unsigned), s));
     rc = pp_enqueue_crop(s, dframes, h, w, t->d_xf, n_person, t->in_w, t->in_h, t->d_lut, t->chan_map, t->flip,
-                         static_cast<float*>(in_ptr), nullptr);
-    if (rc != PP_OK) return rc;
+                         static_cast<float*>(in_ptr), nullptr, t->in_amax);
+    if (rc != PP_OK) return rc;
+    if (t->in_amax) {
+        void* am = nullptr;
+        rc = pp_net_input_amax(t->net, t->in_buf, &am);
+        if (rc != PP_OK) return rc;
+    }
     return topdown_tail(t, n_person, kpts, kpts_mem, true);
 }
 
```

Result: no change. 616.8, median of 6 (+0.4%).
